# maxpit/human-pose-estimation

Measured on AMD Instinct MI355X. Metric: images/sec (224x224, batch 256/GPU), higher is better.
Workload: dtype f32; 1 GPU; batch=256/GPU 224x224x3 synthetic images, fp32 ResNet-50 v1 + 3-iter regressor + SMPL LBS at all 3 stages (configs[1] at batch 256; the BASELINE metric batch); global_batch=256, parallelism=dp1 (batch shard, replicated weights), regressor=synthetic 'survey' variant, input=float32 images resident in HBM

## Files before the change

human-pose-estimation_amd/_lib.py:

```python
from __future__ import annotations

import ctypes as C
import os

import numpy as np

_HERE = os.path.dirname(os.path.abspath(__file__))
LIB_PATH = os.path.join(_HERE, "lib", "libhpe_hip.so")

NUM_CONV = 53
NUM_DENSE = 3
NUM_VERTS = 6890
THETA_DIM = 85
FEATURE_DIM = 2048


class HpeError(RuntimeError):
    pass


class HpeConfig(C.Structure):
    _fields_ = [
        ("struct_size", C.c_int),
        ("device", C.c_int),
        ("max_batch", C.c_int),
        ("num_stage", C.c_int),
        ("bn_eps", C.c_float),
        ("encoder_dtype", C.c_int),
        ("n_streams", C.c_int),
        ("dual_gemm", C.c_int),
        ("stem_fused", C.c_int),
        ("wino_min_c", C.c_int),
        ("wino_min_items", C.c_int),
        ("wino_fused", C.c_int),
        ("wino_fused_min_hw", C.c_int),
        ("mesh_a2b", C.c_int),
        ("wino_f4", C.c_int),
        ("wino4_fused", C.c_int),
        ("bf16_p8", C.c_int),
        ("wino4_ksplit", C.c_int),
        ("chain_fuse", C.c_int),
        ("halo3", C.c_int),
    ]


PLAN_OPTIONS = ("n_streams", "dual_gemm", "stem_fused", "wino_min_c", "wino_min_items", "wino_fused", "wino_fused_min_hw", "mesh_a2b", "wino_f4", "wino4_fused", "bf16_p8", "wino4_ksplit", "chain_fuse", "halo3")


class HpeSmplModel(C.Structure):
    _fields_ = [
        ("v_template", C.c_void_p),
        ("shapedirs", C.c_void_p),
        ("posedirs", C.c_void_p),
        ("J_regressor", C.c_void_p),
        ("weights", C.c_void_p),
        ("kp_regressor", C.c_void_p),
        ("parents", C.c_void_p),
        ("num_kp", C.c_int),
    ]


class HpeRenderParams(C.Structure):
    _fields_ = [
        ("struct_size", C.c_int),
        ("color_id", C.c_int),
        ("do_alpha", C.c_int),
        ("rot_axis", C.c_int),
        ("rot_deg", C.c_float),
        ("near", C.c_float),
        ("far", C.c_float),
    ]


OUTPUT_FIELDS = ("verts", "joints", "cams", "theta", "J_transformed", "kp2d", "verts2d", "Rs")


class HpeOutputs(C.Structure):
    _fields_ = [(n, C.c_void_p) for n in OUTPUT_FIELDS]


_PROTOS = {
    "hpe_last_error": (C.c_char_p, []),
    "hpe_version": (C.c_char_p, []),
    "hpe_conv_layer_name": (C.c_char_p, [C.c_int]),
    "hpe_bn_layer_name": (C.c_char_p, [C.c_int]),
    "hpe_conv_layer_geometry": (C.c_int, [C.c_int, C.POINTER(C.c_int)]),
    "hpe_config_init": (None, [C.POINTER(HpeConfig)]),
    "hpe_create": (C.c_int, [C.POINTER(HpeConfig), C.POINTER(C.c_void_p)]),
    "hpe_destroy": (C.c_int, [C.c_void_p]),
    "hpe_load_smpl": (C.c_int, [C.c_void_p, C.POINTER(HpeSmplModel)]),
    "hpe_load_conv": (C.c_int, [C.c_void_p, C.c_int] + [C.c_void_p] * 6),
    "hpe_load_dense": (C.c_int, [C.c_void_p, C.c_int, C.c_void_p, C.c_void_p]),
    "hpe_load_mean_theta": (C.c_int, [C.c_void_p, C.c_void_p]),
    "hpe_finalize": (C.c_int, [C.c_void_p]),
    "hpe_forward": (C.c_int, [C.c_void_p, C.c_void_p, C.c_int, C.POINTER(HpeOutputs), C.c_int, C.c_void_p]),
    "hpe_forward_pipelined": (C.c_int, [C.c_void_p, C.c_void_p, C.c_int, C.POINTER(HpeOutputs), C.c_int, C.c_void_p]),
    "hpe_join": (C.c_int, [C.c_void_p, C.c_void_p]),
    "hpe_tail": (C.c_int, [C.c_void_p, C.c_void_p, C.c_int, C.POINTER(HpeOutputs), C.c_int, C.c_void_p]),
    "hpe_tail_stream": (C.c_void_p, [C.c_void_p]),
    "hpe_encoder": (C.c_int, [C.c_void_p, C.c_void_p, C.c_int, C.c_void_p, C.c_void_p]),
    "hpe_regress_stage": (C.c_int, [C.c_void_p, C.c_void_p, C.c_void_p, C.c_int, C.c_void_p, C.c_void_p]),
    "hpe_smpl": (C.c_int, [C.c_void_p, C.c_void_p, C.c_int, C.POINTER(HpeOutputs), C.c_void_p]),
    "hpe_orth_proj": (C.c_int, [C.c_void_p, C.c_void_p, C.c_int, C.c_int, C.c_void_p, C.c_void_p]),
    "hpe_reproject_vertices": (C.c_int, [C.c_void_p, C.c_void_p, C.c_int, C.c_int, C.c_float, C.c_float, C.c_void_p, C.c_void_p]),
    "hpe_preprocess_u8": (C.c_int, [C.c_void_p, C.c_int, C.c_int, C.c_int, C.c_void_p, C.POINTER(C.c_int), C.c_void_p]),
    "hpe_preprocess_u8_batch": (C.c_int, [C.c_void_p, C.POINTER(C.c_longlong), C.POINTER(C.c_int), C.c_int, C.c_int, C.c_void_p, C.POINTER(C.c_int),
                                          C.c_void_p, C.c_void_p]),
    "hpe_get_original": (C.c_int, [C.c_void_p, C.c_void_p, C.c_int, C.c_int, C.c_int, C.POINTER(C.c_int), C.c_float, C.c_int, C.c_void_p, C.POINTER(C.c_float), C.c_void_p, C.c_void_p, C.c_void_p]),
    "hpe_kp_loss": (C.c_int, [C.c_void_p, C.c_void_p, C.c_int, C.c_int, C.c_void_p, C.c_void_p]),
    "hpe_mesh_loss": (C.c_int, [C.c_void_p, C.c_void_p, C.c_void_p, C.c_int, C.c_int, C.c_int, C.c_int, C.c_void_p, C.c_void_p]),
    "hpe_val_losses": (C.c_int, [C.c_void_p, C.c_void_p, C.c_void_p, C.POINTER(C.c_void_p), C.POINTER(C.c_void_p), C.c_int, C.c_int, C.c_int,
                                 C.c_int, C.c_int, C.c_int, C.c_void_p, C.c_void_p]),
    "hpe_device_status": (C.c_int, [C.c_void_p, C.c_void_p]),
    "hpe_debug_conv": (C.c_int, [C.c_void_p, C.c_int, C.c_void_p, C.c_int, C.c_void_p, C.c_int, C.c_void_p, C.c_void_p]),
    "hpe_debug_chain": (C.c_int, [C.c_void_p, C.c_int, C.c_void_p, C.c_void_p, C.c_int, C.c_void_p, C.c_void_p, C.POINTER(C.c_int), C.c_void_p]),
    "hpe_debug_stem": (C.c_int, [C.c_void_p, C.c_void_p, C.c_int, C.c_int, C.c_void_p, C.c_void_p]),
    "hpe_debug_gemm": (C.c_int, [C.c_void_p, C.c_void_p, C.c_void_p, C.c_int, C.c_int, C.c_int, C.c_int, C.c_int, C.c_void_p, C.c_int, C.c_void_p, C.c_void_p]),
    "hpe_debug_set_dbg": (C.c_int, [C.c_void_p, C.c_void_p]),
    "hpe_debug_maxpool": (C.c_int, [C.c_void_p, C.c_int, C.c_int, C.c_int, C.c_void_p, C.c_void_p]),
    "hpe_debug_avgpool": (C.c_int, [C.c_void_p, C.c_int, C.c_int, C.c_int, C.c_void_p, C.c_void_p]),
    "hpe_debug_joint_regress": (C.c_int, [C.c_void_p, C.c_void_p, C.c_int, C.c_int, C.c_void_p, C.c_void_p]),
    "hpe_enable_timing": (C.c_int, [C.c_void_p, C.c_int]),
    "hpe_get_timings": (C.c_int, [C.c_void_p, C.POINTER(C.c_float)]),
    "hpe_get_span_stats": (C.c_int, [C.c_void_p, C.POINTER(C.c_float), C.POINTER(C.c_int)]),
    "hpe_get_loss_timings": (C.c_int, [C.c_void_p, C.POINTER(C.c_float)]),
    "hpe_debug_set_loss_counter": (C.c_int, [C.c_void_p, C.c_void_p]),
    "hpe_get_conv_timings": (C.c_int, [C.c_void_p, C.POINTER(C.c_float)]),
    "hpe_render_params_init": (None, [C.POINTER(HpeRenderParams)]),
    "hpe_renderer_create": (C.c_int, [C.c_int, C.c_void_p, C.c_int, C.c_int, C.c_int, C.POINTER(C.c_void_p)]),
    "hpe_renderer_destroy": (C.c_int, [C.c_void_p]),
    "hpe_render": (C.c_int, [C.c_void_p, C.c_void_p, C.c_void_p, C.c_int, C.c_int, C.c_int, C.c_void_p, C.POINTER(HpeRenderParams), C.c_void_p,
                             C.c_void_p]),
    "hpe_debug_render_ids": (C.c_int, [C.c_void_p, C.c_void_p, C.c_void_p, C.c_int, C.c_int, C.c_int, C.POINTER(HpeRenderParams), C.c_void_p,
                                       C.c_void_p, C.c_void_p]),
    "hpe_debug_render_vertices": (C.c_int, [C.c_void_p, C.c_void_p, C.c_void_p, C.c_int, C.c_int, C.c_int, C.POINTER(HpeRenderParams),
                                            C.c_void_p, C.c_void_p]),
}

_lib = None


def load():
    global _lib
    if _lib is not None:
        return _lib
    if not os.path.exists(LIB_PATH):
        raise HpeError(
            "%s not found: build it with `python -c 'import __graft_entry__ as g; g.build()'` "
            "(hipcc --offload-arch=gfx950).  There is no CPU fallback." % LIB_PATH
        )
    try:
        import torch
    except Exception:
        pass
    lib = C.CDLL(LIB_PATH, mode=C.RTLD_GLOBAL)
    for name, (res, args) in _PROTOS.items():
        fn = getattr(lib, name)
        fn.restype = res
        fn.argtypes = args
    _lib = lib
    return lib


def declared_symbols():
    return sorted(_PROTOS)


def check(rc):
    if rc != 0:
        msg = load().hpe_last_error()
        raise HpeError("libhpe_hip error %d: %s" % (rc, msg.decode() if msg else "?"))


def f32(a):
    arr = np.ascontiguousarray(a, dtype=np.float32)
    return arr, arr.ctypes.data_as(C.c_void_p)
```

human-pose-estimation_amd/build.py:

```python
from __future__ import annotations

import os
import shutil
import subprocess
import sys

HERE = os.path.dirname(os.path.abspath(__file__))
CSRC = os.path.join(HERE, "csrc")
LIBDIR = os.path.join(HERE, "lib")
LIB = os.path.join(LIBDIR, "libhpe_hip.so")
SOURCES = ["conv_gemm.hip", "conv_gemm_bf16.hip", "conv_gemm_bf16_p8.hip", "conv_chain_bf16.hip", "conv_chain_f32.hip", "conv3_halo_bf16.hip", "conv_wino.hip", "conv_wino4.hip", "stem_fused.hip", "encoder_ops.hip", "smpl.hip", "losses.hip", "prepost.hip", "render.hip", "hpe_api.hip"]
CFLAGS = ["--offload-arch=gfx950", "-O3", "-std=c++17", "-fPIC", "-fvisibility=hidden", "-fno-fast-math"]


def _hipcc():
    for cand in (os.environ.get("HIPCC"), shutil.which("hipcc"), "/opt/rocm/bin/hipcc"):
        if cand and os.path.exists(cand):
            return cand
    raise RuntimeError("hipcc not found (set HIPCC or install ROCm under /opt/rocm)")


def _deps():
    return [os.path.join(CSRC, f) for f in os.listdir(CSRC) if f.endswith(".h")] + [os.path.join(HERE, "..", "include", "hpe.h")]


def _obj_stale(src, obj):
    if not os.path.exists(obj):
        return True
    t = os.path.getmtime(obj)
    return any(os.path.getmtime(d) > t for d in [src] + _deps() if os.path.exists(d))


def _flags_now():
    return " ".join(CFLAGS + os.environ.get("HPE_EXTRA_FLAGS", "").split())


def built_flags():
    tag = os.path.join(LIBDIR, "obj", "flags.txt")
    return open(tag).read() if os.path.exists(tag) else ""


def _stale():
    if not os.path.exists(LIB):
        return True
    if built_flags() != _flags_now():
        return True
    t = os.path.getmtime(LIB)
    deps = [os.path.join(CSRC, f) for f in os.listdir(CSRC)] + [os.path.join(HERE, "..", "include", "hpe.h")]
    return any(os.path.getmtime(d) > t for d in deps if os.path.exists(d))


def build(force=False, verbose=False):
    if not force and not _stale():
        return LIB
    os.makedirs(LIBDIR, exist_ok=True)
    objdir = os.path.join(LIBDIR, "obj")
    os.makedirs(objdir, exist_ok=True)
    extra = os.environ.get("HPE_EXTRA_FLAGS", "").split()
    tag = os.path.join(objdir, "flags.txt")
    flags_now = _flags_now()
    if force or not os.path.exists(tag) or open(tag).read() != flags_now:
        for f in os.listdir(objdir):
            os.remove(os.path.join(objdir, f))
    hipcc = _hipcc()
    jobs = []
    for s in SOURCES:
        src = os.path.join(CSRC, s)
        if not os.path.exists(src):
            continue
        obj = os.path.join(objdir, s.replace(".hip", ".o"))
        jobs.append((src, obj))

    def compile_one(job):
        src, obj = job
        if not _obj_stale(src, obj):
            return None
        cmd = [hipcc] + CFLAGS + extra + ["-c", "-o", obj + ".tmp%d" % os.getpid(), src]
        if verbose:
            print(" ".join(cmd), file=sys.stderr)
        r = subprocess.run(cmd, capture_output=True, text=True)
        if r.returncode != 0:
            return "hipcc failed on %s:\n%s%s" % (os.path.basename(src), r.stdout, r.stderr)
        os.replace(obj + ".tmp%d" % os.getpid(), obj)
        return None

    from concurrent.futures import ThreadPoolExecutor

    with ThreadPoolExecutor(max_workers=min(len(jobs), max(1, (os.cpu_count() or 2) - 1))) as ex:
        errs = [e for e in ex.map(compile_one, jobs) if e]
    if errs:
        raise RuntimeError("\n".join(errs))
    open(tag, "w").write(flags_now)
    tmp = LIB + ".tmp%d" % os.getpid()
    cmd = [hipcc, "--offload-arch=gfx950", "-shared", "-fPIC", "-o", tmp] + [o for _, o in jobs]
    r = subprocess.run(cmd, capture_output=True, text=True)
    if r.returncode != 0:
        raise RuntimeError("link failed:\n" + r.stdout + r.stderr)
    os.replace(tmp, LIB)
    return LIB


if __name__ == "__main__":
    print(build(force="--force" in sys.argv, verbose=True))
```

human-pose-estimation_amd/csrc/conv_gemm.hip:

```cpp
#include <hip/hip_runtime.h>
#include <stdint.h>
#include <stdlib.h>

#include "hpe_internal.h"

typedef float f32x16 __attribute__((ext_vector_type(16)));
typedef float f32x4 __attribute__((ext_vector_type(4)));

#define BK 32
#define LDS_PITCH 36

namespace {

struct RowAddr {
    int base;
    unsigned mask;
};

template <int MODE>
__device__ __forceinline__ RowAddr make_row(const GemmArgs& p, int m, int kc4) {
    RowAddr r;
    r.mask = 0x1ffu;
    if (m >= p.M) m = p.M - 1;
    if (MODE == GEMM_DENSE || MODE == GEMM_DUAL) {
        r.base = m * p.lda + kc4;
    } else {
        const int hw = p.Ho * p.Wo;
        const int b = m / hw;
        const int rem = m - b * hw;
        const int ho = rem / p.Wo;
        const int wo = rem - ho * p.Wo;
        if (MODE == GEMM_STRIDED) {
            r.base = ((b * p.Hi + ho * p.stride) * p.Wi + wo * p.stride) * p.Cin + kc4;
        } else if (MODE == GEMM_CONV3) {
            r.base = ((b * p.Hi + ho) * p.Wi + wo) * p.Cin + kc4;
            unsigned mk = 0;
#pragma unroll
            for (int tap = 0; tap < 9; ++tap) {
                const int dh = tap / 3 - 1, dw = tap % 3 - 1;
                if ((unsigned)(ho + dh) < (unsigned)p.Hi && (unsigned)(wo + dw) < (unsigned)p.Wi) mk |= 1u << tap;
            }
            r.mask = mk;
        } else {
            r.base = ((b * p.Hi + 2 * ho) * p.Wi + 2 * wo) * 4 + kc4;
        }
    }
    return r;
}

struct SlabPos {
    int off;
    int tap;
    int cs;
};

template <int MODE>
__device__ __forceinline__ void slab_advance(const GemmArgs& p, SlabPos& sp) {
    if (MODE == GEMM_DENSE || MODE == GEMM_STRIDED || MODE == GEMM_DUAL) {
        sp.off += BK;
    } else if (MODE == GEMM_CONV3) {
        sp.cs += 1;
        sp.off += BK;
        if (sp.cs == p.cin_slabs) {
            sp.cs = 0;
            sp.tap += 1;
            const int kh = sp.tap / 3;
            sp.off = ((kh - 1) * p.Wi + (sp.tap - kh * 3 - 1)) * p.Cin;
        }
    } else {
        sp.off += p.Wi * 4;
    }
}

template <int MODE>
__device__ __forceinline__ SlabPos slab_first(const GemmArgs& p) {
    SlabPos sp;
    sp.tap = 0;
    sp.cs = 0;
    sp.off = (MODE == GEMM_CONV3) ? (-p.Wi - 1) * p.Cin : 0;
    return sp;
}

template <int MODE>
__device__ __forceinline__ SlabPos slab_seek(const GemmArgs& p, int slab) {
    SlabPos sp;
    sp.tap = 0;
    sp.cs = 0;
    if (MODE == GEMM_DENSE || MODE == GEMM_STRIDED || MODE == GEMM_DUAL) {
        sp.off = slab * BK;
    } else if (MODE == GEMM_CONV3) {
        sp.tap = slab / p.cin_slabs;
        sp.cs = slab - sp.tap * p.cin_slabs;
        const int kh = sp.tap / 3;
        sp.off = ((kh - 1) * p.Wi + (sp.tap - kh * 3 - 1)) * p.Cin + sp.cs * BK;
    } else {
        sp.off = slab * p.Wi * 4;
    }
    return sp;
}

template <int MODE>
__device__ __forceinline__ f32x4 load_a(const GemmArgs& p, const RowAddr& r, const SlabPos& sp) {
    if (MODE == GEMM_CONV3) {
        const bool ok = (r.mask >> sp.tap) & 1u;
        f32x4 v = *reinterpret_cast<const f32x4*>(p.x + (r.base + (ok ? sp.off : sp.cs * BK)));
        const f32x4 z = {0.f, 0.f, 0.f, 0.f};
        return ok ? v : z;
    }
    return *reinterpret_cast<const f32x4*>(p.x + (r.base + sp.off));
}

template <int MODE, int BM, int BN, int WM, int WN, int SCHED>
__global__ __launch_bounds__(256, 2) void conv_gemm_f32_kernel(GemmArgs p) {
    constexpr int MT = BM / WM / 32;
    constexpr int NT = BN / WN / 32;
    constexpr int AP = BM / 32;
    constexpr int BP = BN / 32;
    constexpr int EP = BN + 4;
    static_assert(WM * WN == 4, "4 waves per workgroup");
    static_assert(MT >= 1 && NT >= 1, "tile too small");
    static_assert(BM * EP <= 2 * (BM + BN) * LDS_PITCH, "epilogue tile must fit the staging LDS");

    __shared__ __attribute__((aligned(16))) float lds[2 * (BM + BN) * LDS_PITCH];
    constexpr int BUF = (BM + BN) * LDS_PITCH;

    const int total = p.n_mtiles * p.n_ntiles;
    const int bid = blockIdx.x;
    const int xcd = bid & 7;
    const int q = total >> 3, rr = total & 7;
    const int swz = (xcd < rr ? xcd * (q + 1) : rr * (q + 1) + (xcd - rr) * q) + (bid >> 3);
    const int mtile = swz / p.n_ntiles;
    const int ntile = swz - mtile * p.n_ntiles;
    const int m0 = mtile * BM;
    const int n0 = ntile * BN;

    const int t = threadIdx.x;
    const int lane = t & 63;
    const int wave = __builtin_amdgcn_readfirstlane(t >> 6);
    const int wm = wave / WN;
    const int wn = wave - wm * WN;

    const int kc4 = (t & 7) * 4;
    const int srow = t >> 3;
    RowAddr arow[AP];
#pragma unroll
    for (int i = 0; i < AP; ++i) arow[i] = make_row<MODE>(p, m0 + srow + 32 * i, kc4);
    const float* wptr = p.w + (size_t)(n0 + srow) * p.ldw + kc4;
    const int lds_st = srow * LDS_PITCH + kc4;

    const int frag = (lane & 31) * LDS_PITCH + 4 * (lane >> 5);
    const int a_off = (wm * MT * 32) * LDS_PITCH + frag;
    const int b_off = (BM + wn * NT * 32) * LDS_PITCH + frag;

    f32x16 acc[MT][NT];
#pragma unroll
    for (int i = 0; i < MT; ++i)
#pragma unroll
        for (int j = 0; j < NT; ++j)
#pragma unroll
            for (int e = 0; e < 16; ++e) acc[i][j][e] = 0.f;

    f32x4 ra[AP], rb[BP];
    const int S = p.K / BK;
    SlabPos sp = slab_first<MODE>(p);

    auto load_slab = [&](int slab) {
#pragma unroll
        for (int i = 0; i < AP; ++i) ra[i] = load_a<MODE>(p, arow[i], sp);
#pragma unroll
        for (int i = 0; i < BP; ++i) rb[i] = *reinterpret_cast<const f32x4*>(wptr + (size_t)(32 * i) * p.ldw + slab * BK);
    };
    auto store_slab = [&](int buf) {
#pragma unroll
        for (int i = 0; i < AP; ++i) *reinterpret_cast<f32x4*>(&lds[buf + lds_st + 32 * i * LDS_PITCH]) = ra[i];
#pragma unroll
        for (int i = 0; i < BP; ++i) *reinterpret_cast<f32x4*>(&lds[buf + lds_st + (BM + 32 * i) * LDS_PITCH]) = rb[i];
    };
    auto mma_groups = [&](int buf, int g0, int g1) {
        const float* A = &lds[buf + a_off];
        const float* B = &lds[buf + b_off];
#pragma unroll
        for (int g = g0; g < g1; ++g) {
            f32x4 fa[MT], fb[NT];
#pragma unroll
            for (int i = 0; i < MT; ++i) fa[i] = *reinterpret_cast<const f32x4*>(A + i * 32 * LDS_PITCH + g * 8);
#pragma unroll
            for (int j = 0; j < NT; ++j) fb[j] = *reinterpret_cast<const f32x4*>(B + j * 32 * LDS_PITCH + g * 8);
#pragma unroll
            for (int ks = 0; ks < 4; ++ks)
#pragma unroll
                for (int i = 0; i < MT; ++i)
#pragma unroll
                    for (int j = 0; j < NT; ++j)
                        acc[i][j] = __builtin_amdgcn_mfma_f32_32x32x2f32(fa[i][ks], fb[j][ks], acc[i][j], 0, 0, 0);
        }
    };

#ifdef HPE_ABLATION
    unsigned long long t_clk0 = 0, t_rt0 = 0;
    if (p.dbg) {
        t_clk0 = __builtin_amdgcn_s_memtime();
        t_rt0 = __builtin_amdgcn_s_memrealtime();
    }
#endif
    load_slab(0);
    store_slab(0);
    if (S > 1) {
        slab_advance<MODE>(p, sp);
        load_slab(1);
    }
    __syncthreads();

    if (SCHED == 8 || SCHED == 9) {
        constexpr int QA = AP / 4 > 0 ? AP / 4 : 1;
        constexpr int QB = BP / 4 > 0 ? BP / 4 : 1;
        constexpr int GA = AP / QA, GB = BP / QB;
        constexpr int MPG = 4 * MT * NT;
        int s = 0;
        for (; s + 2 < S; ++s) {
            const int cur = (s & 1) * BUF;
            const int nxt = BUF - cur;
            const float* A = &lds[cur + a_off];
            const float* B = &lds[cur + b_off];
            slab_advance<MODE>(p, sp);
            f32x4 fa[2][MT], fb[2][NT];
#pragma unroll
            for (int i = 0; i < MT; ++i) fa[0][i] = *reinterpret_cast<const f32x4*>(A + i * 32 * LDS_PITCH);
#pragma unroll
            for (int j = 0; j < NT; ++j) fb[0][j] = *reinterpret_cast<const f32x4*>(B + j * 32 * LDS_PITCH);
#define HPE_KGROUP(G)                                                                                                  \
    {                                                                                                                  \
        if (G < 3) {                                                                                                   \
            _Pragma("unroll") for (int i = 0; i < MT; ++i) fa[(G + 1) & 1][i] =                                        \
                *reinterpret_cast<const f32x4*>(A + i * 32 * LDS_PITCH + (G + 1) * 8);                                 \
            _Pragma("unroll") for (int j = 0; j < NT; ++j) fb[(G + 1) & 1][j] =                                        \
                *reinterpret_cast<const f32x4*>(B + j * 32 * LDS_PITCH + (G + 1) * 8);                                 \
        }                                                                                                              \
        _Pragma("unroll") for (int ks = 0; ks < 4; ++ks) _Pragma("unroll") for (int i = 0; i < MT; ++i)                \
            _Pragma("unroll") for (int j = 0; j < NT; ++j) acc[i][j] =                                                 \
                __builtin_amdgcn_mfma_f32_32x32x2f32(fa[G & 1][i][ks], fb[G & 1][j][ks], acc[i][j], 0, 0, 0);          \
        if (G < GA) {                                                                                                  \
            _Pragma("unroll") for (int q = 0; q < QA; ++q) {                                                           \
                const int i = G * QA + q;                                                                              \
                *reinterpret_cast<f32x4*>(&lds[nxt + lds_st + 32 * i * LDS_PITCH]) = ra[i];                            \
                ra[i] = load_a<MODE>(p, arow[i], sp);                                                                  \
            }                                                                                                          \
        }                                                                                                              \
        if (G < GB) {                                                                                                  \
            _Pragma("unroll") for (int q = 0; q < QB; ++q) {                                                           \
                const int i = G * QB + q;                                                                              \
                *reinterpret_cast<f32x4*>(&lds[nxt + lds_st + (BM + 32 * i) * LDS_PITCH]) = rb[i];                     \
                rb[i] = *reinterpret_cast<const f32x4*>(wptr + (size_t)(32 * i) * p.ldw + (s + 2) * BK);               \
            }                                                                                                          \
        }                                                                                                              \
        if (SCHED == 9) {                                                                                              \
            constexpr int NST = (G < GA ? QA : 0) + (G < GB ? QB : 0);                                                 \
            if (G < 3) __builtin_amdgcn_sched_group_barrier(0x100, MT + NT, 0);                                        \
            if constexpr (NST == 0) {                                                                                  \
                __builtin_amdgcn_sched_group_barrier(0x008, MPG, 0);                                                   \
            } else {                                                                                                   \
                _Pragma("unroll") for (int q = 0; q < NST; ++q) {                                                      \
                    __builtin_amdgcn_sched_group_barrier(0x008, MPG / NST, 0);                                         \
                    __builtin_amdgcn_sched_group_barrier(0x200, 1, 0);                                                 \
                    __builtin_amdgcn_sched_group_barrier(0x020, 1, 0);                                                 \
                }                                                                                                      \
            }                                                                                                          \
        }                                                                                                              \
    }
            HPE_KGROUP(0)
            HPE_KGROUP(1)
            HPE_KGROUP(2)
            HPE_KGROUP(3)
#undef HPE_KGROUP
            __syncthreads();
        }
        for (; s < S; ++s) {
            const int cur = (s & 1) * BUF;
            mma_groups(cur, 0, 2);
            if (s + 1 < S) store_slab(BUF - cur);
            mma_groups(cur, 2, 4);
            __syncthreads();
        }
    } else
    for (int s = 0; s < S; ++s) {
        const int cur = (s & 1) * BUF;
        if (SCHED == 0) {
            mma_groups(cur, 0, 2);
            if (s + 1 < S) {
                store_slab(BUF - cur);
                if (s + 2 < S) {
                    slab_advance<MODE>(p, sp);
                    load_slab(s + 2);
                }
            }
            mma_groups(cur, 2, 4);
        } else if (SCHED == 1) {
            mma_groups(cur, 0, 2);
            __builtin_amdgcn_sched_barrier(0);
            if (s + 1 < S) {
                store_slab(BUF - cur);
                __builtin_amdgcn_sched_barrier(0);
                if (s + 2 < S) {
                    slab_advance<MODE>(p, sp);
                    load_slab(s + 2);
                }
            }
            __builtin_amdgcn_sched_barrier(0);
            mma_groups(cur, 2, 4);
        } else if (SCHED == 6) {
            if (s + 2 < S) {
                slab_advance<MODE>(p, sp);
                load_slab(s + 2);
            }
            mma_groups(cur, 0, 4);
#pragma unroll
            for (int i = 0; i < AP; ++i) asm volatile("" ::"v"(ra[i]));
#pragma unroll
            for (int i = 0; i < BP; ++i) asm volatile("" ::"v"(rb[i]));
        } else if (SCHED == 7) {
            mma_groups(cur, 0, 2);
            if (s + 1 < S) store_slab(BUF - cur);
            mma_groups(cur, 2, 4);
        } else if (SCHED == 3) {
            mma_groups(cur, 0, 4);
        } else if (SCHED == 4) {
            mma_groups(0, 0, 4);
            continue;
        } else if (SCHED == 5) {
            f32x4 fa[MT], fb[NT];
#pragma unroll
            for (int i = 0; i < MT; ++i) fa[i] = ra[i % AP];
#pragma unroll
            for (int j = 0; j < NT; ++j) fb[j] = rb[j % BP];
#pragma unroll
            for (int g = 0; g < 4; ++g)
#pragma unroll
                for (int ks = 0; ks < 4; ++ks)
#pragma unroll
                    for (int i = 0; i < MT; ++i)
#pragma unroll
                        for (int j = 0; j < NT; ++j)
                            acc[i][j] = __builtin_amdgcn_mfma_f32_32x32x2f32(fa[i][ks], fb[j][ks], acc[i][j], 0, 0, 0);
            continue;
        } else {
            mma_groups(cur, 0, 1);
            __builtin_amdgcn_sched_barrier(0);
            if (s + 1 < S) store_slab(BUF - cur);
            mma_groups(cur, 1, 2);
            __builtin_amdgcn_sched_barrier(0);
            if (s + 2 < S) {
                slab_advance<MODE>(p, sp);
                load_slab(s + 2);
            }
            mma_groups(cur, 2, 3);
            __builtin_amdgcn_sched_barrier(0);
            mma_groups(cur, 3, 4);
        }
        __syncthreads();
    }

#ifdef HPE_ABLATION
    if (p.dbg && t == 0) {
        p.dbg[2 * bid] = __builtin_amdgcn_s_memtime() - t_clk0;
        p.dbg[2 * bid + 1] = __builtin_amdgcn_s_memrealtime() - t_rt0;
    }
#endif
    {
        const int col_l = lane & 31;
        const int row_l = 4 * (lane >> 5);
#pragma unroll
        for (int j = 0; j < NT; ++j) {
            const int cl = (wn * NT + j) * 32 + col_l;
            const int n = n0 + cl;
            const bool n_ok = n < p.N;
            const float sc = n_ok ? p.scale[n] : 0.f;
            const float sh = n_ok ? p.shift[n] : 0.f;
#pragma unroll
            for (int i = 0; i < MT; ++i) {
                const int rl = (wm * MT + i) * 32 + row_l;
#pragma unroll
                for (int e = 0; e < 16; ++e) lds[(rl + (e & 3) + 8 * (e >> 2)) * EP + cl] = acc[i][j][e] * sc + sh;
            }
        }
    }
    __syncthreads();
    {
        constexpr int TPR = BN / 4;
        constexpr int RPP = 256 / TPR;
        const int r = t / TPR;
        const int c4 = (t - r * TPR) * 4;
        const int n = n0 + c4;
        const bool full = (n + 3) < p.N;
#pragma unroll 4
        for (int pass = 0; pass < BM / RPP; ++pass) {
            const int row = pass * RPP + r;
            const int m = m0 + row;
            if (m >= p.M || n >= p.N) continue;
            f32x4 v = *reinterpret_cast<const f32x4*>(&lds[row * EP + c4]);
            if (full) {
                if (p.res) v += *reinterpret_cast<const f32x4*>(p.res + (size_t)m * p.ldres + n);
                if (p.relu) {
                    v.x = fmaxf(v.x, 0.f);
                    v.y = fmaxf(v.y, 0.f);
                    v.z = fmaxf(v.z, 0.f);
                    v.w = fmaxf(v.w, 0.f);
                }
                if (p.y_slab8)
                    *reinterpret_cast<f32x4*>(p.y + ((size_t)(n >> 3) * p.M + m) * 8 + (n & 7)) = v;
                else
                    *reinterpret_cast<f32x4*>(p.y + (size_t)m * p.ldy + n) = v;
            } else {
                const float vv[4] = {v.x, v.y, v.z, v.w};
#pragma unroll
                for (int u = 0; u < 4; ++u) {
                    if (n + u < p.N) {
                        float o = vv[u];
                        if (p.res) o += p.res[(size_t)m * p.ldres + n + u];
                        if (p.relu) o = fmaxf(o, 0.f);
                        p.y[(size_t)m * p.ldy + n + u] = o;
                    }
                }
            }
        }
    }
}

#ifdef HPE_F32_RES_NT
#define HPE_RES_LOAD(ptr) __builtin_nontemporal_load(ptr)
#else
#define HPE_RES_LOAD(ptr) (*(ptr))
#endif
template <int BM, int BN, int WM, int WN, int NP>
__device__ __forceinline__ void conv_epilogue(const GemmArgs& p, float* lds, f32x16 (&acc)[BM / WM / 32][BN / WN / 32], int m0, int n0, int t,
                                              int lane, int wm, int wn, const f32x4 (&rpre)[NP], bool use_pre) {
    constexpr int MT = BM / WM / 32;
    constexpr int NT = BN / WN / 32;
    constexpr int NTHR = 64 * WM * WN;
    constexpr int EP = BN + 4;
    {
        const int col_l = lane & 31;
        const int row_l = 4 * (lane >> 5);
#pragma unroll
        for (int j = 0; j < NT; ++j) {
            const int cl = (wn * NT + j) * 32 + col_l;
            const int n = n0 + cl;
            const bool n_ok = n < p.N;
            const float sc = n_ok ? p.scale[n] : 0.f;
            const float sh = n_ok ? p.shift[n] : 0.f;
#pragma unroll
            for (int i = 0; i < MT; ++i) {
                const int rl = (wm * MT + i) * 32 + row_l;
#pragma unroll
                for (int e = 0; e < 16; ++e) lds[(rl + (e & 3) + 8 * (e >> 2)) * EP + cl] = acc[i][j][e] * sc + sh;
            }
        }
    }
    __syncthreads();
    {
        constexpr int TPR = BN / 4;
        constexpr int RPP = NTHR / TPR;
        const int r = t / TPR;
        const int c4 = (t - r * TPR) * 4;
        const int n = n0 + c4;
        const bool full = (n + 3) < p.N;
#pragma unroll
        for (int pass = 0; pass < BM / RPP; ++pass) {
            const int row = pass * RPP + r;
            const int m = m0 + row;
            if (m >= p.M || n >= p.N) continue;
            f32x4 v = *reinterpret_cast<const f32x4*>(&lds[row * EP + c4]);
            if (full) {
                if (use_pre) v += rpre[pass < NP ? pass : 0];
                else if (p.res) v += HPE_RES_LOAD(reinterpret_cast<const f32x4*>(p.res + (size_t)m * p.ldres + n));
                if (p.relu) {
                    v.x = fmaxf(v.x, 0.f);
                    v.y = fmaxf(v.y, 0.f);
                    v.z = fmaxf(v.z, 0.f);
                    v.w = fmaxf(v.w, 0.f);
                }
                if (p.y_slab8)
                    *reinterpret_cast<f32x4*>(p.y + ((size_t)(n >> 3) * p.M + m) * 8 + (n & 7)) = v;
                else
                    *reinterpret_cast<f32x4*>(p.y + (size_t)m * p.ldy + n) = v;
            } else {
                const float vv[4] = {v.x, v.y, v.z, v.w};
#pragma unroll
                for (int u = 0; u < 4; ++u) {
                    if (n + u < p.N) {
                        float o = vv[u];
                        if (p.res) o += p.res[(size_t)m * p.ldres + n + u];
                        if (p.relu) o = fmaxf(o, 0.f);
                        p.y[(size_t)m * p.ldy + n + u] = o;
                    }
                }
            }
        }
    }
}

template <int MODE, int BM, int BN, int WM, int WN>
__global__ __launch_bounds__(64 * WM * WN, (WM * WN) / 2) void conv_gemm_f32_dma_kernel(GemmArgs p) {
    constexpr int MT = BM / WM / 32;
    constexpr int NT = BN / WN / 32;
    constexpr int NW = WM * WN;
    constexpr int NTHR = 64 * NW;
    constexpr int AP = BM / (8 * NW);
    constexpr int BP = BN / (8 * NW);
    constexpr int EP = BN + 4;
    constexpr int BUF = (BM + BN) * BK;
    constexpr int LDS_FLOATS = (2 * BUF > BM * EP) ? 2 * BUF : BM * EP;
    static_assert(NW == 4 || NW == 8, "4 or 8 waves per workgroup");
    static_assert(AP >= 1 && BP >= 1, "tile too small for the wave count");

    __shared__ __attribute__((aligned(16))) float lds[LDS_FLOATS];

    const int total = p.n_mtiles * p.n_ntiles;
    const int bid = blockIdx.x;
    int tile, ks0 = 0, ks1 = p.K / BK, part = -1;
    if (p.split_k > 1) {
        tile = bid / p.split_k;
        part = bid - tile * p.split_k;
        const int S = p.K / BK;
        ks0 = (int)((long)part * S / p.split_k);
        ks1 = (int)((long)(part + 1) * S / p.split_k);
    } else {
        const int xcd = bid & 7;
        const int q = total >> 3, rr = total & 7;
        tile = (xcd < rr ? xcd * (q + 1) : rr * (q + 1) + (xcd - rr) * q) + (bid >> 3);
    }
    const int mtile = tile / p.n_ntiles;
    const int ntile = tile - mtile * p.n_ntiles;
    const int m0 = mtile * BM;
    const int n0 = ntile * BN;

    const int t = threadIdx.x;
    const int lane = t & 63;
    const int wave = __builtin_amdgcn_readfirstlane(t >> 6);
    const int wm = wave / WN;
    const int wn = wave - wm * WN;

    const int drow = lane >> 3;
    RowAddr arow[AP];
    int arow2[MODE == GEMM_DUAL ? AP : 1];
    const float* wsrc[BP];
#pragma unroll
    for (int i = 0; i < AP; ++i) {
        const int r = (NW * i + wave) * 8 + drow;
        const int lc = (lane & 7) ^ ((r >> 1) & 7);
        arow[i] = make_row<MODE>(p, m0 + r, lc * 4);
        if (MODE == GEMM_DUAL) arow2[i] = make_row<GEMM_STRIDED>(p, m0 + r, lc * 4).base;
    }
#pragma unroll
    for (int i = 0; i < BP; ++i) {
        const int r = (NW * i + wave) * 8 + drow;
        const int lc = (lane & 7) ^ ((r >> 1) & 7);
        wsrc[i] = p.w + (size_t)(n0 + r) * p.ldw + lc * 4;
    }

    int a_row[MT], b_row[NT], a_x[MT], b_x[NT];
#pragma unroll
    for (int i = 0; i < MT; ++i) {
        const int r = (wm * MT + i) * 32 + (lane & 31);
        a_row[i] = r * BK;
        a_x[i] = (r >> 1) & 7;
    }
#pragma unroll
    for (int j = 0; j < NT; ++j) {
        const int r = (wn * NT + j) * 32 + (lane & 31);
        b_row[j] = (BM + r) * BK;
        b_x[j] = (r >> 1) & 7;
    }
    const int hi = lane >> 5;

    f32x16 acc[MT][NT];
#pragma unroll
    for (int i = 0; i < MT; ++i)
#pragma unroll
        for (int j = 0; j < NT; ++j)
#pragma unroll
            for (int e = 0; e < 16; ++e) acc[i][j][e] = 0.f;

    constexpr int R_TPR = BN / 4, R_RPP = NTHR / R_TPR, R_NPASS = BM / R_RPP;
    constexpr bool R_PRE = (NW == 8) && R_NPASS <= 4;
    f32x4 rpre[R_PRE ? R_NPASS : 1];
    bool r_pre = false;
    if constexpr (R_PRE) {
        const int rr_ = t / R_TPR;
        const int n = n0 + (t - rr_ * R_TPR) * 4;
        r_pre = p.res != nullptr && p.res_prefetch && part < 0 && (n + 3) < p.N;
        if (r_pre) {
#pragma unroll
            for (int pass = 0; pass < R_NPASS; ++pass) {
                const int m = m0 + pass * R_RPP + rr_;
                rpre[pass] = HPE_RES_LOAD(reinterpret_cast<const f32x4*>(p.res + (size_t)(m < p.M ? m : p.M - 1) * p.ldres + n));
            }
        }
    }

    SlabPos sp = slab_seek<MODE>(p, ks0);

    auto issue_dma = [&](int slab, int buf) {
#pragma unroll
        for (int i = 0; i < AP; ++i) {
            const float* src;
            if (MODE == GEMM_CONV3) {
                const bool ok = (arow[i].mask >> sp.tap) & 1u;
                src = ok ? (p.x + (arow[i].base + sp.off)) : p.zero;
            } else if (MODE == GEMM_DUAL) {
                src = slab < p.k1_slabs ? p.x + (arow[i].base + slab * BK) : p.x2 + (arow2[i] + (slab - p.k1_slabs) * BK);
            } else {
                src = p.x + (arow[i].base + sp.off);
            }
            __builtin_amdgcn_global_load_lds((const __attribute__((address_space(1))) void*)src,
                                             (__attribute__((address_space(3))) void*)(lds + buf + (NW * i + wave) * 8 * BK), 16, 0, 0);
        }
#pragma unroll
        for (int i = 0; i < BP; ++i) {
            __builtin_amdgcn_global_load_lds((const __attribute__((address_space(1))) void*)(wsrc[i] + slab * BK),
                                             (__attribute__((address_space(3))) void*)(lds + buf + (BM + (NW * i + wave) * 8) * BK), 16, 0,
                                             0);
        }
    };

    issue_dma(ks0, 0);
    __builtin_amdgcn_s_waitcnt(0x0F70);
    __syncthreads();

    for (int s = ks0; s < ks1; ++s) {
        const int cur = ((s - ks0) & 1) * BUF;
        if (s + 1 < ks1) {
            slab_advance<MODE>(p, sp);
            issue_dma(s + 1, BUF - cur);
        }
#pragma unroll
        for (int g = 0; g < 4; ++g) {
            f32x4 fa[MT], fb[NT];
            const int lc = 2 * g + hi;
#pragma unroll
            for (int i = 0; i < MT; ++i) fa[i] = *reinterpret_cast<const f32x4*>(&lds[cur + a_row[i] + ((lc ^ a_x[i]) << 2)]);
#pragma unroll
            for (int j = 0; j < NT; ++j) fb[j] = *reinterpret_cast<const f32x4*>(&lds[cur + b_row[j] + ((lc ^ b_x[j]) << 2)]);
#pragma unroll
            for (int ks = 0; ks < 4; ++ks)
#pragma unroll
                for (int i = 0; i < MT; ++i)
#pragma unroll
                    for (int j = 0; j < NT; ++j)
                        acc[i][j] = __builtin_amdgcn_mfma_f32_32x32x2f32(fa[i][ks], fb[j][ks], acc[i][j], 0, 0, 0);
        }
        __builtin_amdgcn_s_waitcnt(0x0F70);
        __syncthreads();
    }

    if (part >= 0) {
        f32x4* dst = reinterpret_cast<f32x4*>(p.partial) + (size_t)(tile * p.split_k + part) * (MT * NT * 4 * NTHR) + t;
#pragma unroll
        for (int i = 0; i < MT; ++i)
#pragma unroll
            for (int j = 0; j < NT; ++j)
#pragma unroll
                for (int qd = 0; qd < 4; ++qd) {
                    f32x4 v = {acc[i][j][4 * qd], acc[i][j][4 * qd + 1], acc[i][j][4 * qd + 2], acc[i][j][4 * qd + 3]};
                    dst[((i * NT + j) * 4 + qd) * NTHR] = v;
                }
        return;
    }
    conv_epilogue<BM, BN, WM, WN>(p, lds, acc, m0, n0, t, lane, wm, wn, rpre, R_PRE && r_pre);
}

template <int BM, int BN, int WM, int WN>
__global__ __launch_bounds__(64 * WM * WN) void conv_gemm_fixup_kernel(GemmArgs p) {
    constexpr int MT = BM / WM / 32;
    constexpr int NT = BN / WN / 32;
    constexpr int NTHR = 64 * WM * WN;
    constexpr int EP = BN + 4;
    __shared__ __attribute__((aligned(16))) float lds[BM * EP];
    const int t = threadIdx.x;
    const int lane = t & 63;
    const int wave = __builtin_amdgcn_readfirstlane(t >> 6);
    const int wm = wave / WN;
    const int wn = wave - wm * WN;
    const int tile = blockIdx.x;
    const int mtile = tile / p.n_ntiles;
    const int ntile = tile - mtile * p.n_ntiles;
    f32x16 acc[MT][NT];
#pragma unroll
    for (int i = 0; i < MT; ++i)
#pragma unroll
        for (int j = 0; j < NT; ++j)
#pragma unroll
            for (int e = 0; e < 16; ++e) acc[i][j][e] = 0.f;
    const f32x4* src = reinterpret_cast<const f32x4*>(p.partial) + (size_t)tile * p.split_k * (MT * NT * 4 * NTHR) + t;
    for (int part = 0; part < p.split_k; ++part) {
#pragma unroll
        for (int i = 0; i < MT; ++i)
#pragma unroll
            for (int j = 0; j < NT; ++j)
#pragma unroll
                for (int qd = 0; qd < 4; ++qd) {
                    const f32x4 v = src[(size_t)part * (MT * NT * 4 * NTHR) + ((i * NT + j) * 4 + qd) * NTHR];
                    acc[i][j][4 * qd] += v.x;
                    acc[i][j][4 * qd + 1] += v.y;
                    acc[i][j][4 * qd + 2] += v.z;
                    acc[i][j][4 * qd + 3] += v.w;
                }
    }
    const f32x4 no_pre[1] = {{0.f, 0.f, 0.f, 0.f}};
    conv_epilogue<BM, BN, WM, WN>(p, lds, acc, mtile * BM, ntile * BN, t, lane, wm, wn, no_pre, false);
}

int stage_variant() {
    static const int v = [] {
        const char* e = getenv("HPE_STAGE");
        return (e && e[0] == 'r') ? 0 : 1;
    }();
    return v;
}

int sched_variant() {
    static const int v = [] {
        const char* e = getenv("HPE_SCHED");
        const int x = e ? atoi(e) : 0;
        return (x < 0 || x > 9) ? 0 : x;
    }();
    return v;
}

int splitk_enabled() {
    static const int v = [] {
        const char* e = getenv("HPE_SPLITK");
        return e ? atoi(e) : 1;
    }();
    return v;
}

template <int MODE, int BM, int BN, int WM, int WN>
hipError_t launch_cfg(GemmArgs& p, hipStream_t st) {
    p.n_mtiles = (p.M + BM - 1) / BM;
    p.n_ntiles = (p.N + BN - 1) / BN;
    const int grid = p.n_mtiles * p.n_ntiles;
    p.split_k = 1;
    if constexpr (WM * WN == 8) {
        static const int res_prefetch = [] {
            const char* e = getenv("HPE_RES_PREFETCH");
            return e ? atoi(e) : 1;
        }();
        p.res_prefetch = res_prefetch;
        hipLaunchKernelGGL((conv_gemm_f32_dma_kernel<MODE, BM, BN, WM, WN>), dim3(grid), dim3(512), 0, st, p);
        return hipGetLastError();
    } else {
    if ((stage_variant() == 1 && p.zero) || MODE == GEMM_DUAL) {
        const int S = p.K / BK;
        static const int min_slabs = [] {
            const char* e = getenv("HPE_SPLITK_SLABS");
            const int v = e ? atoi(e) : 4;
            return v < 2 ? 2 : v;
        }();
        if (p.partial && splitk_enabled() && grid < 128 && S >= 2 * min_slabs) {
            int sk = 256 / grid;
            if (sk > S / min_slabs) sk = S / min_slabs;
            if (sk > 16) sk = 16;
            while (sk > 1 && (size_t)grid * sk * BM * BN > p.partial_floats) --sk;
            if (sk > 1) p.split_k = sk;
        }
        hipLaunchKernelGGL((conv_gemm_f32_dma_kernel<MODE, BM, BN, WM, WN>), dim3(grid * p.split_k), dim3(256), 0, st, p);
        hipError_t e = hipGetLastError();
        if (e != hipSuccess || p.split_k == 1) return e;
        hipLaunchKernelGGL((conv_gemm_fixup_kernel<BM, BN, WM, WN>), dim3(grid), dim3(256), 0, st, p);
        return hipGetLastError();
    }
    if constexpr (MODE == GEMM_DUAL) return hipErrorInvalidValue;
    else
    switch (sched_variant()) {
        case 1: hipLaunchKernelGGL((conv_gemm_f32_kernel<MODE, BM, BN, WM, WN, 1>), dim3(grid), dim3(256), 0, st, p); break;
        case 2: hipLaunchKernelGGL((conv_gemm_f32_kernel<MODE, BM, BN, WM, WN, 2>), dim3(grid), dim3(256), 0, st, p); break;
#ifdef HPE_ABLATION
        case 3: hipLaunchKernelGGL((conv_gemm_f32_kernel<MODE, BM, BN, WM, WN, 3>), dim3(grid), dim3(256), 0, st, p); break;
        case 4: hipLaunchKernelGGL((conv_gemm_f32_kernel<MODE, BM, BN, WM, WN, 4>), dim3(grid), dim3(256), 0, st, p); break;
        case 5: hipLaunchKernelGGL((conv_gemm_f32_kernel<MODE, BM, BN, WM, WN, 5>), dim3(grid), dim3(256), 0, st, p); break;
        case 6: hipLaunchKernelGGL((conv_gemm_f32_kernel<MODE, BM, BN, WM, WN, 6>), dim3(grid), dim3(256), 0, st, p); break;
        case 7: hipLaunchKernelGGL((conv_gemm_f32_kernel<MODE, BM, BN, WM, WN, 7>), dim3(grid), dim3(256), 0, st, p); break;
        case 8: hipLaunchKernelGGL((conv_gemm_f32_kernel<MODE, BM, BN, WM, WN, 8>), dim3(grid), dim3(256), 0, st, p); break;
        case 9: hipLaunchKernelGGL((conv_gemm_f32_kernel<MODE, BM, BN, WM, WN, 9>), dim3(grid), dim3(256), 0, st, p); break;
#endif
        default: hipLaunchKernelGGL((conv_gemm_f32_kernel<MODE, BM, BN, WM, WN, 0>), dim3(grid), dim3(256), 0, st, p); break;
    }
    return hipGetLastError();
    }
}

template <int MODE>
hipError_t launch_mode(GemmArgs& p, int tile, hipStream_t st) {
    switch (tile) {
        case TILE_128x128: return launch_cfg<MODE, 128, 128, 2, 2>(p, st);
        case TILE_128x64: return launch_cfg<MODE, 128, 64, 2, 2>(p, st);
        case TILE_64x64: return launch_cfg<MODE, 64, 64, 2, 2>(p, st);
        case TILE_64x128: return launch_cfg<MODE, 64, 128, 2, 2>(p, st);
        case TILE_128x128_W8: return launch_cfg<MODE, 128, 128, 2, 4>(p, st);
        case TILE_128x64_W8: return launch_cfg<MODE, 128, 64, 4, 2>(p, st);
        case TILE_256x128_W8: return launch_cfg<MODE, 256, 128, 4, 2>(p, st);
        default: return hipErrorInvalidValue;
    }
// ... 39 lines not shown
```

human-pose-estimation_amd/csrc/hpe_api.hip:

```cpp
#include <hip/hip_runtime.h>

#include <cmath>
#include <cstdint>
#include <cstdio>
#include <cstdlib>
#include <cstring>
#include <string>
#include <vector>

#include "../../include/hpe.h"
#include "hpe_internal.h"

namespace {

thread_local std::string g_err;

int fail(int code, const std::string& msg) {
    g_err = msg;
    return code;
}

#define HIP_TRY(expr)                                                                                             \
    do {                                                                                                          \
        hipError_t _e = (expr);                                                                                   \
        if (_e != hipSuccess)                                                                                     \
            return fail(HPE_ERR_HIP, std::string(#expr) + ": " + hipGetErrorString(_e) + " (" __FILE__ ":" +      \
                                         std::to_string(__LINE__) + ")");                                         \
    } while (0)

struct ConvSpec {
    char name[24];
    char bn[24];
    int kh, kw, cin, cout, stride, hin, hout;
};

std::vector<ConvSpec> build_specs() {
    std::vector<ConvSpec> v;
    auto add = [&](const std::string& n, const std::string& b, int kh, int cin, int cout, int s, int hin, int hout) {
        ConvSpec c;
        snprintf(c.name, sizeof c.name, "%s", n.c_str());
        snprintf(c.bn, sizeof c.bn, "%s", b.c_str());
        c.kh = c.kw = kh;
        c.cin = cin;
        c.cout = cout;
        c.stride = s;
        c.hin = hin;
        c.hout = hout;
        v.push_back(c);
    };
    add("conv1", "bn_conv1", 7, 3, 64, 2, 224, 112);
    const int nblk[4] = {3, 4, 6, 3};
    const int filt[4][3] = {{64, 64, 256}, {128, 128, 512}, {256, 256, 1024}, {512, 512, 2048}};
    int cin = 64, h = 56;
    for (int st = 0; st < 4; ++st) {
        for (int b = 0; b < nblk[st]; ++b) {
            const bool first = b == 0;
            const int s = (first && st > 0) ? 2 : 1;
            const int hout = h / s;
            char base[24], bn[24];
            snprintf(base, sizeof base, "res%d%c_branch", st + 2, 'a' + b);
            snprintf(bn, sizeof bn, "bn%d%c_branch", st + 2, 'a' + b);
            add(std::string(base) + "2a", std::string(bn) + "2a", 1, cin, filt[st][0], s, h, hout);
            add(std::string(base) + "2b", std::string(bn) + "2b", 3, filt[st][0], filt[st][1], 1, hout, hout);
            add(std::string(base) + "2c", std::string(bn) + "2c", 1, filt[st][1], filt[st][2], 1, hout, hout);
            if (first) add(std::string(base) + "1", std::string(bn) + "1", 1, cin, filt[st][2], s, h, hout);
            cin = filt[st][2];
            h = hout;
        }
    }
    return v;
}

const std::vector<ConvSpec>& specs() {
    static const std::vector<ConvSpec> s = build_specs();
    return s;
}

inline int round_up(int x, int m) { return ((x + m - 1) / m) * m; }

struct ConvLayer {
    std::vector<float> kernel, bias, gamma, beta, mean, var;
    bool loaded = false;
    float* w = nullptr;
    float* scale = nullptr;
    float* shift = nullptr;
    float* w_dual = nullptr;
    float* shift_dual = nullptr;
    int k_dual = 0, k1_dual = 0;
    void* stem_w = nullptr;
    float* wino_u = nullptr;
    float* wino4_u = nullptr;
    int n_pad = 0, k_pad = 0;
};

inline unsigned short f2bf(float f) {
    unsigned u;
    memcpy(&u, &f, 4);
    return (unsigned short)((u + 0x7FFFu + ((u >> 16) & 1u)) >> 16);
}

struct DenseLayer {
    std::vector<float> kernel, bias;
    bool loaded = false;
};

constexpr int STEM_HP = 230;
constexpr int STEM_WP = 232;
constexpr int THETA_LD = 96;
constexpr size_t WINO_V_PITCH = 802816 + 16384;
constexpr size_t WINO_V_SLACK = 524288;

}

struct TileKnobs {
    int force_wide = -1, force_narrow = -1, shortk = TILE_128x64_W8, force_bf16 = -1;
    int bf16_128_min_tiles = 192;
    int concurrent_tiles = 0;
    int wide128_min_tiles = 384;
    int force_expand = -1;
    int expand_small_grid = 128;
    int bf16_w8_min_tiles = 128;
    int force_ns_bf16 = -1;
    int bf16_rules = 1;
    int bf16_p8 = 0;
    int bf16_p8_min_n = 256;
    int bf16_p8_min_k = 512;
};

struct hpe_ctx {
    HpeConfig cfg{};
    bool finalized = false;
    bool dead = false;
    TileKnobs knobs;
    bool bf16 = false;
    bool have_encoder = false, have_regressor = false, have_smpl = false;
    ConvLayer conv[HPE_NUM_CONV];
    DenseLayer dense[HPE_NUM_DENSE];
    bool smpl_loaded = false, mean_loaded = false;
    std::vector<float> h_vt, h_sd, h_pd, h_jreg, h_w, h_kreg;
    std::vector<int> h_par;
    int num_kp = 19;
    float h_mean[HPE_THETA_DIM];
    float *w1f = nullptr, *w1t = nullptr, *w2 = nullptr, *w3 = nullptr, *b1 = nullptr, *b2 = nullptr, *b3 = nullptr;
    float *ones = nullptr, *zeros = nullptr, *mean_dev = nullptr;
    SmplDev smpl{};
    SmplWork work{};
    float* smpl_basis_src = nullptr;
    float *padded = nullptr, *X0 = nullptr, *X1 = nullptr, *T1 = nullptr, *T2 = nullptr, *SC = nullptr;
    float *feat = nullptr, *P1 = nullptr, *H1 = nullptr, *H2 = nullptr, *thA = nullptr, *thB = nullptr;
    float* loss_ws = nullptr;
    unsigned long long* dbg = nullptr;
    size_t loss_ws_floats = 0;
    std::vector<void*> allocs;
    int n_streams = 1;
    float* partial = nullptr;
    size_t partial_floats = 0;
    int chunk_images = 0;
    float* wino_v = nullptr;
    float* wino_ws = nullptr;
    unsigned* wino_flags = nullptr;
    unsigned* dev_err = nullptr;
    unsigned wino_epoch = 0;
    int n_cu = 0;
    int wino_min_c = 128;
    int wino_min_items = 128;
    int wino_fused_min_hw = 28;
    int dual_gemm = 1;
    int stem_fused = 1;
    int wino4_min_items = 64;
    int wino4_fused = 0;
    int wino_f4 = 0;
    int mesh_a2b = 0;
    bool loss_attr_done = false;
    unsigned long long* loss_counter = nullptr;
    int wino_fused = 1;
    hipStream_t aux[3]{};
    int min_chunk = 32;
    hipEvent_t ev_fork{}, ev_join[3]{};
    hipStream_t tail_st{};
    hipEvent_t ev_enc{}, ev_tail{}, ev_feat_free[2]{};
    bool feat_free_valid[2] = {false, false};
    bool tail_pending = false;
    unsigned pipe_idx = 0;
    float* feat_alt = nullptr;
    int wino4_ksplit = 1;
    int halo3_two = 4;
    int halo3 = 0;
    int chain_fuse = 0;
    int co_running = 1;
    float* w4_split = nullptr;
    float* partial_tail = nullptr;
    size_t partial_tail_floats = 0;
    bool dense_on_tail = false;
    int timing = 0;
    hipEvent_t ev[8]{};
    static constexpr int SPAN_RING = 64;
    hipEvent_t span0[SPAN_RING]{}, span1[SPAN_RING]{};
    unsigned span_n = 0;
    hipEvent_t cev0[HPE_NUM_CONV]{}, cev1[HPE_NUM_CONV]{};
    hipEvent_t lev0[16]{}, lev1[16]{}, lev_all[2]{};
    int loss_timed_stages = 0;
    bool ev_ok = false, timed_valid = false, conv_timed_valid = false;
};

namespace {

struct DeviceGuard {
    int prev = -1;
    bool changed = false;
    explicit DeviceGuard(int dev) {
        if (hipGetDevice(&prev) == hipSuccess && prev != dev) changed = hipSetDevice(dev) == hipSuccess;
    }
    ~DeviceGuard() {
        if (changed) (void)hipSetDevice(prev);
    }
};

int dev_alloc(hpe_ctx* c, float** p, size_t n_floats, bool zero) {
    void* q = nullptr;
    HIP_TRY(hipMalloc(&q, n_floats * sizeof(float)));
    c->allocs.push_back(q);
    if (zero) HIP_TRY(hipMemset(q, 0, n_floats * sizeof(float)));
    *p = static_cast<float*>(q);
    return HPE_OK;
}

int upload(hpe_ctx* c, float** p, const std::vector<float>& h) {
    int rc = dev_alloc(c, p, h.size(), false);
    if (rc) return rc;
    HIP_TRY(hipMemcpy(*p, h.data(), h.size() * sizeof(float), hipMemcpyHostToDevice));
    return HPE_OK;
}

int pick_tile(const TileKnobs& kn, int M, int N, int K, bool residual_expand = false, bool concurrent = false) {
    const bool wide = N > 64;
    if (wide && residual_expand) {
        if (kn.force_expand >= 0) return kn.force_expand;
        return (long)((M + 127) / 128) * ((N + 63) / 64) < kn.expand_small_grid ? TILE_64x64 : TILE_128x64_W8;
    }
    if (wide && kn.force_wide >= 0) return kn.force_wide;
    if (!wide && kn.force_narrow >= 0) return kn.force_narrow;
    if (!wide) return TILE_128x64;
    if (K <= 128 && M >= 150000) return kn.shortk;
    if ((concurrent || kn.concurrent_tiles) && kn.wide128_min_tiles > 0 && (long)((M + 127) / 128) * ((N + 127) / 128) >= kn.wide128_min_tiles) return TILE_128x128;
    if (M >= 150000) return TILE_64x128;
    return TILE_64x64;
}

struct Bf16Plan {
    int tile, ns;
};

Bf16Plan pick_bf16(const TileKnobs& kn, int M, int N, int K, bool residual_expand, bool concurrent = false, int mode = GEMM_DENSE) {
    Bf16Plan pl{TILE_128x64, 2};
    if (kn.bf16_p8 && N >= kn.bf16_p8_min_n && N % 256 == 0 && K >= kn.bf16_p8_min_k && !residual_expand) {
        const int bit = mode == GEMM_CONV3 ? (N == 256 ? 1 : 2) : (mode == GEMM_DUAL ? (N >= 2048 ? 8 : 16) : 4);
        if (kn.bf16_p8 & bit) return Bf16Plan{TILE_P8_256x256, 2};
    }
    if (N > 64) {
        const long t128 = (long)((M + 127) / 128) * ((N + 127) / 128);
        pl.tile = t128 >= ((concurrent || kn.concurrent_tiles) ? kn.bf16_128_min_tiles : 512) ? TILE_128x128 : TILE_64x128;
        if (kn.bf16_rules) {
            if (residual_expand) pl.tile = TILE_128x64_W8;
            else if (M <= 16384 && M >= 8192 && K >= 1024 && N >= 256) pl.tile = TILE_256x128_W8;
            if (kn.bf16_w8_min_tiles > 0 && t128 >= kn.bf16_w8_min_tiles) pl.tile = TILE_128x128_W8;
        }
        if (kn.force_bf16 >= 0) pl.tile = kn.force_bf16;
    }
    if (kn.force_ns_bf16 >= 2) pl.ns = kn.force_ns_bf16;
    return pl;
}

#define HIPE(expr)                               \
    do {                                         \
        hipError_t _e = (expr);                  \
        if (_e != hipSuccess) return _e;         \
    } while (0)


inline int f4_bit(int hin) { return hin <= 7 ? 1 : (hin <= 14 ? 2 : (hin <= 28 ? 4 : 8)); }

bool use_wino4(const hpe_ctx* c, int idx, int B) {
    const ConvSpec& s = specs()[idx];
    return !c->bf16 && c->conv[idx].wino4_u && s.kh == 3 && s.stride == 1 && (c->wino_f4 & f4_bit(s.hin)) &&
           hpe_wino4_items(B, s.hin, s.hin, s.cout) >= (c->wino_min_items < c->wino4_min_items ? c->wino_min_items : c->wino4_min_items);
}

bool use_wino4_fused(const hpe_ctx* c, int idx, int B) {
    const ConvSpec& s = specs()[idx];
    return !c->bf16 && c->conv[idx].wino4_u && s.kh == 3 && s.stride == 1 && (c->wino4_fused & f4_bit(s.hin)) &&
           hpe_wino4_fused_items(B, s.hin, s.hin, s.cout) >= (c->wino_min_items < c->wino4_min_items ? c->wino_min_items : c->wino4_min_items);
}

bool use_wino_fused(const hpe_ctx* c, int idx, int B) {
    const ConvSpec& s = specs()[idx];
    if (use_wino4_fused(c, idx, B) || use_wino4(c, idx, B)) return false;
    return c->wino_fused && !c->bf16 && c->conv[idx].wino_u && s.kh == 3 && s.stride == 1 && s.hin >= c->wino_fused_min_hw &&
           hpe_wino_fused_items(B, s.hin, s.hin, s.cout) >= c->wino_min_items;
}

enum { CONV_OUT_SLAB8 = 1, CONV_IN_SLAB8 = 2, CONV_CONCURRENT = 4 };

hipError_t run_conv(hpe_ctx* c, int idx, const float* x, int B, const float* res, int relu, float* y, hipStream_t st,
                    float* wino_v = nullptr, int slot = 0, int flags = 0) {
    const ConvSpec& s = specs()[idx];
    const ConvLayer& L = c->conv[idx];
    if ((flags & CONV_IN_SLAB8) && use_wino4_fused(c, idx, B))
        return hpe_launch_wino4_fused_conv3(x, L.wino4_u, L.scale, L.shift, c->zeros, y, s.cout, B, s.hin, s.hin, s.cin, s.cout, relu, st);
    if (flags & CONV_IN_SLAB8)
        return hpe_launch_wino_fused_conv3(x, L.wino_u, L.scale, L.shift, c->zeros, y, s.cout, B, s.hin, s.hin, s.cin, s.cout, relu, st);
    if (wino_v && !res && use_wino4(c, idx, B))
        return hpe_launch_wino4_conv3(x, s.cin, L.wino4_u, L.scale, L.shift, y, s.cout, B, s.hin, s.hin, s.cin, s.cout, relu, wino_v, st,
                                      (flags & CONV_CONCURRENT) ? c->co_running : 1,
                                      c->w4_split && slot >= 0 && slot < 4 ? c->w4_split + (size_t)slot * hpe_wino4_split_ws_floats() : nullptr);
    if (L.wino_u && wino_v && !res && s.cin >= c->wino_min_c &&
        (long)((B * ((s.hin + 1) / 2) * ((s.hin + 1) / 2) + 63) / 64) * (s.cout / 64) >= c->wino_min_items)
    {
        WinoStreamK sk{};
        if (c->wino_ws && slot >= 0 && slot < 4) {
            sk.ws = c->wino_ws + (size_t)slot * c->n_cu * HPE_WINO_WS_FLOATS;
            sk.flags = c->wino_flags + (size_t)slot * c->n_cu;
            sk.epoch = ++c->wino_epoch;
            if (sk.epoch == 0) sk.epoch = ++c->wino_epoch;
            sk.n_wg = c->n_cu;
            sk.err = c->dev_err;
        }
        return hpe_launch_wino_conv3(x, s.cin, L.wino_u, L.scale, L.shift, y, s.cout, B, s.hin, s.hin, s.cin, s.cout, relu, wino_v,
                                     c->wino_ws ? &sk : nullptr, st);
    }
    GemmArgs p{};
    p.x = x;
    p.w = L.w;
    p.scale = L.scale;
    p.shift = L.shift;
    p.res = res;
    p.y = y;
    p.M = B * s.hout * s.hout;
    p.N = s.cout;
    p.K = L.k_pad;
    p.ldw = L.k_pad;
    p.w_rows = L.n_pad;
    p.ldy = s.cout;
    p.ldres = s.cout;
    p.relu = relu;
    p.Hi = p.Wi = s.hin;
    p.Cin = s.cin;
    p.Ho = p.Wo = s.hout;
    p.stride = s.stride;
    p.cin_slabs = s.cin / 32;
    p.lda = s.cin;
    p.zero = c->zeros;
    p.y_slab8 = (flags & CONV_OUT_SLAB8) ? 1 : 0;
    if (!(flags & CONV_CONCURRENT)) {
        p.partial = c->partial;
        p.partial_floats = c->partial_floats;
    }
    int mode;
    if (idx == 0) {
        mode = GEMM_STEM;
        p.Hi = STEM_HP;
        p.Wi = STEM_WP;
        p.Cin = 4;
    } else if (s.kh == 3) {
        mode = GEMM_CONV3;
    } else if (s.stride == 1) {
        mode = GEMM_DENSE;
    } else {
        mode = GEMM_STRIDED;
    }
    if (c->bf16 && mode == GEMM_CONV3 && !res && s.stride == 1 && (c->halo3 & f4_bit(s.hin) ? true : false) &&
        hpe_halo3_bf16_supported(s.hin, s.cin, s.cout) && L.k_pad >= 9 * s.cin)
    {
        Halo3Args h{};
        h.x = reinterpret_cast<const __bf16*>(x);
        h.w = reinterpret_cast<const __bf16*>(L.w);
        h.scale = L.scale;
        h.shift = L.shift;
        h.y = reinterpret_cast<__bf16*>(y);
        h.M = p.M;
        h.N = s.cout;
        h.ldw = L.k_pad;
        h.relu = relu;
        h.two = c->halo3_two;
        return hpe_launch_halo3_bf16(h, s.hin, s.cin, st);
    }
    if (c->bf16) {
        p.cin_slabs = s.cin / 64;
        const Bf16Plan pl = pick_bf16(c->knobs, p.M, p.N, p.K, mode == GEMM_DENSE && res != nullptr && s.cout == 4 * s.cin, (flags & CONV_CONCURRENT) != 0, mode);
        return hpe_launch_gemm_bf16(p, mode, pl.tile, pl.ns, st);
    }
    return hpe_launch_gemm(p, mode, pick_tile(c->knobs, p.M, p.N, p.K, mode == GEMM_DENSE && res != nullptr && s.cout == 4 * s.cin, (flags & CONV_CONCURRENT) != 0), st);
}

hipError_t run_dual(hpe_ctx* c, int i2c, int i1, const float* t2, const float* x, int B, float* y, hipStream_t st, int flags) {
    const ConvSpec& s2 = specs()[i2c];
    const ConvSpec& s1 = specs()[i1];
    const ConvLayer& L = c->conv[i2c];
    const int slab = c->bf16 ? 64 : 32;
    GemmArgs p{};
    p.x = t2;
    p.x2 = x;
    p.w = L.w_dual;
    p.scale = c->ones;
    p.shift = L.shift_dual;
    p.y = y;
    p.M = B * s2.hout * s2.hout;
    p.N = s2.cout;
    p.K = L.k_dual;
    p.k1_slabs = L.k1_dual / slab;
    p.lda = s2.cin;
    p.ldw = L.k_dual;
    p.w_rows = round_up(s2.cout, 128);
    p.ldy = s2.cout;
    p.relu = 1;
    p.Hi = p.Wi = s1.hin;
    p.Cin = s1.cin;
    p.Ho = p.Wo = s1.hout;
    p.stride = s1.stride;
    p.zero = c->zeros;
    if (!(flags & CONV_CONCURRENT)) {
        p.partial = c->partial;
        p.partial_floats = c->partial_floats;
    }
    if (c->bf16) {
        const Bf16Plan pl = pick_bf16(c->knobs, p.M, p.N, p.K, false, (flags & CONV_CONCURRENT) != 0, GEMM_DUAL);
        return hpe_launch_gemm_bf16(p, GEMM_DUAL, pl.tile, pl.ns, st);
    }
    return hpe_launch_gemm(p, GEMM_DUAL, pick_tile(c->knobs, p.M, p.N, p.K, false, (flags & CONV_CONCURRENT) != 0), st);
}

bool use_chain(const hpe_ctx* c, int stg, int i2c, bool first, bool has_next) {
    if (!has_next) return false;
    const ConvSpec& s2 = specs()[i2c];
    if (!c->bf16) {
        if (first || stg != 0 || !(c->chain_fuse & 8)) return false;
        const ConvSpec& sn = specs()[i2c + 1];
        return sn.kh == 1 && sn.stride == 1 && sn.cin == s2.cout && hpe_chain_f32_supported(s2.cin, s2.cout, sn.cout);
    }
    if (first) {
        const ConvSpec& s1 = specs()[i2c + 1];
        const ConvSpec& sn = specs()[i2c + 2];
        return stg == 0 && (c->chain_fuse & 4) && c->conv[i2c].w_dual && s1.stride == 1 && s1.hin == s2.hin && sn.kh == 1 && sn.stride == 1 &&
               sn.cin == s2.cout && c->conv[i2c].k_dual == s2.cin + s1.cin && hpe_chain_bf16_supported(s2.cin, s2.cout, sn.cout, s1.cin);
    }
    const int bit = stg == 0 ? 1 : stg == 1 ? 2 : stg == 2 ? 16 : 0;
    if (!(c->chain_fuse & bit)) return false;
    const ConvSpec& sn = specs()[i2c + 1];
    return sn.kh == 1 && sn.stride == 1 && sn.cin == s2.cout && hpe_chain_bf16_supported(s2.cin, s2.cout, sn.cout, 0);
}

hipError_t run_chain(hpe_ctx* c, int i2c, bool first, const float* t2, const float* res, int B, float* t3, float* u1, hipStream_t st,
                     bool u1_slab8 = false) {
    const ConvSpec& s2 = specs()[i2c];
    const int inext = i2c + (first ? 2 : 1);
    const ConvSpec& sn = specs()[inext];
    const ConvLayer& L2 = c->conv[i2c];
    const ConvLayer& Ln = c->conv[inext];
    if (!c->bf16) {
        ChainArgsF32 q{};
        q.t2 = t2;
        q.res = res;
        q.w2c = L2.w;
        q.w2a = Ln.w;
        q.scaleA = L2.scale;
        q.shiftA = L2.shift;
        q.scaleB = Ln.scale;
        q.shiftB = Ln.shift;
        q.t3 = t3;
        q.u1 = u1;
        q.M = B * s2.hout * s2.hout;
        q.ldw2c = L2.k_pad;
        q.ldw2a = Ln.k_pad;
        q.u1_slab8 = u1_slab8 ? 1 : 0;
        return hpe_launch_chain_f32(q, s2.cin, s2.cout, sn.cout, st);
    }
    ChainArgs p{};
    p.t2 = reinterpret_cast<const __bf16*>(t2);
    if (first) {
        p.x2 = reinterpret_cast<const __bf16*>(res);
        p.w2c = reinterpret_cast<const __bf16*>(L2.w_dual);
        p.scaleA = c->ones;
        p.shiftA = L2.shift_dual;
        p.ldw2c = L2.k_dual;
    } else {
        p.res = reinterpret_cast<const __bf16*>(res);
        p.w2c = reinterpret_cast<const __bf16*>(L2.w);
        p.scaleA = L2.scale;
        p.shiftA = L2.shift;
        p.ldw2c = L2.k_pad;
    }
    p.w2a = reinterpret_cast<const __bf16*>(Ln.w);
    p.scaleB = Ln.scale;
    p.shiftB = Ln.shift;
    p.t3 = reinterpret_cast<__bf16*>(t3);
    p.u1 = reinterpret_cast<__bf16*>(u1);
    p.M = B * s2.hout * s2.hout;
    p.ldw2a = Ln.k_pad;
    return hpe_launch_chain_bf16(p, s2.cin, s2.cout, sn.cout, first ? specs()[i2c + 1].cin : 0, st);
}

hipError_t run_dense(hpe_ctx* c, const float* x, int lda, int M, int K, const float* w, int w_rows, int N, const float* scale,
                     const float* shift, const float* res, int ldres, int relu, float* y, int ldy, hipStream_t st) {
    if (M <= 4) return hpe_launch_dense_gemv(x, lda, M, K, w, N, scale, shift, res, ldres, relu, y, ldy, st);
    GemmArgs p{};
    p.zero = shift;
    p.partial = c->dense_on_tail ? c->partial_tail : c->partial;
    p.partial_floats = c->dense_on_tail ? c->partial_tail_floats : c->partial_floats;
    p.x = x;
    p.w = w;
    p.scale = scale;
    p.shift = shift;
    p.res = res;
    p.y = y;
    p.M = M;
    p.N = N;
    p.K = K;
    p.lda = lda;
    p.ldw = K;
    p.w_rows = w_rows;
    p.ldy = ldy;
    p.ldres = ldres;
    p.relu = relu;
    return hpe_launch_gemm(p, GEMM_DENSE, TILE_64x64, st);
}

hipError_t timed_conv(hpe_ctx* c, int idx, const float* x, int B, const float* res, int relu, float* y, hipStream_t st,
                      float* wino_v = nullptr, int slot = 0, int flags = 0) {
    const bool t2 = c->timing >= 2;
    if (t2) HIPE(hipEventRecord(c->cev0[idx], st));
    HIPE(run_conv(c, idx, x, B, res, relu, y, st, wino_v, slot, flags));
    if (t2) HIPE(hipEventRecord(c->cev1[idx], st));
    return hipSuccess;
}

hipError_t encoder_chunk(hpe_ctx* c, const float* images, int i0, int B, float* features, int ldfeat, hipStream_t st, int slot = 0,
                         bool concurrent = false) {
    const int cf = concurrent ? CONV_CONCURRENT : 0;
    const int esz = c->bf16 ? 2 : 4;
    auto at = [&](float* base, size_t elems) { return reinterpret_cast<float*>(reinterpret_cast<char*>(base) + elems * esz); };
    const size_t o_img = (size_t)i0 * HPE_IMG_SIZE * HPE_IMG_SIZE * 3;
    const size_t o_pad = (size_t)i0 * STEM_HP * STEM_WP * 4;
    const size_t o_big = (size_t)i0 * 802816;
    const size_t o_mid = (size_t)i0 * 200704;
    float* padded = at(c->padded, o_pad);
    float* SC = at(c->SC, o_big);
    float* T1 = at(c->T1, o_mid);
    float* T2 = at(c->T2, o_mid);
    float* cur = at(c->X0, o_big);
    float* nxt = at(c->X1, o_big);
    float* wv = (c->wino_v && (i0 == 0 || B >= 32)) ? c->wino_v + (size_t)i0 * WINO_V_PITCH : nullptr;
    if (c->stem_fused && (reinterpret_cast<uintptr_t>(images + o_img) & 15) == 0) {
        const bool t2 = c->timing >= 2;
        if (t2) HIPE(hipEventRecord(c->cev0[0], st));
        HIPE(hpe_launch_stem_fused(images + o_img, c->conv[0].stem_w, c->conv[0].scale, c->conv[0].shift, cur, B, hpe_stem_fused_pick_rows(B),
                                   c->bf16 ? 1 : 0, st));
        if (t2) HIPE(hipEventRecord(c->cev1[0], st));
    } else if (c->bf16) {
        HIPE(hpe_launch_pad_input_bf16(images + o_img, padded, B, HPE_IMG_SIZE, HPE_IMG_SIZE, STEM_HP, STEM_WP, st));
        HIPE(timed_conv(c, 0, padded, B, nullptr, 1, SC, st, nullptr, 0, cf));
        HIPE(hpe_launch_maxpool_bf16(SC, cur, B, 112, 64, st));
    } else {
        HIPE(hpe_launch_pad_input(images + o_img, padded, B, HPE_IMG_SIZE, HPE_IMG_SIZE, STEM_HP, STEM_WP, st));
        HIPE(timed_conv(c, 0, padded, B, nullptr, 1, SC, st, nullptr, 0, cf));
        HIPE(hpe_launch_maxpool(SC, cur, B, 112, 64, st));
    }
    int ci = 1;
    const int nblk[4] = {3, 4, 6, 3};
    bool have_2a = false;
    for (int stg = 0; stg < 4; ++stg) {
        for (int b = 0; b < nblk[stg]; ++b) {
            const bool first = b == 0;
            const int i2a = ci, i2b = ci + 1, i2c = ci + 2, i1 = ci + 3;
            const bool fz = use_wino_fused(c, i2b, B) || use_wino4_fused(c, i2b, B);
            if (have_2a) {
                if (c->timing >= 2) {
                    HIPE(hipEventRecord(c->cev0[i2a], st));
                    HIPE(hipEventRecord(c->cev1[i2a], st));
                }
            } else {
                HIPE(timed_conv(c, i2a, cur, B, nullptr, 1, T1, st, nullptr, 0, cf | (fz ? CONV_OUT_SLAB8 : 0)));
            }
            have_2a = false;
            HIPE(timed_conv(c, i2b, T1, B, nullptr, 1, T2, st, wv, slot, cf | (fz ? CONV_IN_SLAB8 : 0)));
            const float* res = cur;
            if (use_chain(c, stg, i2c, first, b + 1 < nblk[stg])) {
                const bool t2 = c->timing >= 2;
                if (t2) HIPE(hipEventRecord(c->cev0[i2c], st));
                const int i2b_next = i2c + (first ? 3 : 2);
                const bool slab8_next = !c->bf16 && (use_wino_fused(c, i2b_next, B) || use_wino4_fused(c, i2b_next, B));
                HIPE(run_chain(c, i2c, first, T2, cur, B, nxt, T1, st, slab8_next));
                if (t2) {
                    HIPE(hipEventRecord(c->cev1[i2c], st));
                    if (first) {
                        HIPE(hipEventRecord(c->cev0[i1], st));
                        HIPE(hipEventRecord(c->cev1[i1], st));
                    }
                }
                have_2a = true;
            } else if (first && c->conv[i2c].w_dual) {
                const bool t2 = c->timing >= 2;
                if (t2) HIPE(hipEventRecord(c->cev0[i2c], st));
                HIPE(run_dual(c, i2c, i1, T2, cur, B, nxt, st, cf));
                if (t2) {
                    HIPE(hipEventRecord(c->cev1[i2c], st));
                    HIPE(hipEventRecord(c->cev0[i1], st));
                    HIPE(hipEventRecord(c->cev1[i1], st));
                }
            } else {
                if (first) {
                    HIPE(timed_conv(c, i1, cur, B, nullptr, 0, SC, st, nullptr, 0, cf));
                    res = SC;
                }
                HIPE(timed_conv(c, i2c, T2, B, res, 1, nxt, st, nullptr, 0, cf));
            }
            ci += first ? 4 : 3;
            float* t = cur;
            cur = nxt;
            nxt = t;
        }
    }
    if (c->bf16) return hpe_launch_avgpool_bf16(cur, features + (size_t)i0 * ldfeat, B, 49, HPE_FEATURE_DIM, ldfeat, st);
    return hpe_launch_avgpool(cur, features + (size_t)i0 * ldfeat, B, 49, HPE_FEATURE_DIM, ldfeat, st);
}

hipError_t encoder_impl(hpe_ctx* c, const float* images, int B, float* features, int ldfeat, hipStream_t st) {
    int nstream = c->n_streams;
    if (nstream > B / c->min_chunk) nstream = B / c->min_chunk;
    if (c->timing >= 2 || nstream < 2) nstream = 1;
    if (nstream == 1) return encoder_chunk(c, images, 0, B, features, ldfeat, st);
    int nchunk = nstream;
    if (c->chunk_images > 0) {
        const int want = c->chunk_images < c->min_chunk ? c->min_chunk : c->chunk_images;
        nchunk = B / want;
        if (nchunk < nstream) nchunk = nstream;
    }
    const int per = (B + nchunk - 1) / nchunk;
    nchunk = (B + per - 1) / per;
    HIPE(hipEventRecord(c->ev_fork, st));
    for (int k = 1; k < nstream; ++k) HIPE(hipStreamWaitEvent(c->aux[k - 1], c->ev_fork, 0));
    c->co_running = nstream;
    for (int k = 0; k < nchunk; ++k) {
        const int i0 = k * per;
        const int n = (i0 + per <= B) ? per : (B - i0);
        const int sid = k % nstream;
        hipStream_t s = (sid == 0) ? st : c->aux[sid - 1];
        const hipError_t ec = encoder_chunk(c, images, i0, n, features, ldfeat, s, sid, true);
        if (ec != hipSuccess) {
            c->co_running = 1;
            return ec;
        }
    }
    c->co_running = 1;
    for (int k = 1; k < nstream; ++k) {
        HIPE(hipEventRecord(c->ev_join[k - 1], c->aux[k - 1]));
        HIPE(hipStreamWaitEvent(st, c->ev_join[k - 1], 0));
    }
    return hipSuccess;
}

hipError_t regress_impl(hpe_ctx* c, const float* th_prev, float* th_next, int B, hipStream_t st) {
    HIPE(run_dense(c, th_prev, THETA_LD, B, THETA_LD, c->w1t, 1024, 1024, c->ones, c->b1, c->P1, 1024, 1, c->H1, 1024, st));
    HIPE(run_dense(c, c->H1, 1024, B, 1024, c->w2, 1024, 1024, c->ones, c->b2, nullptr, 0, 1, c->H2, 1024, st));
    return run_dense(c, c->H2, 1024, B, 1024, c->w3, 128, HPE_THETA_DIM, c->ones, c->b3, th_prev, THETA_LD, 0, th_next, THETA_LD, st);
}

hipError_t features_proj(hpe_ctx* c, const float* features, int B, hipStream_t st) {
    return run_dense(c, features, HPE_FEATURE_DIM, B, HPE_FEATURE_DIM, c->w1f, 1024, 1024, c->ones, c->zeros, nullptr, 0, 0, c->P1,
                     1024, st);
}

enum { NEED_ENC = 1, NEED_REG = 2, NEED_SMPL = 4 };

int check_ready(hpe_ctx* c, int B, int need) {
    if (!c) return fail(HPE_ERR_INVALID, "null ctx");
    if (c->dead) return fail(HPE_ERR_STATE, "hpe_finalize failed on this ctx: destroy it and create a new one");
    if (!c->finalized) return fail(HPE_ERR_STATE, "hpe_finalize() has not been called");
    if (B < 1 || B > c->cfg.max_batch) return fail(HPE_ERR_INVALID, "batch " + std::to_string(B) + " outside [1, max_batch]");
    if ((need & NEED_ENC) && !c->have_encoder) return fail(HPE_ERR_STATE, "encoder weights were not loaded before hpe_finalize");
    if ((need & NEED_REG) && !c->have_regressor) return fail(HPE_ERR_STATE, "regressor weights / mean theta were not loaded");
    if ((need & NEED_SMPL) && !c->have_smpl) return fail(HPE_ERR_STATE, "SMPL model was not loaded before hpe_finalize");
    return HPE_OK;
}

}

#pragma GCC visibility push(default)
extern "C" {

static void release_device_state(hpe_ctx* c);

const char* hpe_last_error(void) { return g_err.c_str(); }
const char* hpe_version(void) { return "hpe_hip 0.1 (gfx950)"; }

const char* hpe_conv_layer_name(int idx) { return (idx >= 0 && idx < HPE_NUM_CONV) ? specs()[idx].name : nullptr; }
const char* hpe_bn_layer_name(int idx) { return (idx >= 0 && idx < HPE_NUM_CONV) ? specs()[idx].bn : nullptr; }

int hpe_conv_layer_geometry(int idx, int out[7]) {
    if (idx < 0 || idx >= HPE_NUM_CONV || !out) return fail(HPE_ERR_INVALID, "bad conv index");
    const ConvSpec& s = specs()[idx];
    out[0] = s.kh;
    out[1] = s.kw;
    out[2] = s.cin;
    out[3] = s.cout;
    out[4] = s.stride;
    out[5] = s.hin;
    out[6] = s.hout;
    return HPE_OK;
}

void hpe_config_init(HpeConfig* cfg) {
    if (!cfg) return;
    cfg->struct_size = (int)sizeof(HpeConfig);
    cfg->device = 0;
    cfg->max_batch = 8;
    cfg->num_stage = 3;
    cfg->bn_eps = 1e-3f;
    cfg->encoder_dtype = 0;
    cfg->n_streams = cfg->dual_gemm = cfg->stem_fused = cfg->wino_min_c = cfg->wino_min_items = cfg->wino_fused = -1;
    cfg->wino_fused_min_hw = cfg->mesh_a2b = cfg->wino_f4 = cfg->wino4_fused = cfg->bf16_p8 = cfg->wino4_ksplit = cfg->chain_fuse = cfg->halo3 = -1;
}

int hpe_create(const HpeConfig* cfg, hpe_ctx** out) {
    if (!cfg || !out) return fail(HPE_ERR_INVALID, "null argument");
    if (cfg->struct_size != (int)sizeof(HpeConfig))
        return fail(HPE_ERR_INVALID, "HpeConfig.struct_size is " + std::to_string(cfg->struct_size) + ", this library expects " +
                                         std::to_string(sizeof(HpeConfig)) + ": fill the struct with hpe_config_init() of the same header");
    if (cfg->n_streams > 4 || cfg->n_streams == 0) return fail(HPE_ERR_INVALID, "n_streams must be -1 (default) or 1..4");
    if (cfg->mesh_a2b > 2) return fail(HPE_ERR_INVALID, "mesh_a2b must be -1 (default), 0 (grid), 1 (valu) or 2 (mfma)");
    if (cfg->max_batch < 1 || cfg->max_batch > 1024) return fail(HPE_ERR_INVALID, "max_batch must be in [1,1024]");
    if (cfg->num_stage < 1 || cfg->num_stage > 16) return fail(HPE_ERR_INVALID, "num_stage must be in [1,16]");
    if (cfg->encoder_dtype != 0 && cfg->encoder_dtype != 1) return fail(HPE_ERR_INVALID, "encoder_dtype must be 0 (fp32) or 1 (bf16)");
    int ndev = 0;
    if (hipGetDeviceCount(&ndev) != hipSuccess || ndev < 1) return fail(HPE_ERR_NO_DEVICE, "no HIP device visible");
    if (cfg->device < 0 || cfg->device >= ndev) return fail(HPE_ERR_INVALID, "device ordinal out of range");
    hipDeviceProp_t prop;
    HIP_TRY(hipGetDeviceProperties(&prop, cfg->device));
    if (strncmp(prop.gcnArchName, "gfx950", 6) != 0)
        return fail(HPE_ERR_NO_DEVICE, std::string("device is ") + prop.gcnArchName + ", kernels are built for gfx950 only");
    hpe_ctx* c = new hpe_ctx();
    c->cfg = *cfg;
    c->bf16 = cfg->encoder_dtype == 1;
    if (c->cfg.bn_eps <= 0.f) c->cfg.bn_eps = 1e-3f;
    *out = c;
    return HPE_OK;
}

int hpe_destroy(hpe_ctx* c) {
    if (!c) return HPE_OK;
    DeviceGuard g(c->cfg.device);
    (void)hipDeviceSynchronize();
    release_device_state(c);
    delete c;
    return HPE_OK;
}

int hpe_load_smpl(hpe_ctx* c, const HpeSmplModel* m) {
    if (!c || !m) return fail(HPE_ERR_INVALID, "null argument");
    if (c->finalized) return fail(HPE_ERR_STATE, "already finalized");
    if (!m->v_template || !m->shapedirs || !m->posedirs || !m->J_regressor || !m->weights || !m->kp_regressor || !m->parents)
        return fail(HPE_ERR_INVALID, "null SMPL array");
    if (m->num_kp < 1 || m->num_kp > HPE_MAX_KP) return fail(HPE_ERR_INVALID, "num_kp must be in [1,24]");
    if (m->parents[0] >= 0) return fail(HPE_ERR_INVALID, "parents[0] must be negative (root)");
    for (int i = 1; i < 24; ++i)
        if (m->parents[i] < 0 || m->parents[i] >= i) return fail(HPE_ERR_INVALID, "parents[i] must satisfy 0 <= parents[i] < i");
    const int V = HPE_NUM_VERTS;
    c->h_vt.assign(m->v_template, m->v_template + V * 3);
    c->h_sd.assign(m->shapedirs, m->shapedirs + (size_t)V * 3 * 10);
    c->h_pd.assign(m->posedirs, m->posedirs + (size_t)V * 3 * 207);
    c->h_jreg.assign(m->J_regressor, m->J_regressor + (size_t)24 * V);
    c->h_w.assign(m->weights, m->weights + (size_t)V * 24);
    c->h_kreg.assign(m->kp_regressor, m->kp_regressor + (size_t)m->num_kp * V);
    c->h_par.assign(m->parents, m->parents + 24);
    c->num_kp = m->num_kp;
    c->smpl_loaded = true;
    return HPE_OK;
}

int hpe_load_conv(hpe_ctx* c, int idx, const float* kernel, const float* bias, const float* gamma, const float* beta,
                  const float* mean, const float* var) {
    if (!c || idx < 0 || idx >= HPE_NUM_CONV) return fail(HPE_ERR_INVALID, "bad conv index");
    if (c->finalized) return fail(HPE_ERR_STATE, "already finalized");
    if (!kernel || !bias || !gamma || !beta || !mean || !var) return fail(HPE_ERR_INVALID, "null conv array");
    const ConvSpec& s = specs()[idx];
    ConvLayer& L = c->conv[idx];
    L.kernel.assign(kernel, kernel + (size_t)s.kh * s.kw * s.cin * s.cout);
    L.bias.assign(bias, bias + s.cout);
    L.gamma.assign(gamma, gamma + s.cout);
    L.beta.assign(beta, beta + s.cout);
    L.mean.assign(mean, mean + s.cout);
    L.var.assign(var, var + s.cout);
    L.loaded = true;
    return HPE_OK;
}

int hpe_load_dense(hpe_ctx* c, int idx, const float* kernel, const float* bias) {
    if (!c || idx < 0 || idx >= HPE_NUM_DENSE) return fail(HPE_ERR_INVALID, "bad dense index");
    if (c->finalized) return fail(HPE_ERR_STATE, "already finalized");
    if (!kernel || !bias) return fail(HPE_ERR_INVALID, "null dense array");
    const int din[3] = {2133, 1024, 1024}, dout[3] = {1024, 1024, 85};
    c->dense[idx].kernel.assign(kernel, kernel + (size_t)din[idx] * dout[idx]);
    c->dense[idx].bias.assign(bias, bias + dout[idx]);
    c->dense[idx].loaded = true;
    return HPE_OK;
}

int hpe_load_mean_theta(hpe_ctx* c, const float* mean85) {
    if (!c || !mean85) return fail(HPE_ERR_INVALID, "null argument");
    if (c->finalized) return fail(HPE_ERR_STATE, "already finalized");
    memcpy(c->h_mean, mean85, sizeof(float) * HPE_THETA_DIM);
    c->mean_loaded = true;
    return HPE_OK;
}

static int finalize_impl(hpe_ctx* c);

static void release_device_state(hpe_ctx* c) {
    for (void* p : c->allocs) (void)hipFree(p);
    c->allocs.clear();
    for (auto& a : c->aux)
        if (a) {
            (void)hipStreamDestroy(a);
            a = nullptr;
        }
    auto kill = [](hipEvent_t& e) {
        if (e) {
            (void)hipEventDestroy(e);
            e = nullptr;
        }
    };
    kill(c->ev_fork);
    kill(c->ev_enc);
    kill(c->ev_tail);
    for (auto& e : c->ev_feat_free) kill(e);
    if (c->tail_st) {
        (void)hipStreamDestroy(c->tail_st);
        c->tail_st = nullptr;
    }
    for (auto& e : c->ev_join) kill(e);
    for (auto& e : c->ev) kill(e);
    for (auto& e : c->span0) kill(e);
    for (auto& e : c->span1) kill(e);
    for (auto& e : c->cev0) kill(e);
    for (auto& e : c->cev1) kill(e);
    for (auto& e : c->lev0) kill(e);
    for (auto& e : c->lev1) kill(e);
    for (auto& e : c->lev_all) kill(e);
    c->ev_ok = false;
}

int hpe_finalize(hpe_ctx* c) {
    if (!c) return fail(HPE_ERR_INVALID, "null ctx");
    if (c->dead) return fail(HPE_ERR_STATE, "an earlier hpe_finalize failed: destroy this ctx and create a new one");
    if (c->finalized) return fail(HPE_ERR_STATE, "already finalized");
    const int rc = finalize_impl(c);
    if (rc != HPE_OK && rc != HPE_ERR_STATE) {
        const std::string keep = g_err;
        DeviceGuard g(c->cfg.device);
        (void)hipDeviceSynchronize();
        release_device_state(c);
        c->dead = true;
        g_err = keep;
    }
    return rc;
}

static int finalize_impl(hpe_ctx* c) {
    {
        int nconv = 0, ndense = 0;
        for (int i = 0; i < HPE_NUM_CONV; ++i) nconv += c->conv[i].loaded ? 1 : 0;
        for (int i = 0; i < HPE_NUM_DENSE; ++i) ndense += c->dense[i].loaded ? 1 : 0;
        if (nconv != 0 && nconv != HPE_NUM_CONV) {
            for (int i = 0; i < HPE_NUM_CONV; ++i)
                if (!c->conv[i].loaded) return fail(HPE_ERR_STATE, std::string("conv layer not loaded: ") + specs()[i].name);
        }
        if (ndense != 0 && (ndense != HPE_NUM_DENSE || !c->mean_loaded))
            return fail(HPE_ERR_STATE, "regressor needs all 3 dense layers and the mean theta");
        c->have_encoder = nconv == HPE_NUM_CONV;
        c->have_regressor = ndense == HPE_NUM_DENSE && c->mean_loaded;
        c->have_smpl = c->smpl_loaded;
        if (!c->have_encoder && !c->have_regressor && !c->have_smpl) return fail(HPE_ERR_STATE, "nothing was loaded");
    }
    DeviceGuard g(c->cfg.device);
    int rc;
    {
        auto opt = [](int cfg_val, const char* env, int dflt) {
            if (cfg_val >= 0) return cfg_val;
            const char* v = getenv(env);
            return v ? atoi(v) : dflt;
        };
        c->wino_min_c = opt(c->cfg.wino_min_c, "HPE_WINO_MINC", 128);
        c->wino_min_items = opt(c->cfg.wino_min_items, "HPE_WINO_MIN_ITEMS", 128);
        c->wino_fused = opt(c->cfg.wino_fused, "HPE_WINO_FUSED", 1) && c->wino_min_c > 0;
        c->wino_fused_min_hw = opt(c->cfg.wino_fused_min_hw, "HPE_WINO_FUSED_MINHW", 28);
        c->stem_fused = opt(c->cfg.stem_fused, "HPE_STEM_FUSED", 1);
        c->dual_gemm = opt(c->cfg.dual_gemm, "HPE_DUAL", 1);
        c->wino_f4 = c->wino_min_c > 0 ? opt(c->cfg.wino_f4, "HPE_WINO_F4", 7) : 0;
        c->wino4_min_items = opt(-1, "HPE_WINO4_MIN_ITEMS", c->wino4_min_items);
        c->wino4_ksplit = opt(c->cfg.wino4_ksplit, "HPE_WINO4_KSPLIT", 1);
        c->chain_fuse = c->bf16 ? (opt(c->cfg.chain_fuse, "HPE_CHAIN", 7) & 23) : (opt(c->cfg.chain_fuse, "HPE_CHAIN", 8) & 8);
        c->halo3 = c->bf16 ? (opt(c->cfg.halo3, "HPE_HALO3", 15) & 15) : 0;
        c->halo3_two = opt(-1, "HPE_HALO3_TWO", 4) & 7;
        c->wino4_fused = c->wino_min_c > 0 ? (opt(c->cfg.wino4_fused, "HPE_WINO4_FUSED", 0) & 12) : 0;
        const char* e;
        e = getenv("HPE_CONCURRENT_TILES");
        c->knobs.concurrent_tiles = e ? atoi(e) : 0;
        e = getenv("HPE_BF16_128_MIN_TILES");
        if (e) c->knobs.bf16_128_min_tiles = atoi(e);
        e = getenv("HPE_WIDE128_MIN_TILES");
        if (e) c->knobs.wide128_min_tiles = atoi(e);
        e = getenv("HPE_TILE_WIDE");
        c->knobs.force_wide = e ? atoi(e) : -1;
        e = getenv("HPE_TILE_NARROW");
        c->knobs.force_narrow = e ? atoi(e) : -1;
        e = getenv("HPE_SHORTK_TILE");
        c->knobs.shortk = e ? atoi(e) : TILE_128x64_W8;
        e = getenv("HPE_TILE_BF16");
        c->knobs.force_bf16 = e ? atoi(e) : -1;
        e = getenv("HPE_EXPAND_TILE");
        c->knobs.force_expand = e ? atoi(e) : -1;
        e = getenv("HPE_EXPAND_SMALL_GRID");
        if (e) c->knobs.expand_small_grid = atoi(e);
        e = getenv("HPE_BF16_W8_MIN_TILES");
        if (e) c->knobs.bf16_w8_min_tiles = atoi(e);
        e = getenv("HPE_NS_BF16");
        c->knobs.force_ns_bf16 = e ? atoi(e) : -1;
        e = getenv("HPE_BF16_RULES");
        c->knobs.bf16_rules = e ? atoi(e) : 1;
        c->knobs.bf16_p8 = opt(c->cfg.bf16_p8, "HPE_BF16_P8", c->knobs.bf16_p8);
        e = getenv("HPE_BF16_P8_MINN");
        if (e) c->knobs.bf16_p8_min_n = atoi(e);
        e = getenv("HPE_BF16_P8_MINK");
        if (e) c->knobs.bf16_p8_min_k = atoi(e);
        HIP_TRY(hpe_wino_init_device());
        HIP_TRY(hpe_wino4_init_device());
        HIP_TRY(hpe_stem_fused_init_device());
        HIP_TRY(hpe_losses_init_device());
        c->mesh_a2b = c->cfg.mesh_a2b >= 0 ? c->cfg.mesh_a2b : hpe_mesh_a2b_mode_from_env();
        c->loss_attr_done = true;
    }
    if (c->have_encoder && c->dual_gemm) {
        int ci = 1;
        const int nblk[4] = {3, 4, 6, 3};
        for (int stg = 0; stg < 4; ++stg) {
            const int i2c = ci + 2, i1 = ci + 3;
            const ConvSpec& s2 = specs()[i2c];
            const ConvSpec& s1 = specs()[i1];
            ConvLayer& L2 = c->conv[i2c];
            const ConvLayer& L1 = c->conv[i1];
            const int K1 = s2.cin, K2 = s1.cin, N = s2.cout;
            const int slab = c->bf16 ? 64 : 32;
            if (K1 % slab == 0 && K2 % slab == 0) {
                const int n_pad = round_up(N, 128), K = K1 + K2;
                std::vector<float> wt((size_t)n_pad * K, 0.f), sh(N);
                for (int n = 0; n < N; ++n) {
                    const double inv2 = (double)L2.gamma[n] / std::sqrt((double)L2.var[n] + (double)c->cfg.bn_eps);
                    const double inv1 = (double)L1.gamma[n] / std::sqrt((double)L1.var[n] + (double)c->cfg.bn_eps);
                    for (int k = 0; k < K1; ++k) wt[(size_t)n * K + k] = (float)(inv2 * (double)L2.kernel[(size_t)k * N + n]);
                    for (int k = 0; k < K2; ++k) wt[(size_t)n * K + K1 + k] = (float)(inv1 * (double)L1.kernel[(size_t)k * N + n]);
                    sh[n] = (float)((((double)L2.bias[n] - (double)L2.mean[n]) * inv2 + (double)L2.beta[n]) +
                                    (((double)L1.bias[n] - (double)L1.mean[n]) * inv1 + (double)L1.beta[n]));
                }
                if (c->bf16) {
                    std::vector<unsigned short> wb(wt.size());
                    for (size_t q = 0; q < wt.size(); ++q) wb[q] = f2bf(wt[q]);
                    void* qd = nullptr;
                    HIP_TRY(hipMalloc(&qd, wb.size() * 2));
                    c->allocs.push_back(qd);
                    HIP_TRY(hipMemcpy(qd, wb.data(), wb.size() * 2, hipMemcpyHostToDevice));
                    L2.w_dual = static_cast<float*>(qd);
                } else {
                    if ((rc = upload(c, &L2.w_dual, wt))) return rc;
                }
                if ((rc = upload(c, &L2.shift_dual, sh))) return rc;
                L2.k_dual = K;
                L2.k1_dual = K1;
            }
            ci += 4 + 3 * (nblk[stg] - 1);
        }
    }
    for (int i = 0; c->have_encoder && i < HPE_NUM_CONV; ++i) {
        const ConvSpec& s = specs()[i];
        ConvLayer& L = c->conv[i];
        L.n_pad = round_up(s.cout, 128);
        if (c->bf16) {
            L.k_pad = (i == 0) ? 4 * 64 : round_up(s.kh * s.kw * s.cin, 64);
            std::vector<unsigned short> wt((size_t)L.n_pad * L.k_pad, 0);
            for (int kh = 0; kh < s.kh; ++kh)
                for (int kw = 0; kw < s.kw; ++kw)
                    for (int ci = 0; ci < s.cin; ++ci) {
                        const int k = (i == 0) ? (kh * 32 + kw * 4 + ci) : ((kh * s.kw + kw) * s.cin + ci);
                        const float* src = &L.kernel[(((size_t)kh * s.kw + kw) * s.cin + ci) * s.cout];
                        for (int n = 0; n < s.cout; ++n) wt[(size_t)n * L.k_pad + k] = f2bf(src[n]);
                    }
            void* q = nullptr;
            HIP_TRY(hipMalloc(&q, wt.size() * 2));
            c->allocs.push_back(q);
            HIP_TRY(hipMemcpy(q, wt.data(), wt.size() * 2, hipMemcpyHostToDevice));
            L.w = static_cast<float*>(q);
        } else {
        L.k_pad = (i == 0) ? 7 * 32 : round_up(s.kh * s.kw * s.cin, 32);
        std::vector<float> wt((size_t)L.n_pad * L.k_pad, 0.f);
        for (int kh = 0; kh < s.kh; ++kh)
            for (int kw = 0; kw < s.kw; ++kw)
                for (int ci = 0; ci < s.cin; ++ci) {
                    const int k = (i == 0) ? (kh * 32 + kw * 4 + ci) : ((kh * s.kw + kw) * s.cin + ci);
                    const float* src = &L.kernel[(((size_t)kh * s.kw + kw) * s.cin + ci) * s.cout];
                    for (int n = 0; n < s.cout; ++n) wt[(size_t)n * L.k_pad + k] = src[n];
                }
        if ((rc = upload(c, &L.w, wt))) return rc;
        if (c->wino_min_c > 0 && s.kh == 3 && s.stride == 1 && s.cin % 32 == 0 && s.cout % 64 == 0 &&
            (s.cin >= c->wino_min_c || (c->wino_fused && s.hin >= c->wino_fused_min_hw))) {
            static const double G[4][3] = {{1, 0, 0}, {0.5, 0.5, 0.5}, {0.5, -0.5, 0.5}, {0, 0, 1}};
            const int S = s.cin / 8;
            std::vector<float> U((size_t)16 * s.cin * s.cout);
            for (int ci = 0; ci < s.cin; ++ci)
                for (int n = 0; n < s.cout; ++n) {
                    double g[3][3];
                    for (int a = 0; a < 3; ++a)
                        for (int b = 0; b < 3; ++b) g[a][b] = L.kernel[(((size_t)a * 3 + b) * s.cin + ci) * s.cout + n];
                    const size_t base = ((((size_t)(n >> 6) * S + (ci >> 3)) * 16) * 2 + ((ci >> 2) & 1)) * 256 + (size_t)(n & 63) * 4 + (ci & 3);
                    for (int xi = 0; xi < 4; ++xi)
                        for (int nu = 0; nu < 4; ++nu) {
                            double u = 0.0;
                            for (int a = 0; a < 3; ++a)
                                for (int b = 0; b < 3; ++b) u += G[xi][a] * G[nu][b] * g[a][b];
                            U[base + (size_t)(xi * 4 + nu) * 512] = (float)u;
                        }
                }
            if ((rc = upload(c, &L.wino_u, U))) return rc;
        }
        if (s.kh == 3 && s.stride == 1 && s.cin % 32 == 0 && s.cout % 64 == 0 && ((c->wino_f4 | c->wino4_fused) & f4_bit(s.hin))) {
            static const double G4[6][3] = {{0.25, 0, 0}, {-1.0 / 6, -1.0 / 6, -1.0 / 6}, {-1.0 / 6, 1.0 / 6, -1.0 / 6},
                                            {1.0 / 24, 1.0 / 12, 1.0 / 6}, {1.0 / 24, -1.0 / 12, 1.0 / 6}, {0, 0, 1}};
            const int S4 = s.cin / 4;
            std::vector<float> U((size_t)36 * s.cin * s.cout);
            for (int ci = 0; ci < s.cin; ++ci)
                for (int n = 0; n < s.cout; ++n) {
                    double g[3][3];
                    for (int a = 0; a < 3; ++a)
                        for (int b = 0; b < 3; ++b) g[a][b] = L.kernel[(((size_t)a * 3 + b) * s.cin + ci) * s.cout + n];
                    const size_t base = (((size_t)(n >> 6) * S4 + (ci >> 2)) * 36) * 256 + (size_t)(n & 63) * 4 + (ci & 3);
                    for (int xi = 0; xi < 6; ++xi)
                        for (int nu = 0; nu < 6; ++nu) {
                            double u = 0.0;
                            for (int a = 0; a < 3; ++a)
                                for (int b = 0; b < 3; ++b) u += G4[xi][a] * G4[nu][b] * g[a][b];
                            U[base + (size_t)(xi * 6 + nu) * 256] = (float)u;
                        }
                }
            if ((rc = upload(c, &L.wino4_u, U))) return rc;
        }
        }
        if (i == 0) {
            void* q = nullptr;
            if (c->bf16) {
                std::vector<unsigned short> wp((size_t)64 * 7 * 32, 0);
                for (int kh = 0; kh < 7; ++kh)
                    for (int kw = 0; kw < 7; ++kw)
                        for (int ci = 0; ci < 3; ++ci)
                            for (int n = 0; n < 64; ++n)
                                wp[((size_t)n * 7 + kh) * 32 + kw * 4 + ci] = f2bf(L.kernel[(((size_t)kh * 7 + kw) * 3 + ci) * 64 + n]);
                HIP_TRY(hipMalloc(&q, wp.size() * 2));
                c->allocs.push_back(q);
                HIP_TRY(hipMemcpy(q, wp.data(), wp.size() * 2, hipMemcpyHostToDevice));
            } else {
                std::vector<float> wp((size_t)64 * 160, 0.f);
                for (int kh = 0; kh < 7; ++kh)
                    for (int kw = 0; kw < 7; ++kw)
                        for (int ci = 0; ci < 3; ++ci)
                            for (int n = 0; n < 64; ++n)
                                wp[(size_t)n * 160 + kh * 22 + 1 + kw * 3 + ci] = L.kernel[(((size_t)kh * 7 + kw) * 3 + ci) * 64 + n];
                HIP_TRY(hipMalloc(&q, wp.size() * 4));
                c->allocs.push_back(q);
                HIP_TRY(hipMemcpy(q, wp.data(), wp.size() * 4, hipMemcpyHostToDevice));
            }
            L.stem_w = q;
        }
        std::vector<float> sc(s.cout), sh(s.cout);
        for (int n = 0; n < s.cout; ++n) {
            const double inv = (double)L.gamma[n] / std::sqrt((double)L.var[n] + (double)c->cfg.bn_eps);
            sc[n] = (float)inv;
            sh[n] = (float)(((double)L.bias[n] - (double)L.mean[n]) * inv + (double)L.beta[n]);
        }
        if ((rc = upload(c, &L.scale, sc))) return rc;
        if ((rc = upload(c, &L.shift, sh))) return rc;
        std::vector<float>().swap(L.kernel);
    }
    if ((rc = upload(c, &c->ones, std::vector<float>(2048, 1.f)))) return rc;
    if ((rc = upload(c, &c->zeros, std::vector<float>(1024, 0.f)))) return rc;
    if (c->have_regressor) {
        const std::vector<float>& k1 = c->dense[0].kernel;
        std::vector<float> w1f((size_t)1024 * 2048), w1t((size_t)1024 * THETA_LD, 0.f);
        for (int n = 0; n < 1024; ++n) {
            for (int k = 0; k < 2048; ++k) w1f[(size_t)n * 2048 + k] = k1[(size_t)k * 1024 + n];
            for (int k = 0; k < HPE_THETA_DIM; ++k) w1t[(size_t)n * THETA_LD + k] = k1[(size_t)(2048 + k) * 1024 + n];
        }
        const std::vector<float>& k2 = c->dense[1].kernel;
        std::vector<float> w2((size_t)1024 * 1024);
        for (int n = 0; n < 1024; ++n)
            for (int k = 0; k < 1024; ++k) w2[(size_t)n * 1024 + k] = k2[(size_t)k * 1024 + n];
        const std::vector<float>& k3 = c->dense[2].kernel;
        std::vector<float> w3((size_t)128 * 1024, 0.f);
        for (int n = 0; n < HPE_THETA_DIM; ++n)
            for (int k = 0; k < 1024; ++k) w3[(size_t)n * 1024 + k] = k3[(size_t)k * HPE_THETA_DIM + n];
        if ((rc = upload(c, &c->w1f, w1f))) return rc;
        if ((rc = upload(c, &c->w1t, w1t))) return rc;
        if ((rc = upload(c, &c->w2, w2))) return rc;
        if ((rc = upload(c, &c->w3, w3))) return rc;
        if ((rc = upload(c, &c->b1, c->dense[0].bias))) return rc;
        if ((rc = upload(c, &c->b2, c->dense[1].bias))) return rc;
        std::vector<float> b3(128, 0.f);
        for (int n = 0; n < HPE_THETA_DIM; ++n) b3[n] = c->dense[2].bias[n];
        if ((rc = upload(c, &c->b3, b3))) return rc;
        if ((rc = upload(c, &c->mean_dev, std::vector<float>(c->h_mean, c->h_mean + HPE_THETA_DIM)))) return rc;
    }
    if (c->have_smpl) {
        const int V = HPE_NUM_VERTS, V3 = V * 3;
        std::vector<float> src((size_t)11 * V3);
        memcpy(src.data(), c->h_vt.data(), sizeof(float) * V3);
        for (int i = 0; i < V3; ++i)
            for (int k = 0; k < 10; ++k) src[(size_t)(1 + k) * V3 + i] = c->h_sd[(size_t)i * 10 + k];
        if ((rc = upload(c, &c->smpl_basis_src, src))) return rc;
        c->smpl.v_template = c->smpl_basis_src;
        c->smpl.shapedirs = c->smpl_basis_src + V3;
        std::vector<float> pd((size_t)207 * V3);
        for (int i = 0; i < V3; ++i)
            for (int k = 0; k < 207; ++k) pd[(size_t)k * V3 + i] = c->h_pd[(size_t)i * 207 + k];
        float* p = nullptr;
        if ((rc = upload(c, &p, pd))) return rc;
        c->smpl.posedirs = p;
        if ((rc = upload(c, &p, c->h_w))) return rc;
        c->smpl.weights = p;
        std::vector<float> jr((size_t)V * SMPL_KP_PITCH, 0.f), kr((size_t)V * SMPL_KP_PITCH, 0.f);
        for (int j = 0; j < 24; ++j)
            for (int v = 0; v < V; ++v) jr[(size_t)v * SMPL_KP_PITCH + j] = c->h_jreg[(size_t)j * V + v];
        for (int j = 0; j < c->num_kp; ++j)
            for (int v = 0; v < V; ++v) kr[(size_t)v * SMPL_KP_PITCH + j] = c->h_kreg[(size_t)j * V + v];
        if ((rc = upload(c, &p, jr))) return rc;
        c->smpl.j_reg = p;
        if ((rc = upload(c, &p, kr))) return rc;
        c->smpl.kp_reg = p;
        int depth[24], maxd = 0;
        for (int j = 0; j < 24; ++j) {
            depth[j] = c->h_par[j] < 0 ? 0 : depth[c->h_par[j]] + 1;
            if (depth[j] > maxd) maxd = depth[j];
        }
        void* ip = nullptr;
        HIP_TRY(hipMalloc(&ip, sizeof(int) * 48));
        c->allocs.push_back(ip);
        HIP_TRY(hipMemcpy(ip, c->h_par.data(), sizeof(int) * 24, hipMemcpyHostToDevice));
        HIP_TRY(hipMemcpy(static_cast<int*>(ip) + 24, depth, sizeof(int) * 24, hipMemcpyHostToDevice));
        c->smpl.parents = static_cast<int*>(ip);
        c->smpl.depth = static_cast<int*>(ip) + 24;
        c->smpl.max_depth = maxd;
        c->smpl.num_kp = c->num_kp;
        float* jb = nullptr;
        if ((rc = dev_alloc(c, &jb, 11 * 24 * 3, true))) return rc;
        HIP_TRY(hpe_launch_joint_regress(c->smpl_basis_src, c->smpl.j_reg, 11, 24, jb, nullptr, nullptr, nullptr));
        HIP_TRY(hipDeviceSynchronize());
        c->smpl.j_basis = jb;
    }
    {
        const size_t B = (size_t)c->cfg.max_batch;
        const size_t Bpad = (size_t)round_up(c->cfg.max_batch, SMPL_IMG_TILE);
        if (c->have_encoder) {
            if ((rc = dev_alloc(c, &c->padded, B * STEM_HP * STEM_WP * 4 + 64, true))) return rc;
            if ((rc = dev_alloc(c, &c->X0, B * 802816, false))) return rc;
            if ((rc = dev_alloc(c, &c->X1, B * 802816, false))) return rc;
            if ((rc = dev_alloc(c, &c->SC, B * 802816, false))) return rc;
            if ((rc = dev_alloc(c, &c->T1, B * 200704, false))) return rc;
            if ((rc = dev_alloc(c, &c->T2, B * 200704, false))) return rc;
            if ((rc = dev_alloc(c, &c->feat, B * HPE_FEATURE_DIM, true))) return rc;
            if ((rc = dev_alloc(c, &c->feat_alt, B * HPE_FEATURE_DIM, true))) return rc;
        }
        if (c->have_encoder && !c->bf16 && c->wino_min_c > 0) {
            if ((rc = dev_alloc(c, &c->wino_v, B * WINO_V_PITCH + WINO_V_SLACK, false))) return rc;
            if (c->wino_f4 && c->wino4_ksplit) {
                const size_t nws = hpe_wino4_split_ws_floats();
                if ((rc = dev_alloc(c, &c->w4_split, 4 * nws, false))) return rc;
                for (int k = 0; k < 4; ++k) HIP_TRY(hipMemset(c->w4_split + (k + 1) * nws - 256, 0, 256 * sizeof(unsigned)));
            }
            const char* e = getenv("HPE_WINO_STREAMK");
            if (e && atoi(e) != 0) {
                hipDeviceProp_t prop;
                HIP_TRY(hipGetDeviceProperties(&prop, c->cfg.device));
                c->n_cu = prop.multiProcessorCount;
                if ((rc = dev_alloc(c, &c->wino_ws, (size_t)4 * c->n_cu * HPE_WINO_WS_FLOATS, false))) return rc;
                float* fl = nullptr;
                if ((rc = dev_alloc(c, &fl, (size_t)4 * c->n_cu + 4, true))) return rc;
                c->wino_flags = reinterpret_cast<unsigned*>(fl);
                c->dev_err = c->wino_flags + (size_t)4 * c->n_cu;
            }
        }
        {
            c->partial_floats = (size_t)512 * 128 * 128;
            if ((rc = dev_alloc(c, &c->partial, c->partial_floats, false))) return rc;
            c->partial_tail_floats = (size_t)64 * 128 * 128;
            if ((rc = dev_alloc(c, &c->partial_tail, c->partial_tail_floats, false))) return rc;
        }
        if (c->have_regressor) {
            if ((rc = dev_alloc(c, &c->P1, B * 1024, true))) return rc;
            if ((rc = dev_alloc(c, &c->H1, B * 1024, true))) return rc;
            if ((rc = dev_alloc(c, &c->H2, B * 1024, true))) return rc;
            if ((rc = dev_alloc(c, &c->thA, B * THETA_LD, true))) return rc;
            if ((rc = dev_alloc(c, &c->thB, B * THETA_LD, true))) return rc;
        }
        if (c->have_smpl) {
            if ((rc = dev_alloc(c, &c->work.pfT, 207 * Bpad, true))) return rc;
            if ((rc = dev_alloc(c, &c->work.betaT, 10 * Bpad, true))) return rc;
            if ((rc = dev_alloc(c, &c->work.A, Bpad * 288, true))) return rc;
            if ((rc = dev_alloc(c, &c->work.cams, Bpad * 4, true))) return rc;
            if ((rc = dev_alloc(c, &c->work.verts_tmp, B * HPE_NUM_VERTS * 3, false))) return rc;
            if ((rc = dev_alloc(c, &c->work.kp_part, (size_t)SMPL_SMALL_B * ((HPE_NUM_VERTS + 63) / 64) * 72, true))) return rc;
            c->loss_ws_floats = hpe_mesh_loss_ws_floats(c->cfg.max_batch, HPE_IMG_SIZE, HPE_IMG_SIZE, HPE_NUM_VERTS);
            if ((rc = dev_alloc(c, &c->loss_ws, c->loss_ws_floats, true))) return rc;
        }
        c->work.Bpad = (int)Bpad;
    }
    {
        const char* e = getenv("HPE_STREAMS");
        int ns = c->cfg.n_streams > 0 ? c->cfg.n_streams : (e ? atoi(e) : 2);
        if (ns < 1) ns = 1;
        if (ns > 4) ns = 4;
        c->n_streams = ns;
        c->min_chunk = c->bf16 ? 24 : 32;
        e = getenv("HPE_MIN_CHUNK");
        if (e && atoi(e) >= 8) c->min_chunk = atoi(e);
        e = getenv("HPE_CHUNK");
        c->chunk_images = e ? atoi(e) : 0;
        for (int i = 0; i < ns - 1; ++i) HIP_TRY(hipStreamCreateWithFlags(&c->aux[i], hipStreamNonBlocking));
        HIP_TRY(hipEventCreateWithFlags(&c->ev_fork, hipEventDisableTiming));
        HIP_TRY(hipStreamCreateWithFlags(&c->tail_st, hipStreamNonBlocking));
        HIP_TRY(hipEventCreateWithFlags(&c->ev_enc, hipEventDisableTiming));
        HIP_TRY(hipEventCreateWithFlags(&c->ev_tail, hipEventDisableTiming));
        for (auto& ev : c->ev_feat_free) HIP_TRY(hipEventCreateWithFlags(&ev, hipEventDisableTiming));
        for (auto& ev : c->ev_join) HIP_TRY(hipEventCreateWithFlags(&ev, hipEventDisableTiming));
    }
    for (auto& e : c->ev) HIP_TRY(hipEventCreate(&e));
    for (auto& e : c->span0) HIP_TRY(hipEventCreate(&e));
    for (auto& e : c->span1) HIP_TRY(hipEventCreate(&e));
    for (auto& e : c->cev0) HIP_TRY(hipEventCreate(&e));
    for (auto& e : c->cev1) HIP_TRY(hipEventCreate(&e));
    for (auto& e : c->lev0) HIP_TRY(hipEventCreate(&e));
    for (auto& e : c->lev1) HIP_TRY(hipEventCreate(&e));
    for (auto& e : c->lev_all) HIP_TRY(hipEventCreate(&e));
    c->ev_ok = true;
    HIP_TRY(hipDeviceSynchronize());
    c->finalized = true;
    return HPE_OK;
}

int hpe_encoder(hpe_ctx* c, const float* images, int B, float* features, void* stream) {
    int rc = check_ready(c, B, NEED_ENC);
    if (rc) return rc;
    if (!images || !features) return fail(HPE_ERR_INVALID, "null pointer");
    DeviceGuard g(c->cfg.device);
    hipStream_t st = static_cast<hipStream_t>(stream);
    if (c->timing) {
        HIP_TRY(hipEventRecord(c->ev[0], st));
        HIP_TRY(hipEventRecord(c->span0[c->span_n % hpe_ctx::SPAN_RING], st));
    }
    HIP_TRY(encoder_impl(c, images, B, features, HPE_FEATURE_DIM, st));
    if (c->timing) {
        HIP_TRY(hipEventRecord(c->span1[c->span_n % hpe_ctx::SPAN_RING], st));
        ++c->span_n;
        HIP_TRY(hipEventRecord(c->ev[1], st));
        HIP_TRY(hipEventRecord(c->ev[4], st));
        c->timed_valid = true;
        c->conv_timed_valid = c->timing >= 2;
    }
    return HPE_OK;
}

int hpe_regress_stage(hpe_ctx* c, const float* features, const float* theta_prev, int B, float* theta_out, void* stream) {
    int rc = check_ready(c, B, NEED_REG);
    if (rc) return rc;
    if (!features || !theta_out) return fail(HPE_ERR_INVALID, "null pointer");
    DeviceGuard g(c->cfg.device);
    hipStream_t st = static_cast<hipStream_t>(stream);
    if (c->tail_pending) {
        HIP_TRY(hipStreamWaitEvent(st, c->ev_tail, 0));
        c->tail_pending = false;
    }
    HIP_TRY(features_proj(c, features, B, st));
    if (theta_prev)
        HIP_TRY(hpe_launch_copy_theta(theta_prev, HPE_THETA_DIM, c->thA, THETA_LD, B, HPE_THETA_DIM, st));
    else
        HIP_TRY(hpe_launch_tile_theta(c->mean_dev, c->thA, B, THETA_LD, st));
    HIP_TRY(regress_impl(c, c->thA, c->thB, B, st));
    HIP_TRY(hpe_launch_copy_theta(c->thB, THETA_LD, theta_out, HPE_THETA_DIM, B, HPE_THETA_DIM, st));
    return HPE_OK;
}

int hpe_smpl(hpe_ctx* c, const float* theta, int B, const HpeOutputs* outs, void* stream) {
    int rc = check_ready(c, B, NEED_SMPL);
    if (rc) return rc;
    if (!theta || !outs) return fail(HPE_ERR_INVALID, "null pointer");
    DeviceGuard g(c->cfg.device);
    if (c->tail_pending) {
        HIP_TRY(hipStreamWaitEvent(static_cast<hipStream_t>(stream), c->ev_tail, 0));
        c->tail_pending = false;
    }
    HIP_TRY(hpe_launch_smpl(c->smpl, c->work, theta, HPE_THETA_DIM, B, outs, static_cast<hipStream_t>(stream)));
    return HPE_OK;
}

static hipError_t tail_impl(hpe_ctx* c, const float* feat, int B, const HpeOutputs* stage_outs, int n_outs, hipStream_t ts, hipEvent_t feat_free) {
    hipError_t e = features_proj(c, feat, B, ts);
    if (e == hipSuccess && feat_free) e = hipEventRecord(feat_free, ts);
    if (e == hipSuccess) e = hpe_launch_tile_theta(c->mean_dev, c->thA, B, THETA_LD, ts);
    float* prev = c->thA;
    float* next = c->thB;
// ... 685 lines not shown
```

human-pose-estimation_amd/csrc/hpe_internal.h:

```cpp
#pragma once
#include <hip/hip_runtime.h>
#include <stddef.h>

enum GemmMode { GEMM_DENSE = 0, GEMM_STRIDED = 1, GEMM_CONV3 = 2, GEMM_STEM = 3, GEMM_DUAL = 4 };
enum GemmTile { TILE_128x128 = 0, TILE_128x64 = 1, TILE_64x64 = 2, TILE_64x128 = 3, TILE_128x128_W8 = 4, TILE_128x64_W8 = 5, TILE_256x128_W8 = 6,
                TILE_P8_256x256 = 7  };

struct GemmArgs {
    const float* x;
    const float* w;
    const float* scale;
    const float* shift;
    const float* res;
    float* y;
    int M, N, K;
    int lda, ldw, ldy, ldres, w_rows;
    int relu;
    int Hi, Wi, Cin, Ho, Wo, stride, cin_slabs;
    int n_mtiles, n_ntiles;
    int split_k;
    float* partial;
    size_t partial_floats;
    const float* zero;
    unsigned long long* dbg;
    const float* x2;
    int k1_slabs;
    int res_prefetch;
    int y_slab8;
};

hipError_t hpe_launch_gemm(GemmArgs p, int mode, int tile, hipStream_t st);

size_t hpe_wino_v_floats(int B, int H, int W, int C);
hipError_t hpe_wino_init_device();
#define HPE_WINO_WS_FLOATS 65536
struct WinoStreamK {
    float* ws;
    unsigned* flags;
    unsigned epoch;
    int n_wg;
    unsigned* err;
};
hipError_t hpe_launch_wino_conv3(const float* x, int lda, const float* U, const float* scale, const float* shift, float* y, int ldy,
                                 int B, int H, int W, int C, int N, int relu, float* V, const WinoStreamK* sk, hipStream_t st);

hipError_t hpe_launch_wino_fused_conv3(const float* xs, const float* U, const float* scale, const float* shift, const float* zero16, float* y,
                                       int ldy, int B, int H, int W, int C, int N, int relu, hipStream_t st);
int hpe_wino_fused_items(int B, int H, int W, int N);
hipError_t hpe_launch_nhwc_to_slab8(const float* x, float* xs, long M, int C, hipStream_t st);

size_t hpe_wino4_v_floats(int B, int H, int W, int C);
int hpe_wino4_items(int B, int H, int W, int N);
hipError_t hpe_wino4_init_device();
hipError_t hpe_launch_wino4_conv3(const float* x, int lda, const float* U, const float* scale, const float* shift, float* y, int ldy, int B,
                                  int H, int W, int C, int N, int relu, float* V, hipStream_t st, int co_running = 1, float* split_ws = nullptr);
size_t hpe_wino4_split_ws_floats();

hipError_t hpe_launch_wino4_fused_conv3(const float* xs, const float* U, const float* scale, const float* shift, const float* zero16, float* y,
                                        int ldy, int B, int H, int W, int C, int N, int relu, hipStream_t st);
int hpe_wino4_fused_items(int B, int H, int W, int N);

hipError_t hpe_launch_gemm_bf16(GemmArgs p, int mode, int tile, int ring_depth, hipStream_t st);
hipError_t hpe_launch_gemm_bf16_p8(GemmArgs p, int mode, hipStream_t st);
struct ChainArgs {
    const __bf16* t2;
    const __bf16* res;
    const __bf16* x2;
    const __bf16* w2c;
    const __bf16* w2a;
    const float *scaleA, *shiftA;
    const float *scaleB, *shiftB;
    __bf16* t3;
    __bf16* u1;
    int M, ldw2c, ldw2a;
};
struct Halo3Args {
    const __bf16* x;
    const __bf16* w;
    const float* scale;
    const float* shift;
    __bf16* y;
    int M, N, ldw, relu;
    int n_ntiles;
    int two;
};
bool hpe_halo3_bf16_supported(int HW, int Cin, int N);
hipError_t hpe_launch_halo3_bf16(const Halo3Args& p, int HW, int Cin, hipStream_t st);

bool hpe_chain_bf16_supported(int C, int C4, int CP, int C2);
hipError_t hpe_launch_chain_bf16(const ChainArgs& p, int C, int C4, int CP, int C2, hipStream_t st);
hipError_t hpe_chain_bf16_occupancy(int out[3]);
struct ChainArgsF32 {
    const float *t2, *res, *w2c, *w2a, *scaleA, *shiftA, *scaleB, *shiftB;
    float *t3, *u1;
    int M, ldw2c, ldw2a, u1_slab8;
};
bool hpe_chain_f32_supported(int C, int C4, int CP);
hipError_t hpe_launch_chain_f32(const ChainArgsF32& p, int C, int C4, int CP, hipStream_t st);
hipError_t hpe_chain_f32_occupancy(int* out);
hipError_t hpe_launch_f32_to_bf16(const float* x, void* y, long n, hipStream_t st);
hipError_t hpe_launch_bf16_to_f32(const void* x, float* y, long n, hipStream_t st);
hipError_t hpe_launch_pad_input_bf16(const float* img, void* out, int B, int H, int W, int Hp, int Wp, hipStream_t st);
hipError_t hpe_launch_maxpool_bf16(const void* x, void* y, int B, int H, int C, hipStream_t st);
hipError_t hpe_launch_avgpool_bf16(const void* x, float* y, int B, int HW, int C, int ldy, hipStream_t st);

hipError_t hpe_launch_stem_fused(const float* img, const void* w, const float* scale, const float* shift, void* y, int B, int R, int bf16,
                                 hipStream_t st);
hipError_t hpe_stem_fused_init_device();
int hpe_stem_fused_pick_rows(int B);

hipError_t hpe_launch_pad_input(const float* img, float* out, int B, int H, int W, int Hp, int Wp, hipStream_t st);
hipError_t hpe_launch_maxpool(const float* x, float* y, int B, int H, int C, hipStream_t st);
hipError_t hpe_launch_avgpool(const float* x, float* y, int B, int HW, int C, int ldy, hipStream_t st);
hipError_t hpe_launch_dense_gemv(const float* x, int lda, int M, int K, const float* wt, int N, const float* scale, const float* shift, const float* res,
                                 int ldres, int relu, float* y, int ldy, hipStream_t st);
hipError_t hpe_launch_tile_theta(const float* mean85, float* theta, int B, int ld, hipStream_t st);
hipError_t hpe_launch_copy_theta(const float* src, int lds, float* dst, int ldd, int B, int n, hipStream_t st);

struct SmplDev {
    const float* v_template;
    const float* shapedirs;
    const float* posedirs;
    const float* weights;
    const float* kp_reg;
    const float* j_reg;
    const float* j_basis;
    const int* parents;
    const int* depth;
    int num_kp;
    int max_depth;
};
#define SMPL_V 6890
#define SMPL_KP_PITCH 24
#define SMPL_IMG_TILE 8
#define SMPL_SMALL_B 8

struct SmplWork {
    float* pfT;
    float* betaT;
    float* A;
    float* cams;
    float* verts_tmp;
    float* kp_part;
    int Bpad;
};

struct HpeOutputs;
hipError_t hpe_launch_smpl(const SmplDev& d, const SmplWork& w, const float* theta, int ldtheta, int B, const HpeOutputs* o,
                           hipStream_t st);
hipError_t hpe_launch_joint_regress(const float* X, const float* reg, int n, int K, float* out, const float* cams,
                                    float* kp2d, hipStream_t st);
hipError_t hpe_launch_orth_proj(const float* X, const float* cam, int B, int P, float sx, float sy, int pixels, float* out,
                                hipStream_t st);

hipError_t hpe_launch_kp_loss(const float* gt, const float* pred, int n, float* out, hipStream_t st);
hipError_t hpe_losses_init_device();
size_t hpe_mesh_loss_ws_floats(int B, int H, int W, int P);
int hpe_mesh_a2b_mode_from_env();
hipError_t hpe_launch_mesh_loss(const float* seg, const float* v2d, int B, int H, int W, int P, float* ws, float* out,
                                hipStream_t st, int a2b_mode, unsigned long long* counter);
hipError_t hpe_launch_mesh_loss_prepare(const float* seg, int B, int H, int W, int P, float* ws, hipStream_t st);
hipError_t hpe_launch_mesh_loss_search(const float* v2d, int B, int H, int W, int P, float* ws, float* out, hipStream_t st,
                                       hipEvent_t ev_a2b0, hipEvent_t ev_a2b1, int a2b_mode, unsigned long long* counter);

hipError_t hpe_launch_preprocess_u8(const unsigned char* img, int H, int W, int C, int newH, int newW, int start_x, int start_y,
                                    int margin, float* out, int S, hipStream_t st);
struct PreprocFrame {
    long long offset;
    int H, W, newH, newW, start_x, start_y;
};
hipError_t hpe_launch_preprocess_u8_batch(const unsigned char* img, const PreprocFrame* table_dev, PreprocFrame uni, int B, int C, int margin,
                                          float* out, int S, hipStream_t st);
hipError_t hpe_launch_shift_verts(const float* verts, const float* cam, int B, int P, float flength, float img_size, float* out,
                                  hipStream_t st);

struct RenderVert {
    int U, V;
    int valid;
    int pad;
    float iz;
    float r, g, b;
};
struct RenderArgs {
    const float* verts;
    const float* cam;
    const int* faces;
    const int* adj_off;
    const int* adj_face;
    RenderVert* rec;
    uint2* box;
    float* center;
    const unsigned char* bg;
    unsigned char* out;
    int* out_face;
    float* out_z;
    int B, P, Fn, H, W, C;
    int rotate;
    float R[9];
    float znear, zfar;
    float albedo[3];
    float light[9];
    float light_color[3];
};
hipError_t hpe_launch_render(const RenderArgs& a, int stage, hipStream_t st);
```

human-pose-estimation_amd/engine.py:

```python
from __future__ import annotations

import ctypes as C

import numpy as np

from . import _lib
from .resnet_spec import CONV_SPECS

NUM_VERTS = _lib.NUM_VERTS


def _torch():
    import torch

    return torch


def _require_cuda_tensor(t, name, shape_tail=None):
    torch = _torch()
    if not isinstance(t, torch.Tensor):
        raise TypeError("%s must be a torch.Tensor on the GPU" % name)
    if not t.is_cuda:
        raise ValueError("%s must live on the GPU (got %s); there is no CPU path" % (name, t.device))
    if t.dtype != torch.float32:
# ... 108 lines not shown
        return C.c_void_p(_torch().cuda.current_stream(self.tdev).cuda_stream)

    def _new(self, *shape):
        return _torch().empty(shape, dtype=_torch().float32, device=self.tdev)

    def _alloc_outputs(self, B, want):
        shapes = {
            "verts": (B, NUM_VERTS, 3),
            "joints": (B, self.num_kp, 3),
            "cams": (B, 3),
            "theta": (B, 85),
            "J_transformed": (B, 24, 3),
            "kp2d": (B, self.num_kp, 2),
            "verts2d": (B, NUM_VERTS, 2),
            "Rs": (B, 24, 3, 3),
        }
        tensors = {k: self._new(*shapes[k]) for k in want}
        o = _lib.HpeOutputs(*[tensors[k].data_ptr() if k in tensors else None for k in _lib.OUTPUT_FIELDS])
        return tensors, o

    DEFAULT_OUTPUTS = ("verts", "joints", "cams", "theta", "J_transformed", "kp2d")

    def forward(self, images, all_stages=False, want=DEFAULT_OUTPUTS, pipelined=False):
        images = _require_cuda_tensor(images, "images", (224, 224, 3))
        B = images.shape[0]
        n_outs = self.num_stage if all_stages else 1
        outs = []
        arr = (_lib.HpeOutputs * n_outs)()
        for i in range(n_outs):
            t, o = self._alloc_outputs(B, want)
            outs.append(t)
            arr[i] = o
        fwd = self.lib.hpe_forward_pipelined if pipelined else self.lib.hpe_forward
        if pipelined:
            ts = self.tail_stream()
            for t in outs:
                for v in t.values():
                    v.record_stream(ts)
        _lib.check(fwd(self._h, images.data_ptr(), B, arr, n_outs, self._stream()))
        return outs

    def tail(self, features, all_stages=False, want=DEFAULT_OUTPUTS):
        features = _require_cuda_tensor(features, "features", (2048,))
        B = features.shape[0]
        n_outs = self.num_stage if all_stages else 1
        outs = []
        arr = (_lib.HpeOutputs * n_outs)()
        for i in range(n_outs):
            t, o = self._alloc_outputs(B, want)
            outs.append(t)
            arr[i] = o
        _lib.check(self.lib.hpe_tail(self._h, features.data_ptr(), B, arr, n_outs, self._stream()))
        return outs

    def make_overlapped_plan(self, B, all_stages=False, want=DEFAULT_OUTPUTS, graph=False, tail_extra=None, n_sets=2):
        torch = _torch()
        n_outs = self.num_stage if all_stages else 1
        sets = []
        for _ in range(n_sets):
            outs, arr = [], (_lib.HpeOutputs * n_outs)()
            for i in range(n_outs):
                t, o = self._alloc_outputs(B, want)
                outs.append(t)
                arr[i] = o
            sets.append((outs, arr))
        feats = [self._new(B, 2048) for _ in range(2)]
        side = self.tail_stream()
        lib, h = self.lib, self._h
        state = {"k": 0}

        def enqueue(images, k, with_tail, with_enc):
            cur = torch.cuda.current_stream(self.tdev)
            if with_tail:
                side.wait_stream(cur)
                with torch.cuda.stream(side):
                    outs, arr = sets[(k - 1) % n_sets]
                    _lib.check(lib.hpe_tail(h, feats[(k - 1) & 1].data_ptr(), B, arr, n_outs, C.c_void_p(side.cuda_stream)))
                    if tail_extra is not None:
                        tail_extra(outs, (k - 1) % n_sets)
            if with_enc:
                _lib.check(lib.hpe_encoder(h, images.data_ptr(), B, feats[k & 1].data_ptr(), self._stream()))
            if with_tail:
                cur.wait_stream(side)

        if not graph:

            def step(images):
                k = state["k"]
                enqueue(images, k, k > 0, True)
                state["k"] = k + 1
                if k > 0:
                    step.last = (k - 1) % n_sets
                return sets[(k - 1) % n_sets][0] if k > 0 else None

            def flush():
                k = state["k"]
                if k == 0:
                    return None
                enqueue(None, k, True, False)
                state["k"] = 0
                step.last = (k - 1) % n_sets
                return sets[(k - 1) % n_sets][0]

            step.flush = flush
            step.last = None
            step.sets = [s_[0] for s_ in sets]
            return step

        static_in = torch.zeros((B, 224, 224, 3), dtype=torch.float32, device=self.tdev)
        self.enable_timing(0)
        enqueue(static_in, 0, False, True)
        enqueue(static_in, 1, True, True)
        enqueue(None, 2, True, False)
        torch.cuda.synchronize(self.tdev)
        period = 2 * n_sets // (2 if n_sets % 2 == 0 else 1)

        def capture(k, with_tail, with_enc):
            g = torch.cuda.CUDAGraph()
            with torch.cuda.graph(g):
                enqueue(static_in, k, with_tail, with_enc)
            return g

        g_first = capture(0, False, True)
        g_steady = [capture(period + r, True, True) for r in range(period)]
        g_flush = [capture(period + r, True, False) for r in range(period)]

        def step(images):
            k = state["k"]
            static_in.copy_(images, non_blocking=True)
            (g_first if k == 0 else g_steady[k % period]).replay()
            state["k"] = k + 1
            if k > 0:
                step.last = (k - 1) % n_sets
            return sets[(k - 1) % n_sets][0] if k > 0 else None

        def flush():
            k = state["k"]
            if k == 0:
                return None
            g_flush[k % period].replay()
            state["k"] = 0
            step.last = (k - 1) % n_sets
            return sets[(k - 1) % n_sets][0]

        step.flush = flush
        step.last = None
        step.sets = [s_[0] for s_ in sets]
        step.graphs = (g_first, g_steady, g_flush)
        return step

    def tail_stream(self):
        torch = _torch()
        ptr = self.lib.hpe_tail_stream(self._h)
        if not ptr:
            raise _lib.HpeError("no tail stream (ctx not finalized)")
        return torch.cuda.ExternalStream(ptr, device=self.tdev)

    def join(self):
        _lib.check(self.lib.hpe_join(self._h, self._stream()))

    def make_forward_plan(self, B, all_stages=False, want=DEFAULT_OUTPUTS, graph=False, pipelined=False):
        torch = _torch()
        n_outs = self.num_stage if all_stages else 1
        outs = []
        arr = (_lib.HpeOutputs * n_outs)()
        for i in range(n_outs):
            t, o = self._alloc_outputs(B, want)
            outs.append(t)
            arr[i] = o
        lib, h = self.lib, self._h
        fwd = lib.hpe_forward_pipelined if pipelined else lib.hpe_forward
        if pipelined and graph:
            raise ValueError("a pipelined plan cannot be captured into a graph")

        def launch(images):
            _lib.check(fwd(h, images.data_ptr(), B, arr, n_outs, self._stream()))

        if not graph:

            def run(images):
                launch(images)
                return outs

            return run, outs

        static_in = torch.zeros((B, 224, 224, 3), dtype=torch.float32, device=self.tdev)
        self.enable_timing(0)
        side = torch.cuda.Stream(device=self.tdev)
        side.wait_stream(torch.cuda.current_stream(self.tdev))
        with torch.cuda.stream(side):
            launch(static_in)
        torch.cuda.current_stream(self.tdev).wait_stream(side)
        torch.cuda.synchronize(self.tdev)
        g = torch.cuda.CUDAGraph()
        with torch.cuda.graph(g):
            launch(static_in)

        def run_graph(images):
            static_in.copy_(images, non_blocking=True)
            g.replay()
            return outs

        run_graph.graph = g
        return run_graph, outs

    def encoder(self, images):
        images = _require_cuda_tensor(images, "images", (224, 224, 3))
        feat = self._new(images.shape[0], 2048)
        _lib.check(self.lib.hpe_encoder(self._h, images.data_ptr(), images.shape[0], feat.data_ptr(), self._stream()))
        return feat

    def regress_stage(self, features, theta_prev=None):
        features = _require_cuda_tensor(features, "features", (2048,))
        B = features.shape[0]
        tp = None
        if theta_prev is not None:
            theta_prev = _require_cuda_tensor(theta_prev, "theta_prev", (85,))
            tp = theta_prev.data_ptr()
        out = self._new(B, 85)
        _lib.check(self.lib.hpe_regress_stage(self._h, features.data_ptr(), tp, B, out.data_ptr(), self._stream()))
        return out

    def smpl(self, theta, want=("verts", "joints", "J_transformed", "kp2d", "Rs")):
        theta = _require_cuda_tensor(theta, "theta", (85,))
        B = theta.shape[0]
        t, o = self._alloc_outputs(B, want)
        _lib.check(self.lib.hpe_smpl(self._h, theta.data_ptr(), B, C.byref(o), self._stream()))
        return t

    def mesh_loss(self, seg, verts2d):
        torch = _torch()
        seg = _require_cuda_tensor(seg, "seg")
        verts2d = _require_cuda_tensor(verts2d, "verts2d")
        B, H, W = seg.shape[0], seg.shape[1], seg.shape[2]
        P = verts2d.shape[1]
        out = torch.zeros(4, dtype=torch.float32, device=self.tdev)
        _lib.check(self.lib.hpe_mesh_loss(self._h, seg.data_ptr(), verts2d.data_ptr(), B, H, W, P, out.data_ptr(), self._stream()))
        return out[0]

    def val_losses(self, kp_gt, kp2d_stages, seg=None, verts2d_stages=None, out=None):
        torch = _torch()
        kp_gt = _require_cuda_tensor(kp_gt, "kp_gt")
        n = len(kp2d_stages)
        kp2d = [_require_cuda_tensor(t, "kp2d") for t in kp2d_stages]
        B, K = kp_gt.shape[0], kp_gt.shape[1]
        kp_ptrs = (C.c_void_p * n)(*[t.data_ptr() for t in kp2d])
        H = W = P = 0
        seg_ptr, v_ptrs, keep = None, None, None
        if seg is not None and verts2d_stages is not None:
            seg = _require_cuda_tensor(seg, "seg")
            keep = [_require_cuda_tensor(t, "verts2d") for t in verts2d_stages]
            if len(keep) != n or seg.shape[0] != B:
                raise ValueError("one verts2d tensor per stage and one silhouette per image are needed")
            H, W, P = seg.shape[1], seg.shape[2], keep[0].shape[1]
            seg_ptr = seg.data_ptr()
            v_ptrs = (C.c_void_p * n)(*[t.data_ptr() for t in keep])
        if out is None:
            out = torch.empty((n, 4), dtype=torch.float32, device=self.tdev)
        _lib.check(self.lib.hpe_val_losses(self._h, seg_ptr, kp_gt.data_ptr(), kp_ptrs, v_ptrs, n, B, K, H, W, P, out.data_ptr(), self._stream()))
        return out

    def check_device(self):
        _lib.check(self.lib.hpe_device_status(self._h, self._stream()))

    def debug_conv(self, idx, x, residual=None, relu=True):
        s = CONV_SPECS[idx]
        x = _require_cuda_tensor(x, "x")
        B = x.shape[0]
        y = self._new(B, s.hout, s.hout, s.cout)
        r = None
        if residual is not None:
            r = _require_cuda_tensor(residual, "residual").data_ptr()
        _lib.check(self.lib.hpe_debug_conv(self._h, idx, x.data_ptr(), B, r, int(relu), y.data_ptr(), self._stream()))
        return y

    def debug_chain(self, idx2c, t2, residual):
        s = CONV_SPECS[idx2c]
        first = CONV_SPECS[idx2c + 1].name.endswith("branch1")
        sn = CONV_SPECS[idx2c + (2 if first else 1)]
        t2 = _require_cuda_tensor(t2, "t2", (s.hin, s.hin, s.cin))
        residual = _require_cuda_tensor(residual, "residual", (s.hout, s.hout, CONV_SPECS[idx2c + 1].cin if first else s.cout))
        B = t2.shape[0]
        t3 = self._new(B, s.hout, s.hout, s.cout)
        u1 = self._new(B, sn.hout, sn.hout, sn.cout)
        occ = (C.c_int * 3)()
        _lib.check(self.lib.hpe_debug_chain(self._h, idx2c, t2.data_ptr(), residual.data_ptr(), B, t3.data_ptr(), u1.data_ptr(), occ, self._stream()))
        return t3, u1, (occ[0], occ[1], occ[2])

    def debug_stem(self, images, rows_per_strip=0):
        images = _require_cuda_tensor(images, "images", (224, 224, 3))
        y = self._new(images.shape[0], 56, 56, 64)
        _lib.check(self.lib.hpe_debug_stem(self._h, images.data_ptr(), images.shape[0], int(rows_per_strip), y.data_ptr(), self._stream()))
        return y

    def joint_regress(self, X, use_kp_regressor=True):
        X = _require_cuda_tensor(X, "X", (NUM_VERTS, 3))
        K = self.num_kp if use_kp_regressor else 24
        out = self._new(X.shape[0], K, 3)
        _lib.check(self.lib.hpe_debug_joint_regress(self._h, X.data_ptr(), X.shape[0], int(use_kp_regressor), out.data_ptr(), self._stream()))
        return out

    def encoder_kernel_description(self):
        if self.encoder_dtype == "fp32":
            return ("conv_gemm_f32_dma_kernel (the 1x1 / strided / dual-source layers) + w4_input_kernel + w4_gemm_kernel / w4_gemm32_kernel "
                    "(the 13 3x3 layers on the 28x28 / 14x14 / 7x7 maps as fp32 Winograd F(4x4,3x3); F(2x2,3x3) / direct below 64 work "
                    "items) + wino_fused_kernel (the three 56x56 3x3 layers, F(2x2,3x3)) + stem_fused_f32_kernel -- the 53 conv layers of one "
                    "step, priced at their direct-convolution FLOPs")
        return ("conv_gemm_bf16_dma_kernel (1x1 / strided / dual-source layers) + chain_expand_reduce_bf16_kernel (branch2c + next branch2a of "
                "stages 2-3 as one launch) + conv3_halo_bf16_kernel (the sixteen 3x3 layers, tile + halo resident in LDS) + stem_fused_bf16_kernel "
                "-- the 53 conv layers of one step, priced at their algorithmic HBM bytes")

    def enable_timing(self, level=1):
        _lib.check(self.lib.hpe_enable_timing(self._h, int(level)))

    def timings(self):
        ms = (C.c_float * 5)()
        _lib.check(self.lib.hpe_get_timings(self._h, ms))
        return dict(encoder_ms=ms[0], conv_ms=ms[1], regress_smpl_ms=ms[2], total_ms=ms[4])

    def span_stats(self):
        ms = (C.c_float * 3)()
        n = C.c_int()
        _lib.check(self.lib.hpe_get_span_stats(self._h, ms, C.byref(n)))
        return dict(mean_ms=ms[0], min_ms=ms[1], max_ms=ms[2], calls=n.value)

    def set_loss_counter(self, counter=None):
        _lib.check(self.lib.hpe_debug_set_loss_counter(self._h, None if counter is None else counter.data_ptr()))
        self._loss_counter = counter

    def loss_timings(self):
        ms = (C.c_float * 2)()
        _lib.check(self.lib.hpe_get_loss_timings(self._h, ms))
        return dict(val_losses_ms=ms[0], a2b_search_ms=ms[1])

    def conv_timings(self):
        ms = (C.c_float * _lib.NUM_CONV)()
        _lib.check(self.lib.hpe_get_conv_timings(self._h, ms))
        return list(ms)


def _cur_stream(t):
    return C.c_void_p(_torch().cuda.current_stream(t.device).cuda_stream)


def orth_proj(X, camera):
    X = _require_cuda_tensor(X, "X")
    camera = _require_cuda_tensor(camera, "camera").reshape(-1, 3)
    B, P = X.shape[0], X.shape[1]
    out = _torch().empty((B, P, 2), dtype=_torch().float32, device=X.device)
    with _torch().cuda.device(X.device):
        _lib.check(_lib.load().hpe_orth_proj(X.data_ptr(), camera.data_ptr(), B, P, out.data_ptr(), _cur_stream(X)))
    return out


def reproject(verts, cam, im_w, im_h):
    verts = _require_cuda_tensor(verts, "verts")
    cam = _require_cuda_tensor(cam, "cam").reshape(-1, 3)
    B, P = verts.shape[0], verts.shape[1]
    out = _torch().empty((B, P, 2), dtype=_torch().float32, device=verts.device)
    with _torch().cuda.device(verts.device):
        _lib.check(
            _lib.load().hpe_reproject_vertices(verts.data_ptr(), cam.data_ptr(), B, P, float(im_w), float(im_h), out.data_ptr(), _cur_stream(verts))
        )
    return out


def kp_loss_parts(kp_gt, kp_pred):
    kp_gt = _require_cuda_tensor(kp_gt, "kp_gt")
    kp_pred = _require_cuda_tensor(kp_pred, "kp_pred")
    B, K = kp_gt.shape[0], kp_gt.shape[1]
    out = _torch().zeros(4, dtype=_torch().float32, device=kp_gt.device)
    with _torch().cuda.device(kp_gt.device):
        _lib.check(_lib.load().hpe_kp_loss(kp_gt.data_ptr(), kp_pred.data_ptr(), B, K, out.data_ptr(), _cur_stream(kp_gt)))
    return out[:3]
```

include/hpe.h:

```cpp
#ifndef HPE_H_
#define HPE_H_

#ifdef __cplusplus
extern "C" {
#endif

#define HPE_OK 0
#define HPE_ERR_INVALID 1
#define HPE_ERR_HIP 2
#define HPE_ERR_STATE 3
#define HPE_ERR_NO_DEVICE 4

#define HPE_NUM_CONV 53
#define HPE_NUM_DENSE 3
#define HPE_NUM_VERTS 6890
#define HPE_NUM_JOINTS 24
#define HPE_NUM_BETAS 10
#define HPE_NUM_POSE_BASIS 207
#define HPE_THETA_DIM 85
#define HPE_FEATURE_DIM 2048
#define HPE_MAX_KP 24
#define HPE_IMG_SIZE 224

typedef struct hpe_ctx hpe_ctx;

typedef struct HpeConfig {
    int struct_size;
    int device;
    int max_batch;
    int num_stage;
    float bn_eps;
    int encoder_dtype;
    int n_streams;
    int dual_gemm;
    int stem_fused;
    int wino_min_c;
    int wino_min_items;
    int wino_fused;
    int wino_fused_min_hw;
    int mesh_a2b;
    int wino_f4;
    int wino4_fused;
    int bf16_p8;
    int wino4_ksplit;
    int chain_fuse;
    int halo3;
} HpeConfig;

void hpe_config_init(HpeConfig* cfg);

typedef struct HpeSmplModel {
    const float* v_template;
    const float* shapedirs;
    const float* posedirs;
    const float* J_regressor;
    const float* weights;
    const float* kp_regressor;
    const int* parents;
    int num_kp;
} HpeSmplModel;

typedef struct HpeOutputs {
    float* verts;
    float* joints;
    float* cams;
    float* theta;
    float* J_transformed;
    float* kp2d;
    float* verts2d;
    float* Rs;
} HpeOutputs;

const char* hpe_last_error(void);
const char* hpe_version(void);

const char* hpe_conv_layer_name(int idx);
const char* hpe_bn_layer_name(int idx);
int hpe_conv_layer_geometry(int idx, int out[7]);

int hpe_create(const HpeConfig* cfg, hpe_ctx** out);
int hpe_destroy(hpe_ctx* ctx);

int hpe_load_smpl(hpe_ctx* ctx, const HpeSmplModel* host_model);
int hpe_load_conv(hpe_ctx* ctx, int idx, const float* kernel_hwio, const float* bias, const float* gamma,
                  const float* beta, const float* moving_mean, const float* moving_variance);
int hpe_load_dense(hpe_ctx* ctx, int idx, const float* kernel_in_out, const float* bias);
int hpe_load_mean_theta(hpe_ctx* ctx, const float* mean85);
int hpe_finalize(hpe_ctx* ctx);

int hpe_forward(hpe_ctx* ctx, const float* images_dev, int B, const HpeOutputs* stage_outs, int n_outs, void* stream);

int hpe_forward_pipelined(hpe_ctx* ctx, const float* images_dev, int B, const HpeOutputs* stage_outs, int n_outs, void* stream);
int hpe_join(hpe_ctx* ctx, void* stream);
int hpe_tail(hpe_ctx* ctx, const float* features_dev, int B, const HpeOutputs* stage_outs, int n_outs, void* stream);
void* hpe_tail_stream(hpe_ctx* ctx);

int hpe_encoder(hpe_ctx* ctx, const float* images_dev, int B, float* features_dev, void* stream);
int hpe_regress_stage(hpe_ctx* ctx, const float* features_dev, const float* theta_prev_dev, int B, float* theta_out_dev,
                      void* stream);
int hpe_smpl(hpe_ctx* ctx, const float* theta_dev, int B, const HpeOutputs* outs, void* stream);
int hpe_orth_proj(const float* X_dev, const float* cam_dev, int B, int P, float* out_dev, void* stream);
int hpe_reproject_vertices(const float* verts_dev, const float* cam_dev, int B, int P, float im_w, float im_h, float* out_dev,
                           void* stream);
int hpe_kp_loss(const float* kp_gt_dev, const float* kp_pred_dev, int B, int K, float* out_dev, void* stream);
int hpe_mesh_loss(hpe_ctx* ctx, const float* seg_dev, const float* verts2d_dev, int B, int H, int W, int P, float* out_dev,
                  void* stream);

int hpe_val_losses(hpe_ctx* ctx, const float* seg_dev, const float* kp_gt_dev, const float* const* kp2d_dev,
                   const float* const* verts2d_dev, int n_stage, int B, int K, int H, int W, int P, float* out_dev, void* stream);

int hpe_preprocess_u8(const unsigned char* img_dev, int H, int W, int C, float* out224_dev, int proc_param[5], void* stream);
int hpe_preprocess_u8_batch(const unsigned char* frames_dev, const long long* offsets, const int* sizes_hw, int B, int C,
                            float* out_dev, int* proc_params, void* table_dev, void* stream);
int hpe_get_original(const float* verts_dev, const float* cam_dev, int B, int P, int K, const int start_pt[2], float scale,
                     int img_size, float* vert_shifted_dev, float cam_for_render[3], float* kp_original_host,
                     const float* joints2d_host, void* stream);

typedef struct hpe_renderer hpe_renderer;

typedef struct HpeRenderParams {
    int struct_size;
    int color_id;
    int do_alpha;
    int rot_axis;
    float rot_deg;
    float near;
    float far;
} HpeRenderParams;

void hpe_render_params_init(HpeRenderParams* p);
int hpe_renderer_create(int device, const int* faces_host, int Fn, int P, int max_batch, hpe_renderer** out);
int hpe_renderer_destroy(hpe_renderer* r);
int hpe_render(hpe_renderer* r, const float* verts_dev, const float* cam_dev, int B, int H, int W, const unsigned char* bg_dev,
               const HpeRenderParams* p, unsigned char* out_dev, void* stream);

int hpe_debug_render_ids(hpe_renderer* r, const float* verts_dev, const float* cam_dev, int B, int H, int W, const HpeRenderParams* p,
                         int* face_dev, float* z_dev, void* stream);
int hpe_debug_render_vertices(hpe_renderer* r, const float* verts_dev, const float* cam_dev, int B, int H, int W, const HpeRenderParams* p,
                              void* rec_dev, void* stream);

int hpe_debug_conv(hpe_ctx* ctx, int idx, const float* x_dev, int B, const float* residual_dev, int relu, float* y_dev,
                   void* stream);
int hpe_debug_chain(hpe_ctx* ctx, int idx2c, const float* t2_dev, const float* residual_dev, int B, float* t3_dev, float* u1_dev,
                    int* occupancy, void* stream);
int hpe_debug_stem(hpe_ctx* ctx, const float* images_dev, int B, int rows_per_strip, float* y_dev, void* stream);
int hpe_debug_gemm(hpe_ctx* ctx, const float* x_dev, const float* wt_dev, int M, int N, int K, int w_rows, int tile,
                   const float* residual_dev, int relu, float* y_dev, void* stream);
int hpe_debug_set_dbg(hpe_ctx* ctx, void* dbg_dev);
int hpe_debug_maxpool(const float* x_dev, int B, int H, int C, float* y_dev, void* stream);
int hpe_debug_avgpool(const float* x_dev, int B, int HW, int C, float* y_dev, void* stream);
int hpe_debug_joint_regress(hpe_ctx* ctx, const float* X_dev, int n, int use_kp_regressor, float* out_dev, void* stream);
int hpe_enable_timing(hpe_ctx* ctx, int level);
int hpe_device_status(hpe_ctx* ctx, void* stream);
int hpe_get_timings(hpe_ctx* ctx, float ms[5]);
int hpe_get_span_stats(hpe_ctx* ctx, float ms[3], int* n_calls);
int hpe_get_loss_timings(hpe_ctx* ctx, float ms[2]);
int hpe_debug_set_loss_counter(hpe_ctx* ctx, void* counter_dev);
int hpe_get_conv_timings(hpe_ctx* ctx, float* ms53);

#ifdef __cplusplus
}
#endif
#endif
```

Baseline: 18760 images/sec.

## Run fp32 1x1 conv GEMMs on bf16 matrix cores via three-piece split

Adds a kernel that splits the fp32 activations and weights into three bf16 pieces each and accumulates the cross products on the bf16 matrix cores, so fp32 1x1, strided and dual-source layers of stages 3-5 get bf16 MFMA throughput while staying close to fp32 accuracy. Weights are pre-split on the host at load time and stored as a 3xK layout. Activations are split inside the kernel. The shared GEMM helpers move into a common header. The cost is extra MFMA work per output (several bf16 products), extra weight memory and in-kernel conversion overhead. The path is selected by a size heuristic and is on by default when the encoder runs in fp32.

```diff
diff --git a/human-pose-estimation_amd/_lib.py b/human-pose-estimation_amd/_lib.py
--- a/human-pose-estimation_amd/_lib.py
+++ b/human-pose-estimation_amd/_lib.py
@@ -41,10 +41,11 @@
         ("wino4_ksplit", C.c_int),
         ("chain_fuse", C.c_int),
         ("halo3", C.c_int),
+        ("f32_split", C.c_int),
     ]
 
 
-PLAN_OPTIONS = ("n_streams", "dual_gemm", "stem_fused", "wino_min_c", "wino_min_items", "wino_fused", "wino_fused_min_hw", "mesh_a2b", "wino_f4", "wino4_fused", "bf16_p8", "wino4_ksplit", "chain_fuse", "halo3")
+PLAN_OPTIONS = ("n_streams", "dual_gemm", "stem_fused", "wino_min_c", "wino_min_items", "wino_fused", "wino_fused_min_hw", "mesh_a2b", "wino_f4", "wino4_fused", "bf16_p8", "wino4_ksplit", "chain_fuse", "halo3", "f32_split")
 
 
 class HpeSmplModel(C.Structure):
diff --git a/human-pose-estimation_amd/build.py b/human-pose-estimation_amd/build.py
--- a/human-pose-estimation_amd/build.py
+++ b/human-pose-estimation_amd/build.py
@@ -9,7 +9,7 @@
 CSRC = os.path.join(HERE, "csrc")
 LIBDIR = os.path.join(HERE, "lib")
 LIB = os.path.join(LIBDIR, "libhpe_hip.so")
-SOURCES = ["conv_gemm.hip", "conv_gemm_bf16.hip", "conv_gemm_bf16_p8.hip", "conv_chain_bf16.hip", "conv_chain_f32.hip", "conv3_halo_bf16.hip", "conv_wino.hip", "conv_wino4.hip", "stem_fused.hip", "encoder_ops.hip", "smpl.hip", "losses.hip", "prepost.hip", "render.hip", "hpe_api.hip"]
+SOURCES = ["conv_gemm.hip", "conv_gemm_f32s.hip", "conv_gemm_bf16.hip", "conv_gemm_bf16_p8.hip", "conv_chain_bf16.hip", "conv_chain_f32.hip", "conv3_halo_bf16.hip", "conv_wino.hip", "conv_wino4.hip", "stem_fused.hip", "encoder_ops.hip", "smpl.hip", "losses.hip", "prepost.hip", "render.hip", "hpe_api.hip"]
 CFLAGS = ["--offload-arch=gfx950", "-O3", "-std=c++17", "-fPIC", "-fvisibility=hidden", "-fno-fast-math"]
 
 
diff --git a/human-pose-estimation_amd/csrc/conv_gemm.hip b/human-pose-estimation_amd/csrc/conv_gemm.hip
--- a/human-pose-estimation_amd/csrc/conv_gemm.hip
+++ b/human-pose-estimation_amd/csrc/conv_gemm.hip
@@ -2,102 +2,12 @@
 #include <stdint.h>
 #include <stdlib.h>
 
+#include "conv_gemm_common.h"
 #include "hpe_internal.h"
 
-typedef float f32x16 __attribute__((ext_vector_type(16)));
-typedef float f32x4 __attribute__((ext_vector_type(4)));
-
-#define BK 32
 #define LDS_PITCH 36
 
 namespace {
-
-struct RowAddr {
-    int base;
-    unsigned mask;
-};
-
-template <int MODE>
-__device__ __forceinline__ RowAddr make_row(const GemmArgs& p, int m, int kc4) {
-    RowAddr r;
-    r.mask = 0x1ffu;
-    if (m >= p.M) m = p.M - 1;
-    if (MODE == GEMM_DENSE || MODE == GEMM_DUAL) {
-        r.base = m * p.lda + kc4;
-    } else {
-        const int hw = p.Ho * p.Wo;
-        const int b = m / hw;
-        const int rem = m - b * hw;
-        const int ho = rem / p.Wo;
-        const int wo = rem - ho * p.Wo;
-        if (MODE == GEMM_STRIDED) {
-            r.base = ((b * p.Hi + ho * p.stride) * p.Wi + wo * p.stride) * p.Cin + kc4;
-        } else if (MODE == GEMM_CONV3) {
-            r.base = ((b * p.Hi + ho) * p.Wi + wo) * p.Cin + kc4;
-            unsigned mk = 0;
-#pragma unroll
-            for (int tap = 0; tap < 9; ++tap) {
-                const int dh = tap / 3 - 1, dw = tap % 3 - 1;
-                if ((unsigned)(ho + dh) < (unsigned)p.Hi && (unsigned)(wo + dw) < (unsigned)p.Wi) mk |= 1u << tap;
-            }
-            r.mask = mk;
-        } else {
-            r.base = ((b * p.Hi + 2 * ho) * p.Wi + 2 * wo) * 4 + kc4;
-        }
-    }
-    return r;
-}
-
-struct SlabPos {
-    int off;
-    int tap;
-    int cs;
-};
-
-template <int MODE>
-__device__ __forceinline__ void slab_advance(const GemmArgs& p, SlabPos& sp) {
-    if (MODE == GEMM_DENSE || MODE == GEMM_STRIDED || MODE == GEMM_DUAL) {
-        sp.off += BK;
-    } else if (MODE == GEMM_CONV3) {
-        sp.cs += 1;
-        sp.off += BK;
-        if (sp.cs == p.cin_slabs) {
-            sp.cs = 0;
-            sp.tap += 1;
-            const int kh = sp.tap / 3;
-            sp.off = ((kh - 1) * p.Wi + (sp.tap - kh * 3 - 1)) * p.Cin;
-        }
-    } else {
-        sp.off += p.Wi * 4;
-    }
-}
-
-template <int MODE>
-__device__ __forceinline__ SlabPos slab_first(const GemmArgs& p) {
-    SlabPos sp;
-    sp.tap = 0;
-    sp.cs = 0;
-    sp.off = (MODE == GEMM_CONV3) ? (-p.Wi - 1) * p.Cin : 0;
-    return sp;
-}
-
-template <int MODE>
-__device__ __forceinline__ SlabPos slab_seek(const GemmArgs& p, int slab) {
-    SlabPos sp;
-    sp.tap = 0;
-    sp.cs = 0;
-    if (MODE == GEMM_DENSE || MODE == GEMM_STRIDED || MODE == GEMM_DUAL) {
-        sp.off = slab * BK;
-    } else if (MODE == GEMM_CONV3) {
-        sp.tap = slab / p.cin_slabs;
-        sp.cs = slab - sp.tap * p.cin_slabs;
-        const int kh = sp.tap / 3;
-        sp.off = ((kh - 1) * p.Wi + (sp.tap - kh * 3 - 1)) * p.Cin + sp.cs * BK;
-    } else {
-        sp.off = slab * p.Wi * 4;
-    }
-    return sp;
-}
 
 template <int MODE>
 __device__ __forceinline__ f32x4 load_a(const GemmArgs& p, const RowAddr& r, const SlabPos& sp) {
@@ -425,79 +335,6 @@
     }
 }
 
-#ifdef HPE_F32_RES_NT
-#define HPE_RES_LOAD(ptr) __builtin_nontemporal_load(ptr)
-#else
-#define HPE_RES_LOAD(ptr) (*(ptr))
-#endif
-template <int BM, int BN, int WM, int WN, int NP>
-__device__ __forceinline__ void conv_epilogue(const GemmArgs& p, float* lds, f32x16 (&acc)[BM / WM / 32][BN / WN / 32], int m0, int n0, int t,
-                                              int lane, int wm, int wn, const f32x4 (&rpre)[NP], bool use_pre) {
-    constexpr int MT = BM / WM / 32;
-    constexpr int NT = BN / WN / 32;
-    constexpr int NTHR = 64 * WM * WN;
-    constexpr int EP = BN + 4;
-    {
-        const int col_l = lane & 31;
-        const int row_l = 4 * (lane >> 5);
-#pragma unroll
-        for (int j = 0; j < NT; ++j) {
-            const int cl = (wn * NT + j) * 32 + col_l;
-            const int n = n0 + cl;
-            const bool n_ok = n < p.N;
-            const float sc = n_ok ? p.scale[n] : 0.f;
-            const float sh = n_ok ? p.shift[n] : 0.f;
-#pragma unroll
-            for (int i = 0; i < MT; ++i) {
-                const int rl = (wm * MT + i) * 32 + row_l;
-#pragma unroll
-                for (int e = 0; e < 16; ++e) lds[(rl + (e & 3) + 8 * (e >> 2)) * EP + cl] = acc[i][j][e] * sc + sh;
-            }
-        }
-    }
-    __syncthreads();
-    {
-        constexpr int TPR = BN / 4;
-        constexpr int RPP = NTHR / TPR;
-        const int r = t / TPR;
-        const int c4 = (t - r * TPR) * 4;
-        const int n = n0 + c4;
-        const bool full = (n + 3) < p.N;
-#pragma unroll
-        for (int pass = 0; pass < BM / RPP; ++pass) {
-            const int row = pass * RPP + r;
-            const int m = m0 + row;
-            if (m >= p.M || n >= p.N) continue;
-            f32x4 v = *reinterpret_cast<const f32x4*>(&lds[row * EP + c4]);
-            if (full) {
-                if (use_pre) v += rpre[pass < NP ? pass : 0];
-                else if (p.res) v += HPE_RES_LOAD(reinterpret_cast<const f32x4*>(p.res + (size_t)m * p.ldres + n));
-                if (p.relu) {
-                    v.x = fmaxf(v.x, 0.f);
-                    v.y = fmaxf(v.y, 0.f);
-                    v.z = fmaxf(v.z, 0.f);
-                    v.w = fmaxf(v.w, 0.f);
-                }
-                if (p.y_slab8)
-                    *reinterpret_cast<f32x4*>(p.y + ((size_t)(n >> 3) * p.M + m) * 8 + (n & 7)) = v;
-                else
-                    *reinterpret_cast<f32x4*>(p.y + (size_t)m * p.ldy + n) = v;
-            } else {
-                const float vv[4] = {v.x, v.y, v.z, v.w};
-#pragma unroll
-                for (int u = 0; u < 4; ++u) {
-                    if (n + u < p.N) {
-                        float o = vv[u];
-                        if (p.res) o += p.res[(size_t)m * p.ldres + n + u];
-                        if (p.relu) o = fmaxf(o, 0.f);
-                        p.y[(size_t)m * p.ldy + n + u] = o;
-                    }
-                }
-            }
-        }
-    }
-}
-
 template <int MODE, int BM, int BN, int WM, int WN>
 __global__ __launch_bounds__(64 * WM * WN, (WM * WN) / 2) void conv_gemm_f32_dma_kernel(GemmArgs p) {
     constexpr int MT = BM / WM / 32;
diff --git a/human-pose-estimation_amd/csrc/conv_gemm_common.h b/human-pose-estimation_amd/csrc/conv_gemm_common.h
--- /dev/null
+++ b/human-pose-estimation_amd/csrc/conv_gemm_common.h
@@ -0,0 +1,173 @@
+#pragma once
+#include <hip/hip_runtime.h>
+
+#include "hpe_internal.h"
+
+typedef float f32x16 __attribute__((ext_vector_type(16)));
+typedef float f32x4 __attribute__((ext_vector_type(4)));
+
+#define BK 32
+
+namespace {
+
+struct RowAddr {
+    int base;
+    unsigned mask;
+};
+
+template <int MODE>
+__device__ __forceinline__ RowAddr make_row(const GemmArgs& p, int m, int kc4) {
+    RowAddr r;
+    r.mask = 0x1ffu;
+    if (m >= p.M) m = p.M - 1;
+    if (MODE == GEMM_DENSE || MODE == GEMM_DUAL) {
+        r.base = m * p.lda + kc4;
+    } else {
+        const int hw = p.Ho * p.Wo;
+        const int b = m / hw;
+        const int rem = m - b * hw;
+        const int ho = rem / p.Wo;
+        const int wo = rem - ho * p.Wo;
+        if (MODE == GEMM_STRIDED) {
+            r.base = ((b * p.Hi + ho * p.stride) * p.Wi + wo * p.stride) * p.Cin + kc4;
+        } else if (MODE == GEMM_CONV3) {
+            r.base = ((b * p.Hi + ho) * p.Wi + wo) * p.Cin + kc4;
+            unsigned mk = 0;
+#pragma unroll
+            for (int tap = 0; tap < 9; ++tap) {
+                const int dh = tap / 3 - 1, dw = tap % 3 - 1;
+                if ((unsigned)(ho + dh) < (unsigned)p.Hi && (unsigned)(wo + dw) < (unsigned)p.Wi) mk |= 1u << tap;
+            }
+            r.mask = mk;
+        } else {
+            r.base = ((b * p.Hi + 2 * ho) * p.Wi + 2 * wo) * 4 + kc4;
+        }
+    }
+    return r;
+}
+
+struct SlabPos {
+    int off;
+    int tap;
+    int cs;
+};
+
+template <int MODE>
+__device__ __forceinline__ void slab_advance(const GemmArgs& p, SlabPos& sp) {
+    if (MODE == GEMM_DENSE || MODE == GEMM_STRIDED || MODE == GEMM_DUAL) {
+        sp.off += BK;
+    } else if (MODE == GEMM_CONV3) {
+        sp.cs += 1;
+        sp.off += BK;
+        if (sp.cs == p.cin_slabs) {
+            sp.cs = 0;
+            sp.tap += 1;
+            const int kh = sp.tap / 3;
+            sp.off = ((kh - 1) * p.Wi + (sp.tap - kh * 3 - 1)) * p.Cin;
+        }
+    } else {
+        sp.off += p.Wi * 4;
+    }
+}
+
+template <int MODE>
+__device__ __forceinline__ SlabPos slab_first(const GemmArgs& p) {
+    SlabPos sp;
+    sp.tap = 0;
+    sp.cs = 0;
+    sp.off = (MODE == GEMM_CONV3) ? (-p.Wi - 1) * p.Cin : 0;
+    return sp;
+}
+
+template <int MODE>
+__device__ __forceinline__ SlabPos slab_seek(const GemmArgs& p, int slab) {
+    SlabPos sp;
+    sp.tap = 0;
+    sp.cs = 0;
+    if (MODE == GEMM_DENSE || MODE == GEMM_STRIDED || MODE == GEMM_DUAL) {
+        sp.off = slab * BK;
+    } else if (MODE == GEMM_CONV3) {
+        sp.tap = slab / p.cin_slabs;
+        sp.cs = slab - sp.tap * p.cin_slabs;
+        const int kh = sp.tap / 3;
+        sp.off = ((kh - 1) * p.Wi + (sp.tap - kh * 3 - 1)) * p.Cin + sp.cs * BK;
+    } else {
+        sp.off = slab * p.Wi * 4;
+    }
+    return sp;
+}
+
+#ifdef HPE_F32_RES_NT
+#define HPE_RES_LOAD(ptr) __builtin_nontemporal_load(ptr)
+#else
+#define HPE_RES_LOAD(ptr) (*(ptr))
+#endif
+template <int BM, int BN, int WM, int WN, int NP>
+__device__ __forceinline__ void conv_epilogue(const GemmArgs& p, float* lds, f32x16 (&acc)[BM / WM / 32][BN / WN / 32], int m0, int n0, int t,
+                                              int lane, int wm, int wn, const f32x4 (&rpre)[NP], bool use_pre) {
+    constexpr int MT = BM / WM / 32;
+    constexpr int NT = BN / WN / 32;
+    constexpr int NTHR = 64 * WM * WN;
+    constexpr int EP = BN + 4;
+    {
+        const int col_l = lane & 31;
+        const int row_l = 4 * (lane >> 5);
+#pragma unroll
+        for (int j = 0; j < NT; ++j) {
+            const int cl = (wn * NT + j) * 32 + col_l;
+            const int n = n0 + cl;
+            const bool n_ok = n < p.N;
+            const float sc = n_ok ? p.scale[n] : 0.f;
+            const float sh = n_ok ? p.shift[n] : 0.f;
+#pragma unroll
+            for (int i = 0; i < MT; ++i) {
+                const int rl = (wm * MT + i) * 32 + row_l;
+#pragma unroll
+                for (int e = 0; e < 16; ++e) lds[(rl + (e & 3) + 8 * (e >> 2)) * EP + cl] = acc[i][j][e] * sc + sh;
+            }
+        }
+    }
+    __syncthreads();
+    {
+        constexpr int TPR = BN / 4;
+        constexpr int RPP = NTHR / TPR;
+        const int r = t / TPR;
+        const int c4 = (t - r * TPR) * 4;
+        const int n = n0 + c4;
+        const bool full = (n + 3) < p.N;
+#pragma unroll
+        for (int pass = 0; pass < BM / RPP; ++pass) {
+            const int row = pass * RPP + r;
+            const int m = m0 + row;
+            if (m >= p.M || n >= p.N) continue;
+            f32x4 v = *reinterpret_cast<const f32x4*>(&lds[row * EP + c4]);
+            if (full) {
+                if (use_pre) v += rpre[pass < NP ? pass : 0];
+                else if (p.res) v += HPE_RES_LOAD(reinterpret_cast<const f32x4*>(p.res + (size_t)m * p.ldres + n));
+                if (p.relu) {
+                    v.x = fmaxf(v.x, 0.f);
+                    v.y = fmaxf(v.y, 0.f);
+                    v.z = fmaxf(v.z, 0.f);
+                    v.w = fmaxf(v.w, 0.f);
+                }
+                if (p.y_slab8)
+                    *reinterpret_cast<f32x4*>(p.y + ((size_t)(n >> 3) * p.M + m) * 8 + (n & 7)) = v;
+                else
+                    *reinterpret_cast<f32x4*>(p.y + (size_t)m * p.ldy + n) = v;
+            } else {
+                const float vv[4] = {v.x, v.y, v.z, v.w};
+#pragma unroll
+                for (int u = 0; u < 4; ++u) {
+                    if (n + u < p.N) {
+                        float o = vv[u];
+                        if (p.res) o += p.res[(size_t)m * p.ldres + n + u];
+                        if (p.relu) o = fmaxf(o, 0.f);
+                        p.y[(size_t)m * p.ldy + n + u] = o;
+                    }
+                }
+            }
+        }
+    }
+}
+
+}
diff --git a/human-pose-estimation_amd/csrc/conv_gemm_f32s.hip b/human-pose-estimation_amd/csrc/conv_gemm_f32s.hip
--- /dev/null
+++ b/human-pose-estimation_amd/csrc/conv_gemm_f32s.hip
@@ -0,0 +1,240 @@
+#include <hip/hip_runtime.h>
+#include <stdint.h>
+#include <stdlib.h>
+
+#include "conv_gemm_common.h"
+#include "hpe_internal.h"
+
+namespace {
+
+typedef __bf16 bf16x8 __attribute__((ext_vector_type(8)));
+
+__device__ __forceinline__ void split3(const f32x4& lo, const f32x4& hi, bf16x8& h0, bf16x8& h1, bf16x8& h2) {
+#pragma unroll
+    for (int e = 0; e < 8; ++e) {
+        const float x = e < 4 ? lo[e] : hi[e - 4];
+        const __bf16 b0 = (__bf16)x;
+        const float r1 = x - (float)b0;
+        const __bf16 b1 = (__bf16)r1;
+        const float r2 = r1 - (float)b1;
+        h0[e] = b0;
+        h1[e] = b1;
+        h2[e] = (__bf16)r2;
+    }
+}
+
+template <int MODE, int BM, int BN, int WM, int WN>
+__global__ __launch_bounds__(64 * WM * WN, 2) void conv_gemm_f32s_dma_kernel(GemmArgs p) {
+    constexpr int MT = BM / WM / 32;
+    constexpr int NT = BN / WN / 32;
+    constexpr int NW = WM * WN;
+    constexpr int NTHR = 64 * NW;
+    constexpr int AP = BM / (8 * NW);
+    constexpr int BP = BN / (16 * NW);
+    constexpr int A_BYTES = BM * BK * 4;
+    constexpr int W_BYTES = BN * BK * 2;
+    constexpr int BUF = A_BYTES + 3 * W_BYTES;
+    constexpr int EPB = BM * (BN + 4) * 4;
+    constexpr int LDS_BYTES = (2 * BUF > EPB) ? 2 * BUF : EPB;
+    static_assert(NW == 4 || NW == 8, "4 or 8 waves per workgroup");
+    static_assert(AP >= 1 && BP >= 1, "tile too small for the wave count");
+    static_assert(MODE == GEMM_DENSE || MODE == GEMM_STRIDED || MODE == GEMM_DUAL, "1x1 layers only");
+
+    __shared__ __attribute__((aligned(16))) float lds[LDS_BYTES / 4];
+    char* const ldsb = reinterpret_cast<char*>(lds);
+
+    const int total = p.n_mtiles * p.n_ntiles;
+    const int bid = blockIdx.x;
+    const int xcd = bid & 7;
+    const int q8 = total >> 3, rr = total & 7;
+    const int tile = (xcd < rr ? xcd * (q8 + 1) : rr * (q8 + 1) + (xcd - rr) * q8) + (bid >> 3);
+    const int mtile = tile / p.n_ntiles;
+    const int ntile = tile - mtile * p.n_ntiles;
+    const int m0 = mtile * BM;
+    const int n0 = ntile * BN;
+
+    const int t = threadIdx.x;
+    const int lane = t & 63;
+    const int wave = __builtin_amdgcn_readfirstlane(t >> 6);
+    const int wm = wave / WN;
+    const int wn = wave - wm * WN;
+
+    RowAddr arow[AP];
+    int arow2[MODE == GEMM_DUAL ? AP : 1];
+#pragma unroll
+    for (int i = 0; i < AP; ++i) {
+        const int r = (NW * i + wave) * 8 + (lane >> 3);
+        const int lc = (lane & 7) ^ ((r >> 1) & 7);
+        arow[i] = make_row<MODE>(p, m0 + r, lc * 4);
+        if (MODE == GEMM_DUAL) arow2[i] = make_row<GEMM_STRIDED>(p, m0 + r, lc * 4).base;
+    }
+    const __bf16* const w16 = reinterpret_cast<const __bf16*>(p.w);
+    const __bf16* wsrc[BP];
+#pragma unroll
+    for (int i = 0; i < BP; ++i) {
+        const int r = (NW * i + wave) * 16 + (lane >> 2);
+        const int lc = (lane & 3) ^ ((r >> 2) & 3);
+        wsrc[i] = w16 + (size_t)(n0 + r) * p.ldw + lc * 8;
+    }
+
+    int a_row[MT], a_x[MT], b_row[NT], b_x[NT];
+#pragma unroll
+    for (int i = 0; i < MT; ++i) {
+        const int r = (wm * MT + i) * 32 + (lane & 31);
+        a_row[i] = r * (BK * 4);
+        a_x[i] = (r >> 1) & 7;
+    }
+#pragma unroll
+    for (int j = 0; j < NT; ++j) {
+        const int r = (wn * NT + j) * 32 + (lane & 31);
+        b_row[j] = A_BYTES + r * (BK * 2);
+        b_x[j] = (r >> 2) & 3;
+    }
+    const int hi = lane >> 5;
+
+    f32x16 acc[MT][NT], acx[MT][NT];
+#pragma unroll
+    for (int i = 0; i < MT; ++i)
+#pragma unroll
+        for (int j = 0; j < NT; ++j)
+#pragma unroll
+            for (int e = 0; e < 16; ++e) acc[i][j][e] = acx[i][j][e] = 0.f;
+
+    constexpr int R_TPR = BN / 4, R_RPP = NTHR / R_TPR, R_NPASS = BM / R_RPP;
+    constexpr bool R_PRE = (NW == 8) && R_NPASS <= 4;
+    f32x4 rpre[R_PRE ? R_NPASS : 1];
+    bool r_pre = false;
+    if constexpr (R_PRE) {
+        const int rr_ = t / R_TPR;
+        const int n = n0 + (t - rr_ * R_TPR) * 4;
+        r_pre = p.res != nullptr && p.res_prefetch && (n + 3) < p.N;
+        if (r_pre) {
+#pragma unroll
+            for (int pass = 0; pass < R_NPASS; ++pass) {
+                const int m = m0 + pass * R_RPP + rr_;
+                rpre[pass] = HPE_RES_LOAD(reinterpret_cast<const f32x4*>(p.res + (size_t)(m < p.M ? m : p.M - 1) * p.ldres + n));
+            }
+        }
+    }
+
+    auto issue_dma = [&](int slab, int buf) {
+#pragma unroll
+        for (int i = 0; i < AP; ++i) {
+            const float* src;
+            if (MODE == GEMM_DUAL)
+                src = slab < p.k1_slabs ? p.x + (arow[i].base + slab * BK) : p.x2 + (arow2[i] + (slab - p.k1_slabs) * BK);
+            else
+                src = p.x + (arow[i].base + slab * BK);
+            __builtin_amdgcn_global_load_lds((const __attribute__((address_space(1))) void*)src,
+                                             (__attribute__((address_space(3))) void*)(ldsb + buf + (NW * i + wave) * 1024), 16, 0, 0);
+        }
+#pragma unroll
+        for (int pc = 0; pc < 3; ++pc)
+#pragma unroll
+            for (int i = 0; i < BP; ++i)
+                __builtin_amdgcn_global_load_lds((const __attribute__((address_space(1))) void*)(wsrc[i] + (size_t)pc * p.w_piece + slab * BK),
+                                                 (__attribute__((address_space(3))) void*)(ldsb + buf + A_BYTES + pc * W_BYTES + (NW * i + wave) * 1024),
+                                                 16, 0, 0);
+    };
+
+    const int S = p.K / BK;
+    issue_dma(0, 0);
+    __builtin_amdgcn_s_waitcnt(0x0F70);
+    __syncthreads();
+
+    for (int s = 0; s < S; ++s) {
+        const int cur = (s & 1) * BUF;
+        if (s + 1 < S) issue_dma(s + 1, BUF - cur);
+#pragma unroll
+        for (int q = 0; q < 2; ++q) {
+            bf16x8 a0[MT], a1[MT], a2[MT], w0[NT], w1[NT], w2[NT];
+#pragma unroll
+            for (int i = 0; i < MT; ++i) {
+                const int lc = 4 * q + 2 * hi;
+                const f32x4 lo = *reinterpret_cast<const f32x4*>(ldsb + cur + a_row[i] + ((lc ^ a_x[i]) << 4));
+                const f32x4 up = *reinterpret_cast<const f32x4*>(ldsb + cur + a_row[i] + (((lc + 1) ^ a_x[i]) << 4));
+                split3(lo, up, a0[i], a1[i], a2[i]);
+            }
+#pragma unroll
+            for (int j = 0; j < NT; ++j) {
+                const int off = cur + b_row[j] + (((2 * q + hi) ^ b_x[j]) << 4);
+                w0[j] = *reinterpret_cast<const bf16x8*>(ldsb + off);
+                w1[j] = *reinterpret_cast<const bf16x8*>(ldsb + off + W_BYTES);
+                w2[j] = *reinterpret_cast<const bf16x8*>(ldsb + off + 2 * W_BYTES);
+            }
+#pragma unroll
+            for (int i = 0; i < MT; ++i)
+#pragma unroll
+                for (int j = 0; j < NT; ++j) {
+                    acx[i][j] = __builtin_amdgcn_mfma_f32_32x32x16_bf16(a2[i], w0[j], acx[i][j], 0, 0, 0);
+                    acx[i][j] = __builtin_amdgcn_mfma_f32_32x32x16_bf16(a1[i], w1[j], acx[i][j], 0, 0, 0);
+                    acx[i][j] = __builtin_amdgcn_mfma_f32_32x32x16_bf16(a0[i], w2[j], acx[i][j], 0, 0, 0);
+                    acx[i][j] = __builtin_amdgcn_mfma_f32_32x32x16_bf16(a1[i], w0[j], acx[i][j], 0, 0, 0);
+                    acx[i][j] = __builtin_amdgcn_mfma_f32_32x32x16_bf16(a0[i], w1[j], acx[i][j], 0, 0, 0);
+                    acc[i][j] = __builtin_amdgcn_mfma_f32_32x32x16_bf16(a0[i], w0[j], acc[i][j], 0, 0, 0);
+                }
+        }
+        __builtin_amdgcn_s_waitcnt(0x0F70);
+        __syncthreads();
+    }
+
+#pragma unroll
+    for (int i = 0; i < MT; ++i)
+#pragma unroll
+        for (int j = 0; j < NT; ++j) acc[i][j] += acx[i][j];
+    conv_epilogue<BM, BN, WM, WN>(p, lds, acc, m0, n0, t, lane, wm, wn, rpre, R_PRE && r_pre);
+}
+
+template <int MODE, int BM, int BN, int WM, int WN>
+hipError_t launch_cfg(GemmArgs& p, hipStream_t st) {
+    p.n_mtiles = (p.M + BM - 1) / BM;
+    p.n_ntiles = (p.N + BN - 1) / BN;
+    p.split_k = 1;
+    static const int res_prefetch = [] {
+        const char* e = getenv("HPE_RES_PREFETCH");
+        return e ? atoi(e) : 1;
+    }();
+    p.res_prefetch = res_prefetch;
+    hipLaunchKernelGGL((conv_gemm_f32s_dma_kernel<MODE, BM, BN, WM, WN>), dim3(p.n_mtiles * p.n_ntiles), dim3(64 * WM * WN), 0, st, p);
+    return hipGetLastError();
+}
+
+template <int MODE>
+hipError_t launch_mode(GemmArgs& p, int tile, hipStream_t st) {
+    switch (tile) {
+        case TILE_128x128: return launch_cfg<MODE, 128, 128, 4, 1>(p, st);
+        case TILE_128x128_W8: return launch_cfg<MODE, 128, 128, 4, 2>(p, st);
+        case TILE_256x128_W8: return launch_cfg<MODE, 256, 128, 8, 1>(p, st);
+        default: return hipErrorInvalidValue;
+    }
+}
+
+}
+
+hipError_t hpe_launch_gemm_f32s(GemmArgs p, int mode, int tile, hipStream_t st) {
+    if (p.M <= 0 || p.N <= 0 || p.K <= 0 || (p.K % BK) != 0 || (p.ldw % 8) != 0 || (p.w_piece % 8) != 0 || p.w_piece < p.K ||
+        p.ldw < p.K + 2 * p.w_piece)
+        return hipErrorInvalidValue;
+    if (!p.x || !p.w || !p.y || !p.scale || !p.shift) return hipErrorInvalidValue;
+    if ((p.ldy % 4) != 0 || ((uintptr_t)p.y & 15) != 0) return hipErrorInvalidValue;
+    if (p.y_slab8 && (p.N % 8) != 0) return hipErrorInvalidValue;
+    if (p.res && ((p.ldres % 4) != 0 || ((uintptr_t)p.res & 15) != 0)) return hipErrorInvalidValue;
+    if (((uintptr_t)p.x & 15) != 0 || ((uintptr_t)p.w & 15) != 0) return hipErrorInvalidValue;
+    if (((p.N + 127) / 128) * 128 > p.w_rows) return hipErrorInvalidValue;
+    switch (mode) {
+        case GEMM_DENSE:
+            if (p.lda < p.K || (p.lda % 4) != 0) return hipErrorInvalidValue;
+            return launch_mode<GEMM_DENSE>(p, tile, st);
+        case GEMM_STRIDED:
+            if (p.Cin != p.K || (p.Cin % 4) != 0) return hipErrorInvalidValue;
+            if ((p.Ho - 1) * p.stride >= p.Hi || (p.Wo - 1) * p.stride >= p.Wi) return hipErrorInvalidValue;
+            return launch_mode<GEMM_STRIDED>(p, tile, st);
+        case GEMM_DUAL:
+            if (!p.x2 || ((uintptr_t)p.x2 & 15) != 0 || p.k1_slabs < 1 || p.k1_slabs * BK >= p.K || p.lda < p.k1_slabs * BK || (p.lda % 4) != 0)
+                return hipErrorInvalidValue;
+            if (p.Cin != p.K - p.k1_slabs * BK || (p.Cin % 4) != 0 || p.M != (p.M / (p.Ho * p.Wo)) * p.Ho * p.Wo) return hipErrorInvalidValue;
+            if ((p.Ho - 1) * p.stride >= p.Hi || (p.Wo - 1) * p.stride >= p.Wi) return hipErrorInvalidValue;
+            return launch_mode<GEMM_DUAL>(p, tile, st);
+        default: return hipErrorInvalidValue;
+    }
+}
diff --git a/human-pose-estimation_amd/csrc/hpe_api.hip b/human-pose-estimation_amd/csrc/hpe_api.hip
--- a/human-pose-estimation_amd/csrc/hpe_api.hip
+++ b/human-pose-estimation_amd/csrc/hpe_api.hip
@@ -87,6 +87,8 @@
     float* w_dual = nullptr;
     float* shift_dual = nullptr;
     int k_dual = 0, k1_dual = 0;
+    void* w_split = nullptr;
+    void* w_dual_split = nullptr;
     void* stem_w = nullptr;
     float* wino_u = nullptr;
     float* wino4_u = nullptr;
@@ -125,6 +127,10 @@
     int bf16_p8 = 0;
     int bf16_p8_min_n = 256;
     int bf16_p8_min_k = 512;
+    int f32s_tile = TILE_128x128;
+    int f32s_expand_tile = TILE_128x128_W8;
+    int f32s_expand_min_k = 256;
+    int f32s_min_tiles = 128;
 };
 
 struct hpe_ctx {
@@ -187,6 +193,7 @@
     int halo3_two = 4;
     int halo3 = 0;
     int chain_fuse = 0;
+    int f32_split = 0;
     int co_running = 1;
     float* w4_split = nullptr;
     float* partial_tail = nullptr;
@@ -230,6 +237,44 @@
     if (rc) return rc;
     HIP_TRY(hipMemcpy(*p, h.data(), h.size() * sizeof(float), hipMemcpyHostToDevice));
     return HPE_OK;
+}
+
+int upload_split(hpe_ctx* c, void** p, const std::vector<float>& wt, int rows, int K) {
+    std::vector<unsigned short> ws((size_t)rows * 3 * K);
+    auto bf2f = [](unsigned short h) {
+        const unsigned u = (unsigned)h << 16;
+        float f;
+        memcpy(&f, &u, 4);
+        return f;
+    };
+    for (int n = 0; n < rows; ++n)
+        for (int k = 0; k < K; ++k) {
+            const float x = wt[(size_t)n * K + k];
+            const unsigned short h0 = f2bf(x);
+            const float r1 = x - bf2f(h0);
+            const unsigned short h1 = f2bf(r1);
+            const float r2 = r1 - bf2f(h1);
+            unsigned short* d = &ws[(size_t)n * 3 * K + k];
+            d[0] = h0;
+            d[K] = h1;
+            d[2 * K] = f2bf(r2);
+        }
+    void* q = nullptr;
+    HIP_TRY(hipMalloc(&q, ws.size() * 2));
+    c->allocs.push_back(q);
+    HIP_TRY(hipMemcpy(q, ws.data(), ws.size() * 2, hipMemcpyHostToDevice));
+    *p = q;
+    return HPE_OK;
+}
+
+inline int stage_bit(int hout) { return hout >= 56 ? 1 : (hout >= 28 ? 2 : (hout >= 14 ? 4 : 8)); }
+
+int pick_f32s(const hpe_ctx* c, const void* w_split, int M, int N, int K, bool residual_expand) {
+    if (!w_split || N <= 64) return -1;
+    if (residual_expand && K < c->knobs.f32s_expand_min_k) return -1;
+    const int tile = residual_expand ? c->knobs.f32s_expand_tile : c->knobs.f32s_tile;
+    const int bm = tile == TILE_256x128_W8 ? 256 : 128;
+    return (long)((M + bm - 1) / bm) * ((N + 127) / 128) >= c->knobs.f32s_min_tiles ? tile : -1;
 }
 
 int pick_tile(const TileKnobs& kn, int M, int N, int K, bool residual_expand = false, bool concurrent = false) {
@@ -389,7 +434,15 @@
         const Bf16Plan pl = pick_bf16(c->knobs, p.M, p.N, p.K, mode == GEMM_DENSE && res != nullptr && s.cout == 4 * s.cin, (flags & CONV_CONCURRENT) != 0, mode);
         return hpe_launch_gemm_bf16(p, mode, pl.tile, pl.ns, st);
     }
-    return hpe_launch_gemm(p, mode, pick_tile(c->knobs, p.M, p.N, p.K, mode == GEMM_DENSE && res != nullptr && s.cout == 4 * s.cin, (flags & CONV_CONCURRENT) != 0), st);
+    const bool expand = mode == GEMM_DENSE && res != nullptr && s.cout == 4 * s.cin;
+    const int f32s = (mode == GEMM_DENSE || mode == GEMM_STRIDED) ? pick_f32s(c, L.w_split, p.M, p.N, p.K, expand) : -1;
+    if (f32s >= 0) {
+        p.w = static_cast<const float*>(L.w_split);
+        p.ldw = 3 * L.k_pad;
+        p.w_piece = L.k_pad;
+        return hpe_launch_gemm_f32s(p, mode, f32s, st);
+    }
+    return hpe_launch_gemm(p, mode, pick_tile(c->knobs, p.M, p.N, p.K, expand, (flags & CONV_CONCURRENT) != 0), st);
 }
 
 hipError_t run_dual(hpe_ctx* c, int i2c, int i1, const float* t2, const float* x, int B, float* y, hipStream_t st, int flags) {
@@ -425,6 +478,13 @@
     if (c->bf16) {
         const Bf16Plan pl = pick_bf16(c->knobs, p.M, p.N, p.K, false, (flags & CONV_CONCURRENT) != 0, GEMM_DUAL);
         return hpe_launch_gemm_bf16(p, GEMM_DUAL, pl.tile, pl.ns, st);
+    }
+    const int f32s = pick_f32s(c, L.w_dual_split, p.M, p.N, p.K, false);
+    if (f32s >= 0) {
+        p.w = static_cast<const float*>(L.w_dual_split);
+        p.ldw = 3 * L.k_dual;
+        p.w_piece = L.k_dual;
+        return hpe_launch_gemm_f32s(p, GEMM_DUAL, f32s, st);
     }
     return hpe_launch_gemm(p, GEMM_DUAL, pick_tile(c->knobs, p.M, p.N, p.K, false, (flags & CONV_CONCURRENT) != 0), st);
 }
@@ -717,7 +777,7 @@
     cfg->bn_eps = 1e-3f;
     cfg->encoder_dtype = 0;
     cfg->n_streams = cfg->dual_gemm = cfg->stem_fused = cfg->wino_min_c = cfg->wino_min_items = cfg->wino_fused = -1;
-    cfg->wino_fused_min_hw = cfg->mesh_a2b = cfg->wino_f4 = cfg->wino4_fused = cfg->bf16_p8 = cfg->wino4_ksplit = cfg->chain_fuse = cfg->halo3 = -1;
+    cfg->wino_fused_min_hw = cfg->mesh_a2b = cfg->wino_f4 = cfg->wino4_fused = cfg->bf16_p8 = cfg->wino4_ksplit = cfg->chain_fuse = cfg->halo3 = cfg->f32_split = -1;
 }
 
 int hpe_create(const HpeConfig* cfg, hpe_ctx** out) {
@@ -900,6 +960,11 @@
         c->chain_fuse = c->bf16 ? (opt(c->cfg.chain_fuse, "HPE_CHAIN", 7) & 23) : (opt(c->cfg.chain_fuse, "HPE_CHAIN", 8) & 8);
         c->halo3 = c->bf16 ? (opt(c->cfg.halo3, "HPE_HALO3", 15) & 15) : 0;
         c->halo3_two = opt(-1, "HPE_HALO3_TWO", 4) & 7;
+        c->f32_split = c->bf16 ? 0 : (opt(c->cfg.f32_split, "HPE_F32_SPLIT", 14) & 15);
+        c->knobs.f32s_tile = opt(-1, "HPE_F32S_TILE", c->knobs.f32s_tile);
+        c->knobs.f32s_min_tiles = opt(-1, "HPE_F32S_MIN_TILES", c->knobs.f32s_min_tiles);
+        c->knobs.f32s_expand_tile = opt(-1, "HPE_F32S_EXPAND_TILE", c->knobs.f32s_expand_tile);
+        c->knobs.f32s_expand_min_k = opt(-1, "HPE_F32S_EXPAND_MINK", c->knobs.f32s_expand_min_k);
         c->wino4_fused = c->wino_min_c > 0 ? (opt(c->cfg.wino4_fused, "HPE_WINO4_FUSED", 0) & 12) : 0;
         const char* e;
         e = getenv("HPE_CONCURRENT_TILES");
@@ -970,6 +1035,7 @@
                     L2.w_dual = static_cast<float*>(qd);
                 } else {
                     if ((rc = upload(c, &L2.w_dual, wt))) return rc;
+                    if ((c->f32_split & stage_bit(s2.hout)) && (rc = upload_split(c, &L2.w_dual_split, wt, n_pad, K))) return rc;
                 }
                 if ((rc = upload(c, &L2.shift_dual, sh))) return rc;
                 L2.k_dual = K;
@@ -1008,6 +1074,7 @@
                     for (int n = 0; n < s.cout; ++n) wt[(size_t)n * L.k_pad + k] = src[n];
                 }
         if ((rc = upload(c, &L.w, wt))) return rc;
+        if (i != 0 && s.kh == 1 && (c->f32_split & stage_bit(s.hout)) && (rc = upload_split(c, &L.w_split, wt, L.n_pad, L.k_pad))) return rc;
         if (c->wino_min_c > 0 && s.kh == 3 && s.stride == 1 && s.cin % 32 == 0 && s.cout % 64 == 0 &&
             (s.cin >= c->wino_min_c || (c->wino_fused && s.hin >= c->wino_fused_min_hw))) {
             static const double G[4][3] = {{1, 0, 0}, {0.5, 0.5, 0.5}, {0.5, -0.5, 0.5}, {0, 0, 1}};
diff --git a/human-pose-estimation_amd/csrc/hpe_internal.h b/human-pose-estimation_amd/csrc/hpe_internal.h
--- a/human-pose-estimation_amd/csrc/hpe_internal.h
+++ b/human-pose-estimation_amd/csrc/hpe_internal.h
@@ -27,9 +27,11 @@
     int k1_slabs;
     int res_prefetch;
     int y_slab8;
+    int w_piece;
 };
 
 hipError_t hpe_launch_gemm(GemmArgs p, int mode, int tile, hipStream_t st);
+hipError_t hpe_launch_gemm_f32s(GemmArgs p, int mode, int tile, hipStream_t st);
 
 size_t hpe_wino_v_floats(int B, int H, int W, int C);
 hipError_t hpe_wino_init_device();
diff --git a/human-pose-estimation_amd/engine.py b/human-pose-estimation_amd/engine.py
--- a/human-pose-estimation_amd/engine.py
+++ b/human-pose-estimation_amd/engine.py
@@ -434,7 +434,8 @@
 
     def encoder_kernel_description(self):
         if self.encoder_dtype == "fp32":
-            return ("conv_gemm_f32_dma_kernel (the 1x1 / strided / dual-source layers) + w4_input_kernel + w4_gemm_kernel / w4_gemm32_kernel "
+            return ("conv_gemm_f32s_dma_kernel (the 1x1 / strided / dual-source layers of stages 3-5 on the bf16 matrix cores, operands split "
+                    "exactly into three bf16 pieces) + conv_gemm_f32_dma_kernel (the other 1x1 layers) + w4_input_kernel + w4_gemm_kernel / w4_gemm32_kernel "
                     "(the 13 3x3 layers on the 28x28 / 14x14 / 7x7 maps as fp32 Winograd F(4x4,3x3); F(2x2,3x3) / direct below 64 work "
                     "items) + wino_fused_kernel (the three 56x56 3x3 layers, F(2x2,3x3)) + stem_fused_f32_kernel -- the 53 conv layers of one "
                     "step, priced at their direct-convolution FLOPs")
diff --git a/include/hpe.h b/include/hpe.h
--- a/include/hpe.h
+++ b/include/hpe.h
@@ -45,6 +45,7 @@
     int wino4_ksplit;
     int chain_fuse;
     int halo3;
+    int f32_split;
 } HpeConfig;
 
 void hpe_config_init(HpeConfig* cfg);
```

Result: faster. 21060 images/sec, median of 6 (+12.2%).
